# lowquark/uflow

Hardware: AMD Instinct MI355X
Metric: device-resident frame-CRC GiB/s (1500-B frames, validate: crc+valid per frame) (higher is better)
Workload: dtype u8

## Files before the change

### include/uflow_frame_crc.h

```cpp
#ifndef UFLOW_FRAME_CRC_H
#define UFLOW_FRAME_CRC_H

#include <stddef.h>
#include <stdint.h>

#ifdef __cplusplus
extern "C" {
#endif

#define UFC_OK 0
#define UFC_ERR_INVALID_ARG (-1)
#define UFC_ERR_NO_DEVICE (-2)
#define UFC_ERR_HIP (-3)
#define UFC_ERR_NOMEM (-4)
#define UFC_ERR_COMM (-5)
#define UFC_ERR_PEER (-6)

#define UFC_FRAME_CRC_SIZE 4
#define UFC_FRAME_OVERHEAD 5
#define UFC_MAX_FRAME_SIZE 1472

uint32_t ufc_crc32_compute(const uint8_t* data, size_t len);
uint32_t ufc_crc32_extend(uint32_t initial_crc, const uint8_t* data, size_t len);
int ufc_frame_validate(const uint8_t* frame, size_t len);
int ufc_frame_seal(uint8_t* frame, size_t len);

typedef struct ufc_ctx ufc_ctx;
int ufc_device_count(void);
int ufc_ctx_create(ufc_ctx** out, int device);
int ufc_ctx_destroy(ufc_ctx* ctx);
int ufc_ctx_release_stream(ufc_ctx* ctx, void* stream);
const char* ufc_error_string(int code);
int ufc_ctx_last_hip_error(const ufc_ctx* ctx);

#define UFC_OPT_FIXED_KERNEL 0
#define UFC_FIXED_AUTO 0
#define UFC_FIXED_GENERIC 1
#define UFC_FIXED_CLAIM16 2
#define UFC_OPT_VARLEN_KERNEL 1
#define UFC_VARLEN_AUTO 0
#define UFC_VARLEN_GENERIC 1
#define UFC_VARLEN_SORTED 2
#define UFC_VARLEN_BLOCKED8 3
#define UFC_VARLEN_CLAIM16 4
#define UFC_VARLEN_BLOCKSTREAM 5
#define UFC_VARLEN_SORTED8 6
#define UFC_VARLEN_STREAM 7
#define UFC_OPT_GENERIC_JC 2
#define UFC_OPT_SEAL_KERNEL 3
#define UFC_SEAL_INLINE 0
#define UFC_SEAL_TWO_PASS 1
#define UFC_OPT_COUNT_ 4
int ufc_ctx_set_option(ufc_ctx* ctx, int option, int value);
int ufc_ctx_get_option(const ufc_ctx* ctx, int option);

int ufc_crc_batch_fixed(ufc_ctx* ctx, const uint8_t* d_frames, size_t stride, size_t frame_len, size_t n,
                        uint32_t* d_crc_out, uint8_t* d_valid_out, void* stream);
int ufc_crc_batch_varlen(ufc_ctx* ctx, const uint8_t* d_bytes, const uint64_t* d_offsets, size_t n,
                         uint32_t* d_crc_out, uint8_t* d_valid_out, void* stream);
int ufc_seal_batch_fixed(ufc_ctx* ctx, uint8_t* d_frames, size_t stride, size_t frame_len, size_t n,
                         uint32_t* d_crc_out, void* stream);
int ufc_seal_batch_varlen(ufc_ctx* ctx, uint8_t* d_bytes, const uint64_t* d_offsets, size_t n,
                          uint32_t* d_crc_out, void* stream);

int ufc_crc_batch_pairs(ufc_ctx* ctx, const uint8_t* d_bytes, size_t bytes_len, const uint64_t* d_pairs, size_t n,
                        uint32_t* d_crc_out, uint8_t* d_valid_out, void* stream);

int ufc_hbm_read_probe(ufc_ctx* ctx, const uint8_t* d_buf, size_t bytes, uint32_t* d_sink, size_t* bytes_read,
                       void* stream);

int ufc_validate_host_varlen(ufc_ctx* ctx, const uint8_t* h_bytes, const uint64_t* h_offsets, size_t n,
                             uint32_t* h_crc_out, uint8_t* h_valid_out);
int ufc_validate_host_slots(ufc_ctx* ctx, const uint8_t* h_slots, size_t slot_stride, const uint32_t* h_lens,
                            size_t n, uint32_t* h_crc_out, uint8_t* h_valid_out);
int ufc_validate_host_slots_async(ufc_ctx* ctx, const uint8_t* h_slots, size_t slot_stride, const uint32_t* h_lens,
                                  size_t n, uint32_t* h_crc_out, uint8_t* h_valid_out, void* stream);
int ufc_seal_host_slots(ufc_ctx* ctx, uint8_t* h_slots, size_t slot_stride, const uint32_t* h_lens, size_t n,
                        uint32_t* h_crc_scratch);
int ufc_seal_host_varlen(ufc_ctx* ctx, uint8_t* h_bytes, const uint64_t* h_offsets, size_t n, uint32_t* h_crc_scratch);

#define UFC_COMM_ID_BYTES 128
#define UFC_MAX_RANKS 64
typedef struct ufc_comm ufc_comm;
int ufc_shard_range(uint64_t n_total, int nranks, int rank, uint64_t* first, uint64_t* count);
int ufc_shard_chunk(uint64_t n_total, int nranks, int rank, int chunk, uint64_t* first, uint64_t* count);
int ufc_shard_bounds_fixed(uint64_t n_total, int nranks, uint64_t* bounds);
int ufc_shard_bounds_varlen(const uint64_t* h_offsets, uint64_t n_total, int nranks, uint64_t* bounds);
#define UFC_OP_GATE 0
#define UFC_OP_SEND 1
#define UFC_OP_RECV 2
typedef struct ufc_xfer {
  int32_t op;
  int32_t peer;
  uint64_t src;
  uint64_t dst;
  uint64_t count;
} ufc_xfer;
int ufc_shard_nchunks(const uint64_t* bounds, int nranks);
int ufc_shard_gather_plan(const uint64_t* bounds, int nranks, int rank, int root, int chunk, ufc_xfer* ops,
                          int max_ops);
int ufc_comm_id_create(uint8_t id[UFC_COMM_ID_BYTES]);
int ufc_comm_create(ufc_comm** out, ufc_ctx* ctx, int nranks, int rank, const uint8_t id[UFC_COMM_ID_BYTES]);
int ufc_comm_destroy(ufc_comm* comm);
int ufc_comm_set_timeout(ufc_comm* comm, int timeout_ms);
int ufc_comm_last_error(const ufc_comm* comm);
int ufc_crc_sharded(ufc_comm* comm, const uint8_t* d_frames, size_t stride, size_t frame_len, uint64_t n_total,
                    uint32_t* d_crc_out, uint8_t* d_valid_out, int root, void* stream, void* gather_stream);
int ufc_crc_sharded_varlen(ufc_comm* comm, const uint8_t* d_bytes, const uint64_t* d_offsets, const uint64_t* bounds,
                           uint32_t* d_crc_out, uint8_t* d_valid_out, int root, void* stream, void* gather_stream);

#ifdef __cplusplus
}
#endif

#endif
```

### uflow_amd/_build.py

```python
import os
import subprocess
import sys

PKG_DIR = os.path.dirname(os.path.abspath(__file__))
REPO_DIR = os.path.dirname(PKG_DIR)
CSRC = os.path.join(PKG_DIR, "csrc")
LIB_PATH = os.path.join(PKG_DIR, "libuflowcrc.so")
SOURCES = ["frame_crc.hip", "frame_crc_varlen8.hip", "frame_parse.hip", "frame_build.hip", "frame_pack.hip",
           "packet_emit.hip", "packet_receive.hip", "frame_window.hip", "frame_queue.hip", "send_rate.hip", "resend.hip",
           "flush_ctl.hip", "route.hip", "hbm_probe.hip", "ufc_api.cpp", "ufc_shard.cpp", "crc_math.cpp",
           "frame_codec.cpp"]
HEADERS = ["frame_crc_dev.hpp", "frame_crc_kernels.hpp", "crc_math.hpp", "frame_codec_core.hpp", "frame_parse.hpp",
           "frame_parse_plan.hpp", "frame_build.hpp", "frame_build_piece.hpp", "frame_pack.hpp", "packet_emit.hpp",
           "packet_receive.hpp", "frame_window.hpp", "frame_queue.hpp", "send_rate.hpp", "resend.hpp", "flush_ctl.hpp",
           "route.hpp", "ufc_internal.hpp", "wave.hpp", "wave_dev.hpp", "scratch.hpp", "scan.hpp"]
HIPCC = os.environ.get("HIPCC", "/opt/rocm/bin/hipcc")


def _stale(target, deps):
    if not os.path.exists(target):
        return True
    t = os.path.getmtime(target)
    return any(os.path.getmtime(d) > t for d in deps)


def _digest(paths, extra=()):
    import hashlib
    h = hashlib.sha256()
    for p in paths:
        h.update(os.path.relpath(p, REPO_DIR).encode() + b"\0")
        with open(p, "rb") as f:
            h.update(f.read())
    for x in extra:
        h.update(str(x).encode() + b"\0")
    return h.hexdigest()


def _stamp_ok(target, digest):
    try:
        with open(target + ".sha256") as f:
            return os.path.exists(target) and f.readline().strip() == digest
    except OSError:
        return False


def _stamp_defines(target):
    try:
        with open(target + ".sha256") as f:
            f.readline()
            line = f.readline().strip()
    except OSError:
        return ()
    return tuple(line[len("defines:"):].split()) if line.startswith("defines:") else ()


def _native_identity(defines=()):
    sources = list(SOURCES)
    deps = [os.path.join(CSRC, s) for s in sources + HEADERS]
    deps += [os.path.join(REPO_DIR, "include", h)
             for h in ("uflow_frame_crc.h", "uflow_frame_codec.h", "uflow_flush_ctl.h", "uflow_route.h")]
    flags = [HIPCC, "-O3", "--offload-arch=gfx950", "-fPIC", "-std=c++17", "-Wall",
             "-mllvm", "-amdgpu-atomic-optimizer-strategy=None"]
    flags += ["-D" + d for d in defines]
    per_source = {s: list(UNSTRUCTURED_FLAGS) for s in UNSTRUCTURED_SOURCES}
    extra = [f"{s}:{' '.join(per_source[s])}" for s in sorted(per_source)]
    return sources, flags, per_source, _digest(deps + [os.path.abspath(__file__)], flags[1:] + extra)


UNSTRUCTURED_FLAGS = ("-mllvm", "-structurizecfg-skip-uniform-regions=true")
UNSTRUCTURED_SOURCES = ("frame_crc_varlen8.hip", "frame_crc.hip")


def build_native(force=False, verbose=False, out=None, defines=()):
    sources, flags, per_source, digest = _native_identity(defines)
    target = out or LIB_PATH
    if not force and _stamp_ok(target, digest):
        return target
    objdir = os.path.join(REPO_DIR, "build", "obj_" + os.path.basename(target).replace(".", "_"))
    os.makedirs(objdir, exist_ok=True)
    jobs, objs = [], []
    for src in sources:
        obj = os.path.join(objdir, src + ".o")
        objs.append(obj)
        jobs.append(flags + per_source.get(src, []) + ["-c", os.path.join(CSRC, src), "-o", obj])
    from concurrent.futures import ThreadPoolExecutor

    def run(cmd):
        if verbose:
            print(" ".join(cmd), file=sys.stderr)
        return subprocess.run(cmd).returncode

    with ThreadPoolExecutor(max_workers=max(1, min(8, len(jobs)))) as ex:
        rcs = list(ex.map(run, jobs))
    if any(rcs):
        raise subprocess.CalledProcessError(max(rcs), "hipcc")
    link = [HIPCC, "--offload-arch=gfx950", "-shared", "-fPIC", "-o", target + ".tmp"] + objs + ["-ldl"]
    if verbose:
        print(" ".join(link), file=sys.stderr)
    subprocess.run(link, check=True)
    os.replace(target + ".tmp", target)
    with open(target + ".sha256", "w") as f:
        f.write(digest + "\n")
        if defines:
            f.write("defines: " + " ".join(defines) + "\n")
    return target


LOOPBACK_SRC = os.path.join(REPO_DIR, "tools", "loopback", "ufc_loopback.cpp")
LOOPBACK_BIN = os.path.join(REPO_DIR, "tools", "loopback", "ufc_loopback")


def build_tools(force=False, verbose=False):
    deps = [LOOPBACK_SRC] + [os.path.join(REPO_DIR, "include", h) for h in ("uflow_frame_crc.h", "uflow_frame_codec.h")]
    cmd = [HIPCC, "-O2", "-std=c++17", "-Wall", "-o", LOOPBACK_BIN + ".tmp", LOOPBACK_SRC,
           "-L" + PKG_DIR, "-luflowcrc", "-Wl,-rpath,$ORIGIN/../../uflow_amd", "-lpthread"]
    digest = _digest(deps + [os.path.abspath(__file__)], cmd[1:])
    if not force and _stamp_ok(LOOPBACK_BIN, digest):
        return LOOPBACK_BIN
    if verbose:
        print(" ".join(cmd), file=sys.stderr)
    subprocess.run(cmd, check=True)
    os.replace(LOOPBACK_BIN + ".tmp", LOOPBACK_BIN)
    with open(LOOPBACK_BIN + ".sha256", "w") as f:
        f.write(digest + "\n")
    return LOOPBACK_BIN


def build_oracle(force=False):
    odir = os.path.join(REPO_DIR, "oracle")
    target = os.path.join(odir, "liboracle.so")
    digest = _digest([os.path.join(odir, "crc_oracle.c"), os.path.join(odir, "Makefile")])
    if force or not _stamp_ok(target, digest):
        subprocess.run(["make", "-C", odir, "-s", "-B"], check=True)
        with open(target + ".sha256", "w") as f:
            f.write(digest + "\n")
    return target


if __name__ == "__main__":
    build_native(force="--force" in sys.argv, verbose=True)
    build_oracle(force="--force" in sys.argv)
    build_tools(force="--force" in sys.argv, verbose=True)
    print(LIB_PATH)
```

### uflow_amd/_native.py

```python
import ctypes
import os

from ._build import LIB_PATH as _DEFAULT_LIB

LIB_PATH = os.environ["UFC_LIB"] if os.environ.get("UFC_AB") == "1" and os.environ.get("UFC_LIB") else _DEFAULT_LIB

UFC_OK = 0
UFC_ERR_INVALID_ARG = -1
UFC_ERR_NO_DEVICE = -2
UFC_ERR_HIP = -3
UFC_ERR_NOMEM = -4
UFC_ERR_COMM = -5
UFC_ERR_PEER = -6
UFC_COMM_ID_BYTES = 128
UFC_MAX_RANKS = 64
UFC_OP_GATE, UFC_OP_SEND, UFC_OP_RECV = 0, 1, 2

UFC_OPT_FIXED_KERNEL, UFC_OPT_VARLEN_KERNEL, UFC_OPT_GENERIC_JC = 0, 1, 2
UFC_FIXED_AUTO, UFC_FIXED_GENERIC, UFC_FIXED_CLAIM16 = 0, 1, 2
UFC_VARLEN_AUTO, UFC_VARLEN_GENERIC, UFC_VARLEN_SORTED, UFC_VARLEN_BLOCKED8, UFC_VARLEN_CLAIM16 = 0, 1, 2, 3, 4
UFC_VARLEN_BLOCKSTREAM, UFC_VARLEN_SORTED8, UFC_VARLEN_STREAM = 5, 6, 7
UFC_OPT_SEAL_KERNEL, UFC_SEAL_INLINE, UFC_SEAL_TWO_PASS = 3, 0, 1
UFC_BUILD_OK, UFC_BUILD_SKIPPED, UFC_BUILD_BAD_FIELD, UFC_BUILD_BAD_SRC = 0, 1, 2, 3
UFC_PACK_DONE, UFC_PACK_SIZE_LIMITED, UFC_PACK_WINDOW_LIMITED, UFC_PACK_BAD_RANGE = 0, 1, 2, 3
UFC_SEND_TIME_SENSITIVE, UFC_SEND_UNRELIABLE, UFC_SEND_PERSISTENT, UFC_SEND_RELIABLE = 0, 1, 2, 3
UFC_NO_PARENT = 0xFFFFFFFF
UFC_EMIT_DONE, UFC_EMIT_WINDOW_LIMITED, UFC_EMIT_ALLOC_LIMITED, UFC_EMIT_BAD_PACKET, UFC_EMIT_BAD_RANGE = 0, 1, 2, 3, 4
UFC_PACKET_NOT_REACHED, UFC_PACKET_EMITTED, UFC_PACKET_DROPPED = 0, 1, 2
UFC_RX_ASM_OPEN, UFC_RX_ASM_CLOSED, UFC_RX_ASM_ACTIVE = 0, 1, 2
UFC_RX_SLOT_ENTRY, UFC_RX_SLOT_DATA, UFC_RX_SLOT_DUD = 1, 2, 4
UFC_RX_PACKET_DUD = 1
(UFC_RX_NOT_HANDLED, UFC_RX_STORED, UFC_RX_COMPLETED, UFC_RX_DUD, UFC_RX_DROPPED_INVALID, UFC_RX_DROPPED_WINDOW,
 UFC_RX_DROPPED_CHANNEL, UFC_RX_DROPPED_CLOSED, UFC_RX_DROPPED_MISMATCH, UFC_RX_DROPPED_DUPLICATE,
 UFC_RX_DROPPED_BAD_SRC) = range(11)
UFC_RX_STATUS_COUNT = 11
UFC_RX_DONE, UFC_RX_BAD_STATE = 0, 1
UFC_FW_DONE, UFC_FW_BAD_STATE = 0, 1
UFC_SENT_NONCE, UFC_SENT_RATE_LIMITED, UFC_SENT_ACKED, UFC_SENT_MARK = 1, 2, 4, 8
UFC_FQ_HAS_RTT, UFC_FQ_RESET_LOSS, UFC_FQ_MARK_RATE_LIMITED, UFC_FQ_FORGET, UFC_FQ_FEEDBACK = 1, 2, 4, 8, 16
UFC_FQ_DONE, UFC_FQ_BAD_STATE = 0, 1
UFC_RATE_AWAIT_SEND, UFC_RATE_SLOW_START, UFC_RATE_THROUGHPUT_EQN = 0, 1, 2
UFC_RATE_FRAME_SENT = 1
UFC_RATE_DONE, UFC_RATE_BAD_STATE, UFC_RATE_REF_PANIC, UFC_RATE_RECV_FULL = 0, 1, 2, 3
UFC_RATE_FEEDBACK, UFC_RATE_NOFEEDBACK, UFC_RATE_RESET_ISSUED, UFC_RATE_ENTERED_EQN, UFC_RATE_INV_STALLED = 1, 2, 4, 8, 16
UFC_TX_RESEND = 1
UFC_RS_NO_DATA_FLUSH = 1
(UFC_RS_DONE, UFC_RS_SIZE_LIMITED, UFC_RS_WINDOW_LIMITED, UFC_RS_REF_HANG, UFC_RS_BAD_STATE, UFC_RS_STAGE_FULL,
 UFC_RS_HEAP_FULL) = range(7)
UFC_FA_DONE, UFC_FA_BAD_STATE, UFC_FA_CARRY_FULL = 0, 1, 2
(UFC_FS_SENT, UFC_FS_ACK_LIMITED, UFC_FS_DATA_LIMITED, UFC_FS_UPSTREAM, UFC_FS_NOT_DUE, UFC_FS_IDLE,
 UFC_FS_NO_ALLOC) = range(7)
UFC_ROUTE_DROP, UFC_ROUTE_CONN, UFC_ROUTE_CONTROL, UFC_ROUTE_DEFERRED = range(4)

_c_u8p = ctypes.POINTER(ctypes.c_uint8)
_V, _Z, _I = ctypes.c_void_p, ctypes.c_size_t, ctypes.c_int
_PARSE_ARGS = [_V, _V, _Z, _V, _V, _V, _Z]
_BUILD_SIZES_ARGS = [_V, _V, _Z, _V, _Z, _Z, _V, _V]
_BUILD_ARGS = [_V, _V, _Z, _V, _V, _Z, _Z, _V, _V, _Z, _I, _V]
_PACK_ARGS = [_V, _Z, _V, _V, _Z, _V, _V, _Z, _V]
_EMIT_ARGS = [_V, _Z, _V, _V, _Z, _V, _Z, _V, _V, _V, _V]
_RX_ARGS = [_V, _Z, _V, _V, _Z, _V, _V, _Z, _V, _V, _Z, _V, _V, _Z, _V, _Z, _V, _Z, _V, _V, _V, _Z, _V, _V, _V, _Z, _V,
            _V, _V, _V]
_FW_ARGS = [_V, _Z, _V, _V, _Z, _V, _V, _Z, _V, _V, _V, _V]
_FQ_ARGS = [_V, _Z, _V, _Z, _V, _V, _Z, _V, _V, _V, _Z, _V, _Z, _V, _Z, _V, _V]
_RATE_BEGIN_ARGS = [_V, _V, _V, _Z, _V, _V]
_RS_BEGIN_ARGS = [_V, _Z, _V, _V, _V, _Z, _V, _V, _V, _V, _V, _Z, _V, _Z, _V, _Z, _V, _Z, _V, _Z, _V, _Z, _V, _Z, _V, _V,
                  _V]
_RS_PLACE_ARGS = [_V, _V, _Z, _V, _Z, _V, _V, _Z]
_RS_COMMIT_ARGS = [_V, _V, _Z, _V, _V, _V, _Z, _V, _V, _Z, _V, _V, _V, _V, _V, _V, _V, _Z, _V, _Z, _V, _Z, _V, _Z, _V, _Z,
                   _V, _Z, _V, _V, _V, _V, _V]
_RATE_STEP_ARGS = [_V, _V, _V, _Z, _V, _Z, _V, _Z, _V, _V, _Z, _V, _V, _V]
_FLUSH_ACKS_ARGS = [_V, _V, _V, _Z, _V, _V, _V, _Z, _V, _Z, _V, _Z, _V, _V, _V, _Z, _V, _V, _V, _V, _V, _V, _V]
_FLUSH_SYNC_ARGS = [_V, _V, _V, _V, _V, _V, _V, _V, _Z, _V, _Z, _V, _V, _V, _V, _V]
_U32, _U64 = ctypes.c_uint32, ctypes.c_uint64
_ROUTE_ARGS = [_V, _V, _V, _Z, _V, _Z, _U32, _U32, _Z, _V, _U64, _U64, _V, _V, _V, _V, _V, _V, _V, _V, _V, _V]
_SIGNATURES = {
    "ufc_crc32_compute": (ctypes.c_uint32, [ctypes.c_void_p, ctypes.c_size_t]),
    "ufc_crc32_extend": (ctypes.c_uint32, [ctypes.c_uint32, ctypes.c_void_p, ctypes.c_size_t]),
    "ufc_frame_validate": (ctypes.c_int, [ctypes.c_void_p, ctypes.c_size_t]),
    "ufc_frame_seal": (ctypes.c_int, [ctypes.c_void_p, ctypes.c_size_t]),
    "ufc_device_count": (ctypes.c_int, []),
    "ufc_ctx_create": (ctypes.c_int, [ctypes.POINTER(ctypes.c_void_p), ctypes.c_int]),
    "ufc_ctx_destroy": (ctypes.c_int, [ctypes.c_void_p]),
    "ufc_ctx_release_stream": (ctypes.c_int, [ctypes.c_void_p, ctypes.c_void_p]),
    "ufc_error_string": (ctypes.c_char_p, [ctypes.c_int]),
    "ufc_ctx_last_hip_error": (ctypes.c_int, [ctypes.c_void_p]),
    "ufc_ctx_set_option": (ctypes.c_int, [ctypes.c_void_p, ctypes.c_int, ctypes.c_int]),
    "ufc_ctx_get_option": (ctypes.c_int, [ctypes.c_void_p, ctypes.c_int]),
    "ufc_crc_batch_fixed": (ctypes.c_int, [ctypes.c_void_p, ctypes.c_void_p, ctypes.c_size_t, ctypes.c_size_t,
                                           ctypes.c_size_t, ctypes.c_void_p, ctypes.c_void_p, ctypes.c_void_p]),
    "ufc_crc_batch_varlen": (ctypes.c_int, [ctypes.c_void_p, ctypes.c_void_p, ctypes.c_void_p, ctypes.c_size_t,
                                            ctypes.c_void_p, ctypes.c_void_p, ctypes.c_void_p]),
    "ufc_seal_batch_fixed": (ctypes.c_int, [ctypes.c_void_p, ctypes.c_void_p, ctypes.c_size_t, ctypes.c_size_t,
                                            ctypes.c_size_t, ctypes.c_void_p, ctypes.c_void_p]),
    "ufc_seal_batch_varlen": (ctypes.c_int, [ctypes.c_void_p, ctypes.c_void_p, ctypes.c_void_p, ctypes.c_size_t,
                                             ctypes.c_void_p, ctypes.c_void_p]),
    "ufc_hbm_read_probe": (ctypes.c_int, [ctypes.c_void_p, ctypes.c_void_p, ctypes.c_size_t, ctypes.c_void_p,
                                          ctypes.POINTER(ctypes.c_size_t), ctypes.c_void_p]),
    "ufc_validate_host_varlen": (ctypes.c_int, [ctypes.c_void_p, ctypes.c_void_p, ctypes.c_void_p, ctypes.c_size_t,
                                                ctypes.c_void_p, ctypes.c_void_p]),
    "ufc_crc_batch_pairs": (ctypes.c_int, [ctypes.c_void_p, ctypes.c_void_p, ctypes.c_size_t, ctypes.c_void_p,
                                           ctypes.c_size_t, ctypes.c_void_p, ctypes.c_void_p, ctypes.c_void_p]),
    "ufc_validate_host_slots": (ctypes.c_int, [ctypes.c_void_p, ctypes.c_void_p, ctypes.c_size_t, ctypes.c_void_p,
                                               ctypes.c_size_t, ctypes.c_void_p, ctypes.c_void_p]),
    "ufc_validate_host_slots_async": (ctypes.c_int, [ctypes.c_void_p, ctypes.c_void_p, ctypes.c_size_t, ctypes.c_void_p,
                                                     ctypes.c_size_t, ctypes.c_void_p, ctypes.c_void_p, ctypes.c_void_p]),
    "ufc_seal_host_slots": (ctypes.c_int, [ctypes.c_void_p, ctypes.c_void_p, ctypes.c_size_t, ctypes.c_void_p,
                                           ctypes.c_size_t, ctypes.c_void_p]),
    "ufc_seal_host_varlen": (ctypes.c_int, [ctypes.c_void_p, ctypes.c_void_p, ctypes.c_void_p, ctypes.c_size_t,
                                            ctypes.c_void_p]),
    "ufc_shard_range": (ctypes.c_int, [ctypes.c_uint64, ctypes.c_int, ctypes.c_int, ctypes.POINTER(ctypes.c_uint64),
                                       ctypes.POINTER(ctypes.c_uint64)]),
    "ufc_shard_chunk": (ctypes.c_int, [ctypes.c_uint64, ctypes.c_int, ctypes.c_int, ctypes.c_int,
                                       ctypes.POINTER(ctypes.c_uint64), ctypes.POINTER(ctypes.c_uint64)]),
    "ufc_shard_bounds_fixed": (ctypes.c_int, [ctypes.c_uint64, ctypes.c_int, ctypes.c_void_p]),
    "ufc_shard_bounds_varlen": (ctypes.c_int, [ctypes.c_void_p, ctypes.c_uint64, ctypes.c_int, ctypes.c_void_p]),
    "ufc_shard_nchunks": (ctypes.c_int, [ctypes.c_void_p, ctypes.c_int]),
    "ufc_shard_gather_plan": (ctypes.c_int, [ctypes.c_void_p, ctypes.c_int, ctypes.c_int, ctypes.c_int, ctypes.c_int,
                                             ctypes.c_void_p, ctypes.c_int]),
    "ufc_comm_id_create": (ctypes.c_int, [ctypes.c_void_p]),
    "ufc_comm_create": (ctypes.c_int, [ctypes.POINTER(ctypes.c_void_p), ctypes.c_void_p, ctypes.c_int, ctypes.c_int,
                                       ctypes.c_void_p]),
    "ufc_comm_destroy": (ctypes.c_int, [ctypes.c_void_p]),
    "ufc_comm_last_error": (ctypes.c_int, [ctypes.c_void_p]),
    "ufc_comm_set_timeout": (ctypes.c_int, [ctypes.c_void_p, ctypes.c_int]),
    "ufc_crc_sharded": (ctypes.c_int, [ctypes.c_void_p, ctypes.c_void_p, ctypes.c_size_t, ctypes.c_size_t, ctypes.c_uint64,
                                       ctypes.c_void_p, ctypes.c_void_p, ctypes.c_int, ctypes.c_void_p, ctypes.c_void_p]),
    "ufc_crc_sharded_varlen": (ctypes.c_int, [ctypes.c_void_p, ctypes.c_void_p, ctypes.c_void_p, ctypes.c_void_p,
                                              ctypes.c_void_p, ctypes.c_void_p, ctypes.c_int, ctypes.c_void_p,
                                              ctypes.c_void_p]),
    "ufc_frame_read": (ctypes.c_int, [ctypes.c_void_p, ctypes.c_size_t, ctypes.c_void_p, ctypes.c_void_p,
                                      ctypes.c_size_t]),
    "ufc_frame_parse": (ctypes.c_int, [ctypes.c_void_p, ctypes.c_size_t, ctypes.c_int, ctypes.c_void_p,
                                       ctypes.c_void_p, ctypes.c_size_t]),
    "ufc_datagram_is_valid": (ctypes.c_int, [ctypes.c_void_p]),
    "ufc_frame_write_fixed": (ctypes.c_size_t, [ctypes.c_void_p, ctypes.c_void_p, ctypes.c_size_t, ctypes.c_int]),
    "ufc_data_frame_builder_init": (ctypes.c_int, [ctypes.c_void_p, ctypes.c_void_p, ctypes.c_size_t, ctypes.c_uint32,
                                                   ctypes.c_int]),
    "ufc_data_frame_builder_add": (ctypes.c_int, [ctypes.c_void_p, ctypes.c_void_p]),
    "ufc_data_frame_encoded_size": (ctypes.c_size_t, [ctypes.c_void_p]),
    "ufc_ack_frame_builder_init": (ctypes.c_int, [ctypes.c_void_p, ctypes.c_void_p, ctypes.c_size_t, ctypes.c_uint32,
                                                  ctypes.c_uint32]),
    "ufc_ack_frame_builder_add": (ctypes.c_int, [ctypes.c_void_p, ctypes.c_uint32, ctypes.c_uint32, ctypes.c_int]),
    "ufc_builder_size": (ctypes.c_size_t, [ctypes.c_void_p]),
    "ufc_builder_build": (ctypes.c_size_t, [ctypes.c_void_p, ctypes.c_int]),
    "ufc_parse_batch_host": (_I, _PARSE_ARGS + [ctypes.POINTER(_Z), _I]),
    "ufc_parse_batch_varlen": (_I, [_V] + _PARSE_ARGS + [_V, _V]),
    "ufc_build_sizes_host": (_I, _BUILD_SIZES_ARGS + [_I]),
    "ufc_build_batch_host": (_I, _BUILD_ARGS + [_I]),
    "ufc_build_sizes_varlen": (_I, [_V] + _BUILD_SIZES_ARGS + [_V]),
    "ufc_build_batch_varlen": (_I, [_V] + _BUILD_ARGS + [_V]),
    "ufc_pack_host": (_I, _PACK_ARGS + [ctypes.POINTER(ctypes.c_uint64), _I]),
    "ufc_pack_varlen": (_I, [_V] + _PACK_ARGS + [_V, _V]),
    "ufc_emit_packets_host": (_I, _EMIT_ARGS + [ctypes.POINTER(ctypes.c_uint64), _I]),
    "ufc_emit_packets_varlen": (_I, [_V] + _EMIT_ARGS + [_V, _V]),
    "ufc_receive_packets_host": (ctypes.c_int, _RX_ARGS + [ctypes.c_int]),
    "ufc_receive_packets_varlen": (ctypes.c_int, [ctypes.c_void_p] + _RX_ARGS + [ctypes.c_void_p]),
    "ufc_frame_window_host": (ctypes.c_int, _FW_ARGS + [ctypes.c_int]),
    "ufc_frame_window_varlen": (ctypes.c_int, [ctypes.c_void_p] + _FW_ARGS + [ctypes.c_void_p]),
    "ufc_frame_queue_host": (ctypes.c_int, _FQ_ARGS + [ctypes.c_int]),
    "ufc_frame_queue_varlen": (ctypes.c_int, [ctypes.c_void_p] + _FQ_ARGS + [ctypes.c_void_p]),
    "ufc_rate_begin_host": (ctypes.c_int, _RATE_BEGIN_ARGS + [ctypes.c_int]),
    "ufc_rate_begin_varlen": (ctypes.c_int, [ctypes.c_void_p] + _RATE_BEGIN_ARGS + [ctypes.c_void_p]),
    "ufc_rate_step_host": (ctypes.c_int, _RATE_STEP_ARGS + [ctypes.c_int]),
    "ufc_rate_step_varlen": (ctypes.c_int, [ctypes.c_void_p] + _RATE_STEP_ARGS + [ctypes.c_void_p]),
    "ufc_resend_begin_host": (ctypes.c_int, _RS_BEGIN_ARGS + [ctypes.c_int]),
    "ufc_resend_begin_varlen": (ctypes.c_int, [ctypes.c_void_p] + _RS_BEGIN_ARGS + [ctypes.c_void_p]),
    "ufc_resend_place_host": (ctypes.c_int, _RS_PLACE_ARGS + [ctypes.c_int]),
    "ufc_resend_place_varlen": (ctypes.c_int, [ctypes.c_void_p] + _RS_PLACE_ARGS + [ctypes.c_void_p]),
    "ufc_resend_commit_host": (ctypes.c_int, _RS_COMMIT_ARGS + [ctypes.c_int]),
    "ufc_resend_commit_varlen": (ctypes.c_int, [ctypes.c_void_p] + _RS_COMMIT_ARGS + [ctypes.c_void_p]),
}
SYMBOLS = tuple(_SIGNATURES)
_FLUSH_SIGNATURES = {
    "ufc_flush_acks_host": (_I, _FLUSH_ACKS_ARGS + [_I]),
    "ufc_flush_acks_varlen": (_I, [_V] + _FLUSH_ACKS_ARGS + [_V]),
    "ufc_flush_sync_host": (_I, _FLUSH_SYNC_ARGS + [_I]),
    "ufc_flush_sync_varlen": (_I, [_V] + _FLUSH_SYNC_ARGS + [_V]),
}
FLUSH_SYMBOLS = tuple(_FLUSH_SIGNATURES)
_ROUTE_SIGNATURES = {
    "ufc_route_table_build_host": (_I, [_V, _Z, _U32, _V, _Z, _V, _V]),
    "ufc_route_frames_host": (_I, _ROUTE_ARGS + [_I]),
    "ufc_route_frames_varlen": (_I, [_V] + _ROUTE_ARGS + [_V]),
}
ROUTE_SYMBOLS = tuple(_ROUTE_SIGNATURES)


class FrameInfo(ctypes.Structure):
    _fields_ = [("kind", ctypes.c_uint8), ("ok", ctypes.c_uint8), ("aux", ctypes.c_uint8), ("crc_ok", ctypes.c_uint8),
                ("f", ctypes.c_uint32 * 5), ("item_count", ctypes.c_uint32), ("item_first", ctypes.c_uint32)]


class Item(ctypes.Structure):
    _fields_ = [("id", ctypes.c_uint32), ("channel_id", ctypes.c_uint8), ("form", ctypes.c_uint8),
                ("window_parent_lead", ctypes.c_uint16), ("channel_parent_lead", ctypes.c_uint16),
                ("fragment_id", ctypes.c_uint16), ("fragment_id_last", ctypes.c_uint16), ("flags", ctypes.c_uint16),
                ("data_offset", ctypes.c_uint32), ("data_len", ctypes.c_uint32)]


class Builder(ctypes.Structure):
    _fields_ = [("buf", ctypes.c_void_p), ("cap", ctypes.c_size_t), ("len", ctypes.c_size_t),
                ("count", ctypes.c_uint32), ("kind", ctypes.c_uint32)]


class Xfer(ctypes.Structure):
    _fields_ = [("op", ctypes.c_int32), ("peer", ctypes.c_int32), ("src", ctypes.c_uint64), ("dst", ctypes.c_uint64),
                ("count", ctypes.c_uint64)]


class DatagramRef(ctypes.Structure):
    _fields_ = [("sequence_id", ctypes.c_uint32), ("channel_id", ctypes.c_uint8), ("reserved", ctypes.c_uint8),
                ("window_parent_lead", ctypes.c_uint16), ("channel_parent_lead", ctypes.c_uint16),
                ("fragment_id", ctypes.c_uint16), ("fragment_id_last", ctypes.c_uint16),
                ("data", ctypes.c_void_p), ("data_len", ctypes.c_size_t)]

_lib = None


class NativeError(RuntimeError):
    def __init__(self, code, what=""):
        msg = _lib.ufc_error_string(code).decode() if _lib is not None else str(code)
        super().__init__(f"{what}: {msg} (code {code})" if what else f"{msg} (code {code})")
        self.code = code


def lib():
    global _lib
    if _lib is None:
        if not os.path.exists(LIB_PATH):
            raise ImportError(f"libuflowcrc.so not found at {LIB_PATH}: run `python -m uflow_amd._build` "
                              "(the native library is required; there is no CPU fallback)")
        l = ctypes.CDLL(LIB_PATH)
        for name, (res, args) in (list(_SIGNATURES.items()) + list(_FLUSH_SIGNATURES.items()) +
                                   list(_ROUTE_SIGNATURES.items())):
            fn = getattr(l, name)
            fn.restype = res
            fn.argtypes = args
        _lib = l
    return _lib


def check(rc, what=""):
    if rc != UFC_OK:
        raise NativeError(rc, what)
    return rc
```

### uflow_amd/csrc/frame_crc.hip

```cpp
#include "frame_crc_dev.hpp"

namespace ufc_dev {

struct RunAcc {
  uint32_t crc;
  uint32_t valid;
};

template <bool SEAL>
__device__ __forceinline__ void finish_set(const Lane& L, const KernelParams& p, const FrameDesc& d, const Chains& c,
                                           uint64_t set, int t, RunAcc& acc) {
  const uint32_t X0 = L.odd ? c.v2 : c.v0, X1 = L.odd ? c.v3 : c.v1;
  const uint32_t X2 = L.odd ? c.v0 : c.v2, X3 = L.odd ? c.v1 : c.v3;
  uint32_t lin = xor3(nib_mul<0>(L.lds, X0, L.K2), nib_mul<1>(L.lds, X1, L.K2), nib_mul<2>(L.lds, X2, L.K2)) ^
                 nib_mul<3>(L.lds, X3, L.K2);
  lin = row_xor16(lin);
  const uint32_t crc = ~lin;
  if (SEAL) {
    const uint64_t f = set * 4 + (uint64_t)L.grp;
    if (L.col == 15 && f < p.nframes && d.len >= 4u) {
      uint8_t* a = p.wbytes + d.start + d.n;
      if (((uintptr_t)a & 3u) == 0) {
        *as_global<g_u32w>((uint32_t*)a) = __builtin_bswap32(crc);
      } else {
        g_u8w* w = as_global<g_u8w>(a);
        w[0] = (uint8_t)(crc >> 24);
        w[1] = (uint8_t)(crc >> 16);
        w[2] = (uint8_t)(crc >> 8);
        w[3] = (uint8_t)crc;
      }
    }
  }
  const uint32_t ok = (d.len >= 5u && __builtin_bswap32(c.tr) == crc) ? 1u : 0u;
  const int dst = L.lane - 4 * t;
#pragma unroll
  for (int g = 0; g < 4; g++) {
    const uint32_t cg = __builtin_amdgcn_readlane(crc, 16 * g);
    acc.crc = (dst == g) ? cg : acc.crc;
    if (!SEAL) {
      const uint32_t vg = __builtin_amdgcn_readlane(ok, 16 * g + 15);
      acc.valid = (dst == g) ? vg : acc.valid;
    }
  }
}

template <bool SEAL>
__device__ __forceinline__ void store_run(const Lane& L, const KernelParams& p, uint64_t run_first, const RunAcc& acc) {
  const uint64_t f = run_first + (uint64_t)L.lane;
  if (f < p.nframes) {
    if (p.crc_out) *as_global<g_u32w>(p.crc_out + f) = acc.crc;
    if (!SEAL && p.valid_out) *as_global<g_u8w>(p.valid_out + f) = (uint8_t)acc.valid;
  }
}

template <bool SEAL>
__device__ __forceinline__ void slow_set(const Lane& L, const KernelParams& p, const FrameDesc& d, int nblocks,
                                         uint64_t set, int t, RunAcc& acc) {
  Chains c{0u, 0u, 0u, 0u, 0u};
#pragma unroll 1
  for (int blk = 0; blk < nblocks; blk++) {
    const int bl = min(blk, d.J - 1);
    uint32_t w[4];
#pragma unroll
    for (int b = 0; b < 4; b++) {
      const int o = 256 * bl + 16 * L.col + 4 * b - d.pad;
      uint32_t a = 0;
#pragma unroll 1
      for (int k = 0; k < 4; k++) {
        const int ob = o + k;
        if (ob >= 0 && ob < (int)d.len) a |= (uint32_t)*as_global<g_u8>(p.bytes + d.start + (uint64_t)ob) << (8 * k);
      }
      w[b] = a;
    }
    process_block<true>(L, d, blk, make_uint4(w[0], w[1], w[2], w[3]), c);
  }
  finish_set<SEAL>(L, p, d, c, set, t, acc);
}


template <int JC>
__device__ __forceinline__ void load_item(const uint8_t* lane_base, int part, ItemBuf<JC>& b) {
  const uint8_t* q = lane_base + (int64_t)part * (JC * 256);
#pragma unroll
  for (int j = 0; j < JC; j++) {
    const u32x4 v = __builtin_nontemporal_load(as_global<g_u32x4>(q + 256 * j));
    b.x[j] = make_uint4(v.x, v.y, v.z, v.w);
  }
}

template <int JC, bool FREEZE, bool PART0>
__device__ __forceinline__ void compute_item(const Lane& L, const FrameDesc& d, int part, const ItemBuf<JC>& b,
                                             Chains& c) {
#pragma unroll
  for (int j = 0; j < JC; j++) process_block<FREEZE>(L, d, PART0 ? j : part * JC + j, b.x[j], c);
}

template <int JC, int MODE>
__global__ __launch_bounds__(1024) void frame_crc_kernel(const KernelParams p) {
  constexpr bool VARLEN = (MODE & kModeVarlen) != 0;
  constexpr bool SEAL = (MODE & kModeSeal) != 0;
  constexpr bool FREEZE = VARLEN || (MODE & kModeFreeze) != 0;
  constexpr bool SINGLE = !VARLEN && (MODE & kModeFreeze) == 0;
  __shared__ __attribute__((aligned(16))) char lds[kLdsBytes];
  stage_tables(p, lds);

  Lane L;
  init_lane(L, lds, p.G);
  const uint64_t nsets = (p.nframes + 3) >> 2;
  const uint64_t W = (uint64_t)gridDim.x * (blockDim.x >> 6);
  const uint32_t wid = __builtin_amdgcn_readfirstlane(threadIdx.x >> 6);
  const uint64_t w0 = (uint64_t)blockIdx.x * (blockDim.x >> 6) + wid;
  constexpr int R = kSetsPerRun;
  uint64_t run = w0;
  int t = 0;
  if (run * R >= nsets) return;
  auto set_of = [&](uint64_t r, int tt) -> uint64_t { return r * R + (uint64_t)tt; };
  auto next_pos = [&](uint64_t r, int tt, uint64_t& r2, int& t2) {
    if (tt + 1 < R && set_of(r, tt + 1) < nsets) {
      r2 = r;
      t2 = tt + 1;
    } else {
      r2 = r + W;
      t2 = 0;
    }
  };
  const uint64_t buf_end =
      VARLEN ? *as_global<g_u64>(p.offsets + p.nframes) : (p.nframes - 1) * p.stride + p.frame_len;

  auto frame_index = [&](uint64_t set) -> uint64_t {
    const uint64_t f = set * 4 + (uint64_t)L.grp;
    return f < p.nframes ? f : p.nframes - 1;
  };
  auto desc_now = [&](uint64_t set) -> FrameDesc {
    const uint64_t f = frame_index(set);
    if (VARLEN) {
      const uint64_t a = *as_global<g_u64>(p.offsets + f), b = *as_global<g_u64>(p.offsets + f + 1);
      return make_desc(a, b - a);
    }
    return make_desc(f * p.stride, p.frame_len);
  };
  auto wave_max = [&](int v) -> int {
    int m = __builtin_amdgcn_readlane(v, 0);
    m = max(m, __builtin_amdgcn_readlane(v, 16));
    m = max(m, __builtin_amdgcn_readlane(v, 32));
    m = max(m, __builtin_amdgcn_readlane(v, 48));
    return m;
  };
  auto set_parts = [&](const FrameDesc& dd) -> int { return (wave_max(dd.J) + JC - 1) / JC; };
  auto set_slow = [&](const FrameDesc& dd, int parts) -> bool {
    const int bad =
        (dd.start < (uint64_t)dd.pad || dd.start - dd.pad + (uint64_t)(256 * JC) * parts > buf_end) ? 1 : 0;
    return wave_max(bad) != 0;
  };

  RunAcc acc{0u, 0u};
  auto after_set = [&](uint64_t r, int tt) {
    uint64_t r2;
    int t2;
    next_pos(r, tt, r2, t2);
    if (r2 != r) store_run<SEAL>(L, p, set_of(r, 0) * 4, acc);
  };

  FrameDesc d = desc_now(set_of(run, t));
  int parts = set_parts(d);
  while (set_slow(d, parts)) {
    slow_set<SEAL>(L, p, d, parts * JC, set_of(run, t), t, acc);
    after_set(run, t);
    next_pos(run, t, run, t);
    if (set_of(run, t) >= nsets) return;
    d = desc_now(set_of(run, t));
    parts = set_parts(d);
  }

  struct Cursor {
    uint64_t run;
    int t, part, parts;
    bool valid, slow;
    FrameDesc d;
  };
  uint64_t pre_a = 0, pre_b = 0;
  auto prefetch_offsets = [&](uint64_t r2, int t2) {
    if (VARLEN) {
      const uint64_t s2 = set_of(r2, t2);
      const uint64_t f = frame_index(s2 < nsets ? s2 : 0);
      pre_a = *as_global<g_u64>(p.offsets + f);
      pre_b = *as_global<g_u64>(p.offsets + f + 1);
    }
  };
  auto advance = [&](Cursor& c) {
    if (!c.valid || c.slow) {
      c.valid = false;
      return;
    }
    if (!SINGLE && c.part + 1 < c.parts) {
      c.part++;
      return;
    }
    uint64_t r2;
    int t2;
    next_pos(c.run, c.t, r2, t2);
    c.run = r2;
    c.t = t2;
    c.part = 0;
    if (set_of(r2, t2) >= nsets) {
      c.valid = false;
      return;
    }
    c.d = VARLEN ? make_desc(pre_a, pre_b - pre_a) : make_desc(frame_index(set_of(r2, t2)) * p.stride, p.frame_len);
    {
      uint64_t r3;
      int t3;
      next_pos(r2, t2, r3, t3);
      prefetch_offsets(r3, t3);
    }
    c.parts = set_parts(c.d);
    c.slow = set_slow(c.d, c.parts);
  };
  auto lane_base = [&](const Cursor& c) -> const uint8_t* { return p.bytes + c.d.start - c.d.pad + 16 * L.col; };

  Cursor C0{run, t, 0, parts, true, false, d};
  {
    uint64_t r2;
    int t2;
    next_pos(run, t, r2, t2);
    prefetch_offsets(r2, t2);
  }
  Cursor C1 = C0;
  advance(C1);
  Cursor C2 = C1;
  advance(C2);
  auto load_cursor = [&](const Cursor& c, ItemBuf<JC>& b) {
    const bool ok = c.valid && !c.slow;
    load_item<JC>(ok ? lane_base(c) : lane_base(C0), ok ? c.part : 0, b);
  };

  Chains c{0u, 0u, 0u, 0u, 0u};
  bool go_slow = false;
  uint64_t slow_run = 0;
  int slow_t = 0;
  auto step = [&](ItemBuf<JC>& cur, ItemBuf<JC>& nxt2) -> bool {
    {
      const bool ok = C2.valid && !C2.slow;
      const uint8_t* q = (ok ? lane_base(C2) : lane_base(C0)) + (int64_t)(ok ? C2.part : 0) * (JC * 256);
      const bool p0 = SINGLE || C0.part == 0;
      if (!p0) __builtin_assume(C0.part >= 1);
#pragma unroll
      for (int j = 0; j < JC; j++) {
        const u32x4 v = __builtin_nontemporal_load(as_global<g_u32x4>(q + 256 * j));
        nxt2.x[j] = make_uint4(v.x, v.y, v.z, v.w);
        __builtin_amdgcn_sched_barrier(0);
        if (p0)
          process_block<FREEZE>(L, C0.d, j, cur.x[j], c);
        else
          process_block<FREEZE>(L, C0.d, C0.part * JC + j, cur.x[j], c);
        __builtin_amdgcn_sched_barrier(0);
      }
    }
    if (SINGLE || C0.part + 1 == C0.parts) {
      finish_set<SEAL>(L, p, C0.d, c, set_of(C0.run, C0.t), C0.t, acc);
      after_set(C0.run, C0.t);
    }
    if (!C1.valid) return false;
    if (C1.slow) {
      go_slow = true;
      slow_run = C1.run;
      slow_t = C1.t;
      return false;
    }
    C0 = C1;
    C1 = C2;
    advance(C2);
    return true;
  };
  {
    ItemBuf<JC> X, Y, Z;
    load_cursor(C0, X);
    load_cursor(C1, Y);
    while (step(X, Z) && step(Y, X) && step(Z, Y)) {
    }
  }
  if (go_slow) {
    run = slow_run;
    t = slow_t;
    while (set_of(run, t) < nsets) {
      d = desc_now(set_of(run, t));
      parts = set_parts(d);
      slow_set<SEAL>(L, p, d, parts * JC, set_of(run, t), t, acc);
      after_set(run, t);
      next_pos(run, t, run, t);
    }
  }
}




constexpr int lean_loadv(int skip, int first, int mid, int last) { return skip | first << 1 | mid << 6 | last << 11; }
[[maybe_unused]] constexpr int kLoadvAllNT = lean_loadv(0, kFixAuxNT, kFixAuxNT, kFixAuxNT);
constexpr int kLoadvProduct = lean_loadv(0, 0, kFixAuxNT, kFixAuxNT);
template <int J, bool SEAL, int DEPTH, int SCHED, int WAVES, int LOADV = kLoadvProduct>
__global__ __launch_bounds__(WAVES * 64) void frame_crc_fixed_kernel(const KernelParams p) {
  static_assert(DEPTH >= 1 && DEPTH <= 3, "pipeline depth (4 spills at J = 6)");
  static_assert(DEPTH != 1 || SCHED != kSchedClaim, "depth 1: static schedules only");
  constexpr bool DYN = SCHED == kSchedClaim;
  constexpr bool ILV = SCHED == kSchedInterleave;
  constexpr uint32_t kInc = ILV ? (uint32_t)WAVES : 1u;
  __shared__ __attribute__((aligned(16))) char lds[kLdsBytes];
  const StageSet<WAVES * 64> sr = stage_load<WAVES * 64>(p);
  Lane L;
  init_lane(L, lds, p.G);

  const uint64_t stride = p.stride;
  const uint32_t len = (uint32_t)p.frame_len;
  const uint32_t n = len - 4u;
  const int pad = J * 256 - (int)len;
  const uint32_t nsets = (uint32_t)((p.nframes + 3) >> 2);
  const uint32_t nfull = (uint32_t)(p.nframes >> 2);
  const bool tail = (p.nframes & 3) != 0;
  const uint32_t wpb = WAVES;
  const uint32_t wid = __builtin_amdgcn_readfirstlane(threadIdx.x >> 6);
  const uint32_t w = blockIdx.x * wpb + wid;
  const uint32_t s_edge =
      p.front_ok ? 0u : (uint32_t)min(((uint64_t)pad + 4 * stride - 1) / (4 * stride), (uint64_t)nsets);
  const bool edge0 = s_edge == 1 && (p.nframes - 1) * stride + len >= 16;
  const uint32_t s_fast = edge0 ? 0u : s_edge;
  const uint32_t nfast = nfull - s_fast;
  uint32_t q_lo, q_end, q_cur, q_nx1, q_nx2;
  if (DYN || ILV) {
    q_lo = s_fast + (uint32_t)((uint64_t)nfast * blockIdx.x / gridDim.x);
    q_end = s_fast + (uint32_t)((uint64_t)nfast * (blockIdx.x + 1) / gridDim.x);
    q_cur = q_lo + wid;
    q_nx1 = q_lo + wpb + wid;
  } else {
    const uint32_t NW = gridDim.x * wpb;
    q_lo = s_fast + (uint32_t)((uint64_t)nfast * w / NW);
    q_end = s_fast + (uint32_t)((uint64_t)nfast * (w + 1) / NW);
    q_cur = q_lo;
    q_nx1 = q_lo + 1;
  }
  uint32_t* ctr = DYN ? p.ctr + blockIdx.x * kCtrWordsPerBlock : nullptr;
  auto claim_issue = [&]() -> uint32_t {
    uint32_t v = 0;
    if (L.lane == 0) v = __hip_atomic_fetch_add(ctr, 1u, __ATOMIC_RELAXED, __HIP_MEMORY_SCOPE_AGENT);
    return v;
  };
  auto claim_set = [&](uint32_t v) -> uint32_t {
    return q_lo + (DEPTH - 1) * wpb + __builtin_amdgcn_readfirstlane(v);
  };

  const int64_t lane_off = (int64_t)L.grp * (int64_t)stride + 16 * L.col - pad;
  uint32_t dm[4], pre[4];
#pragma unroll
  for (int b = 0; b < 4; b++) {
    const int o = 16 * L.col + 4 * b - pad;
    const uint32_t fz = fix_word(0u, o, L.G);
    const uint32_t f1 = fix_word(0xFFFFFFFFu, o, L.G);
    dm[b] = f1 & ~fz;
    pre[b] = fz;
  }
  uint32_t dm1, pre1;
  {
    const int o = 256 + 16 * L.col - pad;
    const uint32_t fz = fix_word(0u, o, L.G), f1 = fix_word(0xFFFFFFFFu, o, L.G);
    dm1 = f1 & ~fz;
    pre1 = fz;
  }
  const uint32_t tmask = (L.col == 15) ? 0u : 0xFFFFFFFFu;

  constexpr int RUNS = lean_runs(WAVES);
  uint32_t acc_crc = 0, acc_qv = 0;
  uint32_t hist_crc[RUNS], hist_qv[RUNS];
#pragma unroll
  for (int r = 0; r < RUNS; r++) hist_crc[r] = hist_qv[r] = 0;
  uint32_t t = 0, nhist = 0;
  auto write_trailer = [&](uint64_t f, uint32_t crc) {
    uint8_t* a = p.wbytes + f * stride + n;
    if (((uintptr_t)a & 3u) == 0) {
      *as_global<g_u32w>((uint32_t*)a) = __builtin_bswap32(crc);
    } else {
      g_u8w* wp = as_global<g_u8w>(a);
      wp[0] = (uint8_t)(crc >> 24);
      wp[1] = (uint8_t)(crc >> 16);
      wp[2] = (uint8_t)(crc >> 8);
      wp[3] = (uint8_t)crc;
    }
  };
  auto store_run = [&](int cnt, uint32_t crcs, uint32_t qv) {
    const uint64_t f = (uint64_t)(qv & 0x7FFFFFFFu) * 4 + (uint64_t)L.grp;
    if (L.col < cnt && f < p.nframes) {
      if (p.crc_out) *as_global<g_u32w>(p.crc_out + f) = crcs;
      if (!SEAL && p.valid_out) *as_global<g_u8w>(p.valid_out + f) = (uint8_t)(qv >> 31);
      if (SEAL) write_trailer(f, crcs);
    }
  };
  auto store_all = [&]() {
    if (t > 0) store_run((int)t, acc_crc, acc_qv);
#pragma unroll
    for (int r = 0; r < RUNS; r++)
      if ((uint32_t)r < nhist) store_run(kSetsPerRun, hist_crc[r], hist_qv[r]);
  };
  auto finish = [&](uint32_t q, const Chains& c, bool may_overflow) {
    const uint32_t crc = ~group_lin(L, c);
    const uint32_t tr = (uint32_t)__builtin_amdgcn_update_dpp(0, (int)c.tr, 0x15F, 0xF, 0xF, false);
    const uint32_t ok = (len >= 5u && __builtin_bswap32(tr) == crc) ? 1u : 0u;
    acc_crc = (L.col == (int)t) ? crc : acc_crc;
    acc_qv = (L.col == (int)t) ? (q | (ok << 31)) : acc_qv;
    if (++t == kSetsPerRun) {
      if (may_overflow && nhist == RUNS) {
        t = 0;
        store_all();
        __builtin_amdgcn_s_waitcnt(0x0F70);
        nhist = 0;
      }
#pragma unroll
      for (int r = RUNS - 1; r > 0; r--) {
        hist_crc[r] = hist_crc[r - 1];
        hist_qv[r] = hist_qv[r - 1];
      }
      hist_crc[0] = acc_crc;
      hist_qv[0] = acc_qv;
      nhist++;
      t = 0;
    }
  };
  auto compute_block = [&](uint32_t q, int j, uint4 x, Chains& c) {
    {
      if (j == J - 1) {
        c.tr = x.w;
        x.w &= tmask;
      }
      if (j == 0) {
        c.v0 = (x.x & dm[0]) | pre[0];
        c.v1 = (x.y & dm[1]) | pre[1];
        c.v2 = (x.z & dm[2]) | pre[2];
        c.v3 = (x.w & dm[3]) | pre[3];
      } else {
        if (j == 1) x.x = (x.x & dm1) | pre1;
        c.v0 = chain_step(L.lds, c.v0, L.K, x.x);
        c.v1 = chain_step(L.lds, c.v1, L.K, x.y);
        c.v2 = chain_step(L.lds, c.v2, L.K, x.z);
        c.v3 = chain_step(L.lds, c.v3, L.K, x.w);
      }
    }
  };
  auto compute = [&](uint32_t q, const ItemBuf<J>& b, Chains& c) {
#pragma unroll
    for (int j = 0; j < J; j++) compute_block(q, j, b.x[j], c);
  };
  const uint32_t voff = (uint32_t)(lane_off + 512);
  auto set_base = [&](uint32_t q) -> const uint8_t* {
    return p.bytes + (uint64_t)(q < q_end ? q : nfull - 1) * 4 * stride - 512;
  };
  auto load_edge0 = [&](ItemBuf<J>& b) {
    const int64_t room = (int64_t)min(p.nframes - 1, (uint64_t)3);
    const int64_t over = (int64_t)L.grp > room ? (int64_t)L.grp - room : 0;
    const int64_t off0 = lane_off - over * (int64_t)stride;
#pragma unroll
    for (int j = 0; j < J; j++) {
      const int64_t off = off0 + 256 * j;
      uint4 v = load_frame16<true>(p.bytes + (off < 0 ? 0 : off));
      if (off < 0) {
        const int64_t d = -off;
        uint64_t lo = (uint64_t)v.x | ((uint64_t)v.y << 32), hi = (uint64_t)v.z | ((uint64_t)v.w << 32);
        if (d >= 16) {
          lo = hi = 0;
        } else if (d >= 8) {
          hi = lo << (8 * (d - 8));
          lo = 0;
        } else {
          hi = (hi << (8 * d)) | (lo >> (64 - 8 * d));
          lo = lo << (8 * d);
        }
        v = make_uint4((uint32_t)lo, (uint32_t)(lo >> 32), (uint32_t)hi, (uint32_t)(hi >> 32));
      }
      b.x[j] = v;
    }
  };
  const uint32_t voff_b0 = ((LOADV & 1) && 16 * L.col + 16 <= pad - 4) ? kFixRecords : voff;
  auto load = [&](uint32_t q, ItemBuf<J>& b) {
    constexpr int kAuxFirst = (LOADV >> 1) & 31, kAuxMid = (LOADV >> 6) & 31, kAuxLast = (LOADV >> 11) & 31;
    const __amdgpu_buffer_rsrc_t rs =
        __builtin_amdgcn_make_buffer_rsrc((void*)set_base(q), 0, (int)kFixRecords, kFixRsrcWord3);
#pragma unroll
    for (int j = 0; j < J; j++) {
      const uint32_t o = (j == 0 ? voff_b0 : voff) + 256u * j;
      u32x4 v;
      if (j == 0)
        v = __builtin_amdgcn_raw_buffer_load_b128(rs, (int)o, 0, kAuxFirst);
      else if (j == J - 1)
        v = __builtin_amdgcn_raw_buffer_load_b128(rs, (int)o, 0, kAuxLast);
      else
        v = __builtin_amdgcn_raw_buffer_load_b128(rs, (int)o, 0, kAuxMid);
      b.x[j] = make_uint4(v.x, v.y, v.z, v.w);
    }
  };
  auto load_tail = [&](ItemBuf<J>& b) {
    const int64_t room = (int64_t)(p.nframes - 1 - 4 * (uint64_t)nfull);
    const int64_t over = (int64_t)L.grp > room ? (int64_t)L.grp - room : 0;
    load_set<J>(p.bytes + (uint64_t)nfull * 4 * stride - 512, voff - (uint32_t)(over * (int64_t)stride), b);
  };

  ItemBuf<J> A, B, C;
  uint32_t cX = 0, cY = 0, cZ = 0;
  if (DYN) {
    cY = claim_issue();
    cZ = claim_issue();
  }
  if (edge0 && q_cur == 0)
    load_edge0(A);
  else
    load(q_cur, A);
  if (DEPTH == 3) load(q_nx1, B);
  stage_store<WAVES * 64>(sr, lds);
  q_nx2 = (DEPTH == 3 && !DYN) ? q_cur + 2 * kInc : 0;

  if (w == 0 && s_fast > 0) {
#pragma unroll 1
    for (uint32_t e = 0; e < s_fast; e++) {
      FrameDesc d = make_desc(min((uint64_t)e * 4 + (uint64_t)L.grp, p.nframes - 1) * stride, len);
      Chains ce{0u, 0u, 0u, 0u, 0u};
#pragma unroll 1
      for (int blk = 0; blk < J; blk++) {
        uint32_t wv[4];
#pragma unroll
        for (int b = 0; b < 4; b++) {
          const int o = 256 * blk + 16 * L.col + 4 * b - d.pad;
          uint32_t a = 0;
#pragma unroll 1
          for (int k = 0; k < 4; k++) {
            const int ob = o + k;
            if (ob >= 0 && ob < (int)d.len) a |= (uint32_t)*as_global<g_u8>(p.bytes + d.start + (uint64_t)ob) << (8 * k);
          }
          wv[b] = a;
        }
        process_block<false>(L, d, blk, make_uint4(wv[0], wv[1], wv[2], wv[3]), ce);
      }
      const uint32_t crc = ~group_lin(L, ce);
      const uint32_t ok = (len >= 5u && __builtin_bswap32(ce.tr) == crc) ? 1u : 0u;
      const uint64_t f = (uint64_t)e * 4 + (uint64_t)L.grp;
      if (L.col == 15 && f < p.nframes) {
        if (p.crc_out) *as_global<g_u32w>(p.crc_out + f) = crc;
        if (!SEAL && p.valid_out) *as_global<g_u8w>(p.valid_out + f) = (uint8_t)ok;
        if (SEAL) write_trailer(f, crc);
      }
    }
    __builtin_amdgcn_s_waitcnt(0x0F70);
  }


  Chains c{0u, 0u, 0u, 0u, 0u};
  auto step = [&](ItemBuf<J>& cur, ItemBuf<J>& fill, uint32_t& c_issue, uint32_t& c_read) {
    uint32_t q_load;
    if (DYN) {
      q_load = claim_set(c_read);
      c_issue = claim_issue();
    } else {
      q_load = (DEPTH == 3) ? q_nx2 : q_nx1;
    }
    load(q_load, fill);
    __builtin_amdgcn_sched_barrier(0);
    if (q_cur < q_end) {
      compute(q_cur, cur, c);
      finish(q_cur, c, DYN);
    }
    __builtin_amdgcn_sched_barrier(0);
    if (DEPTH == 3) {
      q_cur = q_nx1;
      q_nx1 = q_load;
      q_nx2 = q_load + kInc;
    } else {
      q_cur = q_load;
      q_nx1 = q_load + kInc;
    }
  };
  if (DEPTH == 1) {
    while (q_cur < q_end) {
      compute(q_cur, A, c);
      finish(q_cur, c, false);
      q_cur += kInc;
      load(q_cur, A);
    }
  } else if (DEPTH == 2 && !DYN) {
    while (q_cur < q_end) {
      step(A, B, cX, cY);
      step(B, A, cY, cZ);
    }
  } else if (DEPTH == 2) {
    while (q_cur < q_end) {
      step(A, B, cX, cY);
      step(B, A, cY, cZ);
      step(A, B, cZ, cX);
      step(B, A, cX, cY);
      step(A, B, cY, cZ);
      step(B, A, cZ, cX);
    }
  } else {
    while (q_cur < q_end) {
      step(A, C, cX, cY);
      step(B, A, cY, cZ);
      step(C, B, cZ, cX);
    }
  }
  if (tail && blockIdx.x == gridDim.x - 1 && wid == wpb - 1) {
    ItemBuf<J> T;
    load_tail(T);
    compute(nfull, T, c);
    const uint32_t crc = ~group_lin(L, c);
    const uint32_t tr = (uint32_t)__builtin_amdgcn_update_dpp(0, (int)c.tr, 0x15F, 0xF, 0xF, false);
    const uint32_t ok = (len >= 5u && __builtin_bswap32(tr) == crc) ? 1u : 0u;
    const uint64_t f = (uint64_t)nfull * 4 + (uint64_t)L.grp;
    if (L.col == 0 && f < p.nframes) {
      if (p.crc_out) *as_global<g_u32w>(p.crc_out + f) = crc;
      if (!SEAL && p.valid_out) *as_global<g_u8w>(p.valid_out + f) = (uint8_t)ok;
      if (SEAL) write_trailer(f, crc);
    }
  }
  if (DYN) {
    store_all();
  } else {
    uint32_t blo = q_lo, bhi = q_end;
    if (!ILV) {
      const uint64_t NW = (uint64_t)gridDim.x * wpb;
      blo = s_fast + (uint32_t)((uint64_t)nfast * (blockIdx.x * wpb) / NW);
      bhi = s_fast + (uint32_t)((uint64_t)nfast * ((blockIdx.x + 1) * wpb) / NW);
    }
    const uint32_t nfr = 4 * (bhi - blo);
    uint32_t* lcrc = (uint32_t*)lds;
    uint8_t* lval = (uint8_t*)lds + 4 * nfr;
    __builtin_amdgcn_fence(__ATOMIC_RELEASE, "workgroup", "local");
    __builtin_amdgcn_s_barrier();
    __builtin_amdgcn_fence(__ATOMIC_ACQUIRE, "workgroup", "local");
    auto stage = [&](int cnt, uint32_t crcs, uint32_t qv) {
      if (L.col < cnt) {
        const uint32_t q = qv & 0x7FFFFFFFu;
        const uint32_t pos = (q - blo) * 4 + (uint32_t)L.grp;
        lcrc[pos] = crcs;
        lval[pos] = (uint8_t)(qv >> 31);
      }
    };
    if (t > 0) stage((int)t, acc_crc, acc_qv);
#pragma unroll
    for (int r = 0; r < RUNS; r++)
      if ((uint32_t)r < nhist) stage(kSetsPerRun, hist_crc[r], hist_qv[r]);
    __builtin_amdgcn_fence(__ATOMIC_RELEASE, "workgroup", "local");
    __builtin_amdgcn_s_barrier();
    __builtin_amdgcn_fence(__ATOMIC_ACQUIRE, "workgroup", "local");
    const uint64_t f0 = (uint64_t)blo * 4;
    if (p.crc_out)
      for (uint32_t i = threadIdx.x; i < nfr; i += WAVES * 64) *as_global<g_u32w>(p.crc_out + f0 + i) = lcrc[i];
    if (SEAL) {
      for (uint32_t i = threadIdx.x; i < nfr; i += WAVES * 64) {
        const uint32_t v = __builtin_bswap32(lcrc[i]);
        uint8_t* a = p.wbytes + (f0 + i) * stride + n;
        if (((uintptr_t)a & 3u) == 0) {
          __builtin_nontemporal_store(v, as_global<g_u32w>((uint32_t*)a));
        } else {
          g_u8w* wp = as_global<g_u8w>(a);
          __builtin_nontemporal_store((uint8_t)v, wp);
          __builtin_nontemporal_store((uint8_t)(v >> 8), wp + 1);
          __builtin_nontemporal_store((uint8_t)(v >> 16), wp + 2);
          __builtin_nontemporal_store((uint8_t)(v >> 24), wp + 3);
        }
      }
    }
    if (!SEAL && p.valid_out) {
      if ((((uintptr_t)(p.valid_out + f0)) & 3u) == 0) {
        for (uint32_t i = threadIdx.x; i < nfr / 4; i += WAVES * 64)
          *as_global<g_u32w>((uint32_t*)(p.valid_out + f0) + i) = ((const uint32_t*)lval)[i];
      } else {
        for (uint32_t i = threadIdx.x; i < nfr; i += WAVES * 64) *as_global<g_u8w>(p.valid_out + f0 + i) = lval[i];
      }
    }
  }

  if (DYN) {
    __builtin_amdgcn_s_waitcnt(0x0F70);
    uint32_t done = 0;
    if (L.lane == 0) done = __hip_atomic_fetch_add(ctr + 1, 1u, __ATOMIC_RELAXED, __HIP_MEMORY_SCOPE_AGENT);
    if (__builtin_amdgcn_readfirstlane(done) == wpb - 1 && L.lane == 0) {
      __hip_atomic_store(ctr, 0u, __ATOMIC_RELAXED, __HIP_MEMORY_SCOPE_AGENT);
      __hip_atomic_store(ctr + 1, 0u, __ATOMIC_RELAXED, __HIP_MEMORY_SCOPE_AGENT);
    }
  }
}

#define UFC_INST_FIXED(J)                                                                                  \
  template __global__ void frame_crc_fixed_kernel<J, false, 2, kSchedInterleave, 8>(const KernelParams); \
  template __global__ void frame_crc_fixed_kernel<J, true, 2, kSchedInterleave, 8>(const KernelParams);
UFC_INST_FIXED(1) UFC_INST_FIXED(2) UFC_INST_FIXED(3) UFC_INST_FIXED(4) UFC_INST_FIXED(5) UFC_INST_FIXED(6)


const void* fixed_kernel_symbol(int J, bool seal, int depth, int sched, int waves) {
  if (depth == 2 && sched == kSchedInterleave && waves == 8) {
    switch (J) {
#define UFC_PICK_FIXED(JJ)                                                                          \
  case JJ:                                                                                          \
    return seal ? (const void*)frame_crc_fixed_kernel<JJ, true, 2, kSchedInterleave, 8>          \
                : (const void*)frame_crc_fixed_kernel<JJ, false, 2, kSchedInterleave, 8>;
      UFC_PICK_FIXED(1) UFC_PICK_FIXED(2) UFC_PICK_FIXED(3) UFC_PICK_FIXED(4) UFC_PICK_FIXED(5) UFC_PICK_FIXED(6)
#undef UFC_PICK_FIXED
      default: return nullptr;
    }
  }
  return nullptr;
}

#define UFC_INST_MODES(JC)                                                                          \
  template __global__ void frame_crc_kernel<JC, 0>(const KernelParams);                             \
  template __global__ void frame_crc_kernel<JC, kModeSeal>(const KernelParams);                     \
  template __global__ void frame_crc_kernel<JC, kModeFreeze>(const KernelParams);                   \
  template __global__ void frame_crc_kernel<JC, kModeFreeze | kModeSeal>(const KernelParams);       \
  template __global__ void frame_crc_kernel<JC, kModeVarlen>(const KernelParams);                   \
  template __global__ void frame_crc_kernel<JC, kModeVarlen | kModeSeal>(const KernelParams);

#define UFC_CONFIGS(X) X(1) X(2) X(3) X(4) X(5) X(6)

UFC_CONFIGS(UFC_INST_MODES)


const void* kernel_symbol(int jc, int mode) {
#define UFC_PICK(JC)                                                                                   \
  if (jc == JC) {                                                                                      \
    switch (mode) {                                                                                    \
      case 0: return (const void*)frame_crc_kernel<JC, 0>;                                            \
      case kModeSeal: return (const void*)frame_crc_kernel<JC, kModeSeal>;                            \
      case kModeFreeze: return (const void*)frame_crc_kernel<JC, kModeFreeze>;                        \
      case kModeFreeze | kModeSeal: return (const void*)frame_crc_kernel<JC, kModeFreeze | kModeSeal>; \
      case kModeVarlen: return (const void*)frame_crc_kernel<JC, kModeVarlen>;                        \
      case kModeVarlen | kModeSeal: return (const void*)frame_crc_kernel<JC, kModeVarlen | kModeSeal>; \
      default: break;                                                                                  \
    }                                                                                                  \
  }
  UFC_CONFIGS(UFC_PICK)
#undef UFC_PICK
  return nullptr;
}

bool config_available(int jc) { return jc >= 1 && jc <= 6; }

namespace {
__global__ __launch_bounds__(256) void seal_scatter_kernel(uint8_t* bytes, uint64_t stride, uint64_t n_off,
                                                           uint64_t nframes, const uint32_t* crc) {
  for (uint64_t i = (uint64_t)blockIdx.x * 256 + threadIdx.x; i < nframes; i += (uint64_t)gridDim.x * 256) {
    const uint32_t v = __builtin_bswap32(crc[i]);
    uint8_t* a = bytes + i * stride + n_off;
    if (((uintptr_t)a & 3u) == 0) {
      __builtin_nontemporal_store(v, (uint32_t*)a);
    } else {
      __builtin_nontemporal_store((uint8_t)v, a);
      __builtin_nontemporal_store((uint8_t)(v >> 8), a + 1);
      __builtin_nontemporal_store((uint8_t)(v >> 16), a + 2);
      __builtin_nontemporal_store((uint8_t)(v >> 24), a + 3);
    }
  }
}
}

int seal_scatter(uint8_t* bytes, uint64_t stride, uint64_t frame_len, uint64_t nframes, const uint32_t* crc,
                 void* stream) {
  if (nframes == 0) return 0;
  const uint64_t blocks = std::min<uint64_t>((nframes + 255) / 256, 1u << 20);
  hipLaunchKernelGGL(seal_scatter_kernel, dim3((unsigned)blocks), dim3(256), 0, (hipStream_t)stream, bytes, stride,
                     frame_len - 4, nframes, crc);
  return (int)hipGetLastError();
}

}
```

### uflow_amd/csrc/frame_crc_dev.hpp

```cpp
#pragma once
#include <hip/hip_runtime.h>
#include <cstdint>

#include "frame_crc_kernels.hpp"

namespace ufc_dev {

typedef unsigned int u32x4 __attribute__((ext_vector_type(4)));
typedef const __attribute__((address_space(1))) u32x4 g_u32x4;
typedef const __attribute__((address_space(1))) uint8_t g_u8;
typedef const __attribute__((address_space(1))) uint32_t g_u32;
typedef const __attribute__((address_space(1))) uint64_t g_u64;
typedef __attribute__((address_space(1))) uint8_t g_u8w;
typedef __attribute__((address_space(1))) uint32_t g_u32w;

template <typename G, typename T>
__device__ __forceinline__ G* as_global(T* p) {
  return (G*)(p);
}

constexpr int kSetsPerRun = 16;

__device__ __forceinline__ uint32_t xor3(uint32_t a, uint32_t b, uint32_t c) {
  return __builtin_amdgcn_bitop3_b32(a, b, c, 0x96);
}

__device__ __forceinline__ uint32_t perm(uint32_t a, uint32_t b, uint32_t sel) {
  return __builtin_amdgcn_perm(a, b, sel);
}

constexpr uint32_t kChainBase = 32768u;
constexpr uint32_t kSelChain0 = 0x0C020400u, kSelChain1 = 0x0C020501u, kSelChain2 = 0x0C030600u,
                   kSelChain3 = 0x0C030701u;

__device__ __forceinline__ uint32_t chain_step(const char* lds, uint32_t v, uint32_t K, uint32_t x) {
  const char* t = lds + kChainBase;
  const uint32_t r0 = *(const uint32_t*)(t + perm(v, K, kSelChain0));
  const uint32_t r1 = *(const uint32_t*)(t + perm(v, K, kSelChain1));
  const uint32_t r2 = *(const uint32_t*)(t + perm(v, K, kSelChain2));
  const uint32_t r3 = *(const uint32_t*)(t + perm(v, K, kSelChain3));
  return xor3(xor3(r0, r1, r2), r3, x);
}

template <int I>
__device__ __forceinline__ uint32_t nib_mul(const char* lds, uint32_t v, uint32_t K2) {
  const uint32_t lo = v & 0x0F0F0F0Fu;
  const uint32_t hi = (v >> 4) & 0x0F0F0F0Fu;
  uint32_t r[8];
#pragma unroll
  for (int k = 0; k < 8; k++) {
    const uint32_t sel = 0x0C0C0000u | ((uint32_t)(4 + (k >> 1)) << 8) | (uint32_t)I;
    r[k] = *(const uint32_t*)(lds + perm((k & 1) ? hi : lo, K2, sel) + k * 4096);
  }
  return xor3(xor3(r[0], r[1], r[2]), xor3(r[3], r[4], r[5]), xor3(r[6], r[7], 0u));
}

template <int I>
__device__ __forceinline__ void nib_terms(const char* lds, uint32_t v, uint32_t K2, uint32_t* r) {
  const uint32_t lo = v & 0x0F0F0F0Fu, hi = (v >> 4) & 0x0F0F0F0Fu;
#pragma unroll
  for (int k = 0; k < 8; k++) {
    const uint32_t sel = 0x0C0C0000u | ((uint32_t)(4 + (k >> 1)) << 8) | (uint32_t)I;
    r[k] = *(const uint32_t*)(lds + perm((k & 1) ? hi : lo, K2, sel) + k * 4096);
  }
}

__device__ __forceinline__ uint32_t nib_mul4(const char* lds, uint32_t X0, uint32_t X1, uint32_t X2, uint32_t X3,
                                             uint32_t K2) {
  uint32_t r[32];
  nib_terms<0>(lds, X0, K2, r);
  nib_terms<1>(lds, X1, K2, r + 8);
  nib_terms<2>(lds, X2, K2, r + 16);
  nib_terms<3>(lds, X3, K2, r + 24);
  uint32_t t[12];
#pragma unroll
  for (int k = 0; k < 10; k++) t[k] = xor3(r[3 * k], r[3 * k + 1], r[3 * k + 2]);
  t[10] = r[30];
  t[11] = r[31];
  const uint32_t u0 = xor3(t[0], t[1], t[2]), u1 = xor3(t[3], t[4], t[5]), u2 = xor3(t[6], t[7], t[8]),
                 u3 = xor3(t[9], t[10], t[11]);
  return xor3(u0, u1, u2) ^ u3;
}

__device__ __forceinline__ uint32_t row_xor16(uint32_t v) {
  v ^= (uint32_t)__builtin_amdgcn_update_dpp(0, (int)v, 0xB1, 0xF, 0xF, false);
  v ^= (uint32_t)__builtin_amdgcn_update_dpp(0, (int)v, 0x4E, 0xF, 0xF, false);
  v ^= (uint32_t)__builtin_amdgcn_update_dpp(0, (int)v, 0x124, 0xF, 0xF, false);
  v ^= (uint32_t)__builtin_amdgcn_update_dpp(0, (int)v, 0x128, 0xF, 0xF, false);
  return v;
}


__host__ __device__ __forceinline__ uint32_t fix_word(uint32_t v, int o, uint32_t G) {
  const uint64_t pv = (uint64_t)G << 32;
  const uint32_t sh = (uint32_t)(8 * (o + 8)) & 63u;
  const uint32_t pre = (uint32_t)(pv >> sh);
  const uint32_t dm = (o > -4 && o < 0) ? (0xFFFFFFFFu << ((uint32_t)(-8 * o) & 31u)) : 0u;
  const uint32_t mixed = (v & dm) | (pre & ~dm);
  return (o >= 0) ? v : ((o <= -8) ? 0u : mixed);
}

__host__ __device__ __forceinline__ uint4 front_fix(uint4 x, int p, uint32_t G) {
  const uint32_t pc = (uint32_t)(p < 0 ? 0 : (p > 20 ? 20 : p));
  const uint32_t s = 8u * pc;
  const uint64_t lo = (uint64_t)x.x | ((uint64_t)x.y << 32), hi = (uint64_t)x.z | ((uint64_t)x.w << 32);
  const uint64_t mlo = s >= 64u ? 0ull : ~0ull << (s & 63u);
  const uint64_t mhi = s >= 128u ? 0ull : (s <= 64u ? ~0ull : ~0ull << ((s - 64u) & 63u));
  const int q = (int)pc - 4;
  const uint64_t g = G;
  const uint64_t glo = q < 0 ? (g >> ((uint32_t)(-8 * q) & 63u)) & (q == -4 ? 0ull : ~0ull)
                             : (q < 8 ? g << ((uint32_t)(8 * q) & 63u) : 0ull);
  const uint64_t ghi = q <= 4 ? 0ull
                              : (q < 8 ? g >> ((uint32_t)(64 - 8 * q) & 63u)
                                       : (q < 16 ? g << ((uint32_t)(8 * (q - 8)) & 63u) : 0ull));
  const uint64_t rlo = (lo & mlo) | glo, rhi = (hi & mhi) | ghi;
  return make_uint4((uint32_t)rlo, (uint32_t)(rlo >> 32), (uint32_t)rhi, (uint32_t)(rhi >> 32));
}

__host__ __device__ __forceinline__ uint32_t data_mask(int lb) {
  return lb >= 4 ? 0xFFFFFFFFu : (lb > 0 ? 0xFFFFFFFFu >> ((uint32_t)(32 - 8 * lb) & 31u) : 0u);
}

__host__ __device__ __forceinline__ uint32_t data_mask_bits(int b) {
  const uint32_t s = (uint32_t)(b < 0 ? 0 : (b > 32 ? 32 : b));
  return ~(uint32_t)(0xFFFFFFFFFFFFFFFFull << s);
}

__host__ __device__ __forceinline__ uint32_t frame_word_mask(int ob, uint32_t len) {
  const int lo = -ob < 0 ? 0 : (-ob > 4 ? 4 : -ob);
  const int64_t h = (int64_t)len - ob;
  const int hi = h < 0 ? 0 : (h > 4 ? 4 : (int)h);
  const uint32_t mhi = hi >= 4 ? ~0u : ((1u << ((uint32_t)(8 * hi) & 31u)) - 1u),
                 mlo = lo >= 4 ? 0u : (~0u << ((uint32_t)(8 * lo) & 31u));
  return mhi & mlo;
}

__host__ __device__ __forceinline__ uint32_t rot_nibble_key(uint32_t col, uint32_t u, uint32_t e) {
  const uint32_t R = 31u - (e & 31u), sh = (8u * u) & 31u;
  const uint32_t steps = (0x03020100u >> sh) | (0x03020100u << ((32u - sh) & 31u));
#if defined(__HIP_DEVICE_COMPILE__)
  const uint32_t rb = __builtin_amdgcn_perm(0u, R, 0u);
#else
  const uint32_t rb = R * 0x01010101u;
#endif
  return ((steps + (4u * (col & 7u)) * 0x01010101u + rb) & 0x1F1F1F1Fu) << 2;
}

struct FrameDesc {
  uint64_t start;
  uint32_t len;
  uint32_t n;
  int J;
  int pad;
};

__device__ __forceinline__ FrameDesc make_desc(uint64_t start, uint64_t len64) {
  FrameDesc d;
  d.start = start;
  d.len = (uint32_t)len64;
  d.n = d.len >= 4u ? d.len - 4u : d.len;
  const uint32_t E = d.n + 4u;
  d.J = (int)((E + 4u + 255u) >> 8);
  d.pad = d.J * 256 - (int)E;
  return d;
}

struct Lane {
  const char* lds;
  int lane;
  int col;
  int grp;
  bool odd;
  uint32_t K;
  uint32_t K2;
  uint32_t G;
};

struct Chains {
  uint32_t v0, v1, v2, v3;
  uint32_t tr;
};

template <bool FREEZE>
__device__ __forceinline__ void process_block(const Lane& L, const FrameDesc& d, int blk, uint4 x, Chains& c) {
  {
    const bool t = (L.col == 15) && (blk == d.J - 1);
    c.tr = t ? x.w : c.tr;
    x.w = t ? 0u : x.w;
  }
  if (blk == 0) {
    const int o = 16 * L.col - d.pad;
    c.v0 = fix_word(x.x, o, L.G);
    c.v1 = fix_word(x.y, o + 4, L.G);
    c.v2 = fix_word(x.z, o + 8, L.G);
    c.v3 = fix_word(x.w, o + 12, L.G);
    return;
  }
  if (blk == 1) x.x = fix_word(x.x, 256 + 16 * L.col - d.pad, L.G);
  const uint32_t n0 = chain_step(L.lds, c.v0, L.K, x.x);
  const uint32_t n1 = chain_step(L.lds, c.v1, L.K, x.y);
  const uint32_t n2 = chain_step(L.lds, c.v2, L.K, x.z);
  const uint32_t n3 = chain_step(L.lds, c.v3, L.K, x.w);
  if (FREEZE) {
    const bool act = blk < d.J;
    c.v0 = act ? n0 : c.v0;
    c.v1 = act ? n1 : c.v1;
    c.v2 = act ? n2 : c.v2;
    c.v3 = act ? n3 : c.v3;
  } else {
    c.v0 = n0; c.v1 = n1; c.v2 = n2; c.v3 = n3;
  }
}

__device__ __forceinline__ void stage_tables(const KernelParams& p, char* lds) {
  const int t = threadIdx.x;
  const uint32_t cv = *as_global<g_u32>(p.chain_tab + t);
  const u32x4 n0 = *as_global<g_u32x4>(p.nib_img + 8 * t);
  const u32x4 n1 = *as_global<g_u32x4>(p.nib_img + 8 * t + 4);
  const uint32_t k = (uint32_t)t >> 8, e = (uint32_t)t & 255u;
  const uint32_t cbase = kChainBase + (k >> 1) * 65536u + e * 256u + (k & 1u) * 128u;
  const u32x4 cr = {cv, cv, cv, cv};
#pragma unroll
  for (int i = 0; i < 8; i++) *(u32x4*)(lds + cbase + 16 * i) = cr;
  *(u32x4*)(lds + 32 * t) = n0;
  *(u32x4*)(lds + 32 * t + 16) = n1;
  __syncthreads();
}

__device__ __forceinline__ void init_lane(Lane& L, char* lds, uint32_t G) {
  L.lds = lds;
  L.lane = threadIdx.x & 63;
  L.col = L.lane & 15;
  L.grp = L.lane >> 4;
  L.odd = (L.grp & 1) != 0;
  L.G = G;
  const uint32_t c4 = (uint32_t)(L.lane & 31) * 4u;
  L.K = c4 | ((c4 + 128u) << 8) | (1u << 24);
  uint32_t k2 = 0;
#pragma unroll
  for (int i = 0; i < 4; i++) {
    const int sl = 4 * L.col + ((i + (L.odd ? 2 : 0)) & 3);
    k2 |= (uint32_t)(((sl >> 1) + 32 * (sl & 1)) * 4) << (8 * i);
  }
  L.K2 = k2;
}

__device__ __forceinline__ uint32_t group_lin(const Lane& L, const Chains& c) {
  const uint32_t X0 = L.odd ? c.v2 : c.v0, X1 = L.odd ? c.v3 : c.v1;
  const uint32_t X2 = L.odd ? c.v0 : c.v2, X3 = L.odd ? c.v1 : c.v3;
  const uint32_t lin = xor3(nib_mul<0>(L.lds, X0, L.K2), nib_mul<1>(L.lds, X1, L.K2), nib_mul<2>(L.lds, X2, L.K2)) ^
                       nib_mul<3>(L.lds, X3, L.K2);
  return row_xor16(lin);
}

template <int JC>
struct ItemBuf {
  uint4 x[JC];
};

template <bool NT>
__device__ __forceinline__ uint4 load_frame16(const uint8_t* q) {
  u32x4 v;
  if constexpr (NT)
    v = __builtin_nontemporal_load(as_global<g_u32x4>(q));
  else
    v = *as_global<g_u32x4>(q);
  return make_uint4(v.x, v.y, v.z, v.w);
}
constexpr uint32_t kFixRecords = 0x7FFFFFF0u;
constexpr int kFixRsrcWord3 = 0x00020000;
constexpr int kFixAuxNT = 2;
template <int J>
__device__ __forceinline__ void load_set(const uint8_t* sbase, uint32_t voff, ItemBuf<J>& b) {
  const __amdgpu_buffer_rsrc_t rs =
      __builtin_amdgcn_make_buffer_rsrc((void*)sbase, 0, (int)kFixRecords, kFixRsrcWord3);
#pragma unroll
  for (int j = 0; j < J; j++) {
    const u32x4 v = __builtin_amdgcn_raw_buffer_load_b128(rs, (int)(voff + 256u * j), 0, kFixAuxNT);
    b.x[j] = make_uint4(v.x, v.y, v.z, v.w);
  }
}

__device__ __forceinline__ void st_u32_hidden(uint32_t* a, uint32_t v) {
  asm volatile("global_store_dword %0, %1, off" : : "v"(a), "v"(v));
}
__device__ __forceinline__ void st_u8_hidden(uint8_t* a, uint32_t v) {
  asm volatile("global_store_byte %0, %1, off" : : "v"(a), "v"(v));
}

struct StageRegs {
  uint32_t cv;
  u32x4 n0, n1;
};
template <int THREADS = 1024>
struct StageSet {
  static constexpr int kRounds = (1024 + THREADS - 1) / THREADS;
  StageRegs r[kRounds];
};

template <int THREADS = 1024>
__device__ __forceinline__ StageSet<THREADS> stage_load(const KernelParams& p) {
  StageSet<THREADS> s;
#pragma unroll
  for (int i = 0; i < StageSet<THREADS>::kRounds; i++) {
    const int t = min((int)threadIdx.x + i * THREADS, 1023);
    s.r[i].cv = *as_global<g_u32>(p.chain_tab + t);
    s.r[i].n0 = *as_global<g_u32x4>(p.nib_img + 8 * t);
    s.r[i].n1 = *as_global<g_u32x4>(p.nib_img + 8 * t + 4);
  }
  return s;
}

template <int THREADS = 1024>
__device__ __forceinline__ void stage_store(const StageSet<THREADS>& s, char* lds) {
#pragma unroll
  for (int i = 0; i < StageSet<THREADS>::kRounds; i++) {
    const int t = (int)threadIdx.x + i * THREADS;
    if (1024 % THREADS != 0 && t >= 1024) break;
    const StageRegs& r = s.r[i];
    const uint32_t k = (uint32_t)t >> 8, e = (uint32_t)t & 255u;
    const uint32_t cbase = kChainBase + (k >> 1) * 65536u + e * 256u + (k & 1u) * 128u;
    const u32x4 cr = {r.cv, r.cv, r.cv, r.cv};
#pragma unroll
    for (int j = 0; j < 8; j++) *(u32x4*)(lds + cbase + 16 * j) = cr;
    *(u32x4*)(lds + 32 * t) = r.n0;
    *(u32x4*)(lds + 32 * t + 16) = r.n1;
  }
  __builtin_amdgcn_fence(__ATOMIC_RELEASE, "workgroup", "local");
  __builtin_amdgcn_s_barrier();
  __builtin_amdgcn_fence(__ATOMIC_ACQUIRE, "workgroup", "local");
}
}
```

### uflow_amd/csrc/frame_crc_kernels.hpp

```cpp
#pragma once
#include <cstdint>

namespace ufc_dev {

constexpr int kModeVarlen = 1;
constexpr int kModeSeal = 2;
constexpr int kModeFreeze = 4;

constexpr int kBlockThreads = 1024;
constexpr int kLdsBytes = 131072 + 32768;

struct KernelParams {
  const uint8_t* bytes;
  uint8_t* wbytes;
  const uint64_t* offsets;
  uint64_t stride;
  uint64_t frame_len;
  uint64_t nframes;
  uint32_t* crc_out;
  uint8_t* valid_out;
  const uint32_t* chain_tab;
  const uint32_t* nib_img;
  uint32_t G;
  uint32_t* ctr;
  uint32_t front_ok;
  uint32_t* defer_list;
  uint32_t* defer_counts;
};

const void* kernel_symbol(int jc, int mode);
bool config_available(int jc);
constexpr int kLeanDepthDefault = 2;
constexpr int kLeanRuns = 8;
constexpr int lean_runs(int waves) { return waves == 8 ? 32 : kLeanRuns; }
constexpr int kLeanWavesDefault = 8;
constexpr int kSchedRange = 0;
constexpr int kSchedClaim = 1;
constexpr int kSchedInterleave = 2;
constexpr int kLeanSchedDefault = kSchedInterleave;
const void* fixed_kernel_symbol(int J, bool seal, int depth, int sched, int waves);
constexpr int kRunFrames = 64;
const void* varlen8_kernel_symbol(bool seal, bool pairs);
int varlen8_waves();
const void* long8_kernel_symbol(bool seal, bool pairs);
int slots_to_pairs(const uint32_t* d_lens, uint64_t stride, uint64_t n, uint64_t* d_pairs, void* stream);
int seal_scatter(uint8_t* bytes, uint64_t stride, uint64_t frame_len, uint64_t nframes, const uint32_t* crc,
                 void* stream);
int read_stream(const uint8_t* bytes, uint64_t nbytes, uint32_t* sink, int ncu, void* stream);
constexpr int kCtrWordsPerBlock = 32;

}
```

### uflow_amd/csrc/ufc_api.cpp

```cpp
#include <hip/hip_runtime.h>

#include <algorithm>
#include <atomic>
#include <cstdio>
#include <cstdlib>
#include <cstring>
#include <mutex>
#include <new>
#include <vector>

#include "../../include/uflow_frame_codec.h"
#include "../../include/uflow_frame_crc.h"
#include "crc_math.hpp"
#include "frame_build.hpp"
#include "frame_crc_kernels.hpp"
#include "frame_pack.hpp"
#include "frame_parse.hpp"
#include "frame_queue.hpp"
#include "frame_window.hpp"
#include "flush_ctl.hpp"
#include "packet_emit.hpp"
#include "packet_receive.hpp"
#include "resend.hpp"
#include "route.hpp"
#include "send_rate.hpp"
#include "ufc_internal.hpp"

struct ufc_ctx {
  int device = -1;
  int ncu = 0;
  uint32_t* d_chain = nullptr;
  uint32_t* d_nib = nullptr;
  uint32_t* d_chain128 = nullptr;
  uint32_t* d_nib32 = nullptr;
  uint32_t G = 0;
  int last_hip_error = 0;
  std::atomic<int> stalled_comms{0};
  uint8_t* d_stage = nullptr;
  size_t d_stage_cap = 0;
  uint64_t* d_off = nullptr;
  size_t d_off_cap = 0;
  uint32_t* d_crc = nullptr;
  uint8_t* d_valid = nullptr;
  size_t d_out_cap = 0;
  uint64_t* h_off_pinned = nullptr;
  hipStream_t streams[2] = {nullptr, nullptr};
  uint32_t* d_ctr = nullptr;
  std::atomic<uint32_t> ctr_seq{0};
  int opt[UFC_OPT_COUNT_] = {};
  struct Scratch {
    int kind;
    hipStream_t stream;
    void* p;
    size_t cap;
  };
  std::mutex scratch_mu;
  std::vector<Scratch> scratch;
};

constexpr uint32_t kCtrSlots = 64;

namespace {

enum ScratchKind {
  kScratchParse = 0,
  kScratchAsyncSlots = 2,
  kScratchSealCrc = 3,
  kScratchDeferList = 4,
  kScratchDeferCounts = 5,
  kScratchBuild = 6,
  kScratchPack = 7,
  kScratchEmit = 8,
  kScratchReceive = 9,
  kScratchWindow = 10,
  kScratchFlushAcks = 11,
  kScratchFlushSync = 12,
  kScratchRoute = 13
};

hipError_t stream_scratch(ufc_ctx* ctx, int kind, hipStream_t stream, size_t need, void** out, bool* fresh = nullptr) {
  if (fresh) *fresh = false;
  std::lock_guard<std::mutex> lk(ctx->scratch_mu);
  ufc_ctx::Scratch* sc = nullptr;
  for (auto& x : ctx->scratch)
    if (x.kind == kind && x.stream == stream) sc = &x;
  if (!sc) {
    ctx->scratch.push_back({kind, stream, nullptr, 0});
    sc = &ctx->scratch.back();
  }
  if (sc->cap < need) {
    hipError_t e;
    if (sc->p) {
      if ((e = hipStreamSynchronize(stream)) != hipSuccess) return e;
      (void)hipFree(sc->p);
      sc->p = nullptr;
      sc->cap = 0;
    }
    if ((e = hipMalloc(&sc->p, need)) != hipSuccess) return e;
    sc->cap = need;
    if (fresh) *fresh = true;
  }
  *out = sc->p;
  return hipSuccess;
}

struct DeviceGuard {
  int prev = -1;
  explicit DeviceGuard(int dev) {
    if (hipGetDevice(&prev) != hipSuccess) prev = -1;
    if (prev != dev) (void)hipSetDevice(dev);
  }
  ~DeviceGuard() {
    int cur = -1;
    if (prev >= 0 && hipGetDevice(&cur) == hipSuccess && cur != prev) (void)hipSetDevice(prev);
  }
};

int hip_fail(ufc_ctx* ctx, hipError_t e) {
  if (ctx) ctx->last_hip_error = (int)e;
  return UFC_ERR_HIP;
}

struct Config {
  int jc;
};

int launch(ufc_ctx* ctx, Config cfg, int mode, ufc_dev::KernelParams& kp, hipStream_t stream) {
  const void* fn = ufc_dev::kernel_symbol(cfg.jc, mode);
  if (!fn) return UFC_ERR_INVALID_ARG;
  const uint64_t nsets = (kp.nframes + 3) / 4;
  const uint64_t nruns = (nsets + 15) / 16;
  const uint64_t waves_per_block = ufc_dev::kBlockThreads / 64;
  uint64_t blocks = (nruns + waves_per_block - 1) / waves_per_block;
  if (blocks > (uint64_t)ctx->ncu) blocks = (uint64_t)ctx->ncu;
  if (blocks < 1) blocks = 1;
  kp.chain_tab = ctx->d_chain;
  kp.nib_img = ctx->d_nib;
  kp.G = ctx->G;
  void* args[] = {&kp};
  hipError_t e = hipLaunchKernel(fn, dim3((unsigned)blocks), dim3(ufc_dev::kBlockThreads), args, 0, stream);
  if (e != hipSuccess) return hip_fail(ctx, e);
  return UFC_OK;
}

int lean_fixed_blocks(const ufc_ctx* ctx, uint64_t frame_len, uint64_t stride, uint64_t n) {
  if (frame_len < 4) return 0;
  const uint64_t J = (frame_len + 4 + 255) / 256;
  if (J > 6 || stride >= (1ull << 28)) return 0;
  const uint64_t pad = 256 * J - frame_len;
  const uint64_t s_edge = (pad + 4 * stride - 1) / (4 * stride);
  if (n / 4 <= s_edge) return 0;
  if (ctx->opt[UFC_OPT_FIXED_KERNEL] == UFC_FIXED_GENERIC || ctx->opt[UFC_OPT_GENERIC_JC] != 0) return 0;
  return (int)J;
}

int launch_lean_fixed(ufc_ctx* ctx, int J, bool seal, ufc_dev::KernelParams& kp, hipStream_t stream,
                      bool front_ok = false) {
  const int depth = ufc_dev::kLeanDepthDefault, waves = ufc_dev::kLeanWavesDefault;
  const int sched = ufc_dev::kLeanSchedDefault;
  const void* fn = ufc_dev::fixed_kernel_symbol(J, seal, depth, sched, waves);
  if (!fn) return UFC_ERR_INVALID_ARG;
  kp.chain_tab = ctx->d_chain;
  kp.nib_img = ctx->d_nib;
  kp.G = ctx->G;
  const uint64_t waves_per_block = (uint64_t)waves;
  const uint64_t chunk = (uint64_t)ctx->ncu * waves_per_block * (16 * ufc_dev::lean_runs(waves) - 1) * 4;
  const uint64_t total = kp.nframes;
  for (uint64_t f0 = 0, step = 0; f0 < total; f0 += step) {
    ufc_dev::KernelParams c = kp;
    c.nframes = std::min(chunk, total - f0);
    if (total - f0 - c.nframes > 0 && total - f0 - c.nframes < 4) c.nframes -= 4;
    step = c.nframes;
    c.bytes = kp.bytes + f0 * kp.stride;
    if (kp.wbytes) c.wbytes = kp.wbytes + f0 * kp.stride;
    if (kp.crc_out) c.crc_out = kp.crc_out + f0;
    if (kp.valid_out) c.valid_out = kp.valid_out + f0;
    c.front_ok = (f0 > 0 || front_ok) ? 1u : 0u;
    const uint32_t slot = ctx->ctr_seq.fetch_add(1) % kCtrSlots;
    c.ctr = ctx->d_ctr + (size_t)slot * ctx->ncu * ufc_dev::kCtrWordsPerBlock;
    const uint64_t nsets = (c.nframes + 3) / 4;
    uint64_t blocks = (nsets + waves_per_block - 1) / waves_per_block;
    if (blocks > (uint64_t)ctx->ncu) blocks = (uint64_t)ctx->ncu;
    if (blocks < 1) blocks = 1;
    void* args[] = {&c};
    hipError_t e = hipLaunchKernel(fn, dim3((unsigned)blocks), dim3((unsigned)(waves * 64)), args, 0, stream);
    if (e != hipSuccess) return hip_fail(ctx, e);
  }
  return UFC_OK;
}


int launch_varlen8(ufc_ctx* ctx, bool seal, bool pairs, ufc_dev::KernelParams& kp, hipStream_t stream) {
  const void* fn = ufc_dev::varlen8_kernel_symbol(seal, pairs);
  const void* fn_long = ufc_dev::long8_kernel_symbol(seal, pairs);
  if (!fn || !fn_long) return UFC_ERR_INVALID_ARG;
  const int waves = ufc_dev::varlen8_waves();
  kp.chain_tab = ctx->d_chain128;
  kp.nib_img = ctx->d_nib32;
  kp.G = ctx->G;
  const uint64_t chunk = (uint64_t)1 << 29;
  const uint64_t total = kp.nframes;
  void* list = nullptr;
  void* counts = nullptr;
  bool fresh = false;
  hipError_t e;
  const uint64_t nmax = std::min(chunk, total);
  if ((e = stream_scratch(ctx, kScratchDeferList, stream, (size_t)(nmax + 64) * 4, &list)) != hipSuccess ||
      (e = stream_scratch(ctx, kScratchDeferCounts, stream, (size_t)ctx->ncu * 4, &counts, &fresh)) != hipSuccess)
    return hip_fail(ctx, e);
  if (fresh && (e = hipMemsetAsync(counts, 0, (size_t)ctx->ncu * 4, stream)) != hipSuccess) return hip_fail(ctx, e);
  for (uint64_t f0 = 0; f0 < total; f0 += chunk) {
    ufc_dev::KernelParams c = kp;
    c.nframes = std::min(chunk, total - f0);
    c.offsets = kp.offsets + (pairs ? 2 * f0 : f0);
    if (kp.crc_out) c.crc_out = kp.crc_out + f0;
    if (kp.valid_out) c.valid_out = kp.valid_out + f0;
    c.defer_list = (uint32_t*)list;
    c.defer_counts = (uint32_t*)counts;
    const uint64_t nruns = (c.nframes + 63) / 64;
    uint64_t blocks = (nruns + waves - 1) / waves;
    if (blocks > (uint64_t)ctx->ncu) blocks = (uint64_t)ctx->ncu;
    if (blocks < 1) blocks = 1;
    void* args[] = {&c};
    if ((e = hipLaunchKernel(fn, dim3((unsigned)blocks), dim3((unsigned)(waves * 64)), args, 0, stream)) != hipSuccess)
      return hip_fail(ctx, e);
    uint32_t nb = (uint32_t)blocks;
    void* args_long[] = {&c, &nb};
    if ((e = hipLaunchKernel(fn_long, dim3((unsigned)blocks), dim3((unsigned)(waves * 64)), args_long, 0, stream)) !=
        hipSuccess)
      return hip_fail(ctx, e);
  }
  return UFC_OK;
}

Config fixed_config(const ufc_ctx* ctx, uint64_t frame_len, int* freeze) {
  const uint64_t n = frame_len >= 4 ? frame_len - 4 : frame_len;
  const uint64_t J = (n + 8 + 255) / 256;
  Config c;
  const int jc = ctx->opt[UFC_OPT_GENERIC_JC];
  c.jc = ufc_dev::config_available(jc) ? jc : (J <= 6 ? (int)J : 6);
  *freeze = ((uint64_t)c.jc == J) ? 0 : ufc_dev::kModeFreeze;
  return c;
}

Config varlen_config(const ufc_ctx* ctx) {
  const int jc = ctx->opt[UFC_OPT_GENERIC_JC];
  return Config{ufc_dev::config_available(jc) ? jc : 3};
}

int launch_varlen_any(ufc_ctx* ctx, bool seal, bool pairs, ufc_dev::KernelParams& kp, hipStream_t stream) {
  if (ctx->opt[UFC_OPT_VARLEN_KERNEL] == UFC_VARLEN_GENERIC && !pairs)
    return launch(ctx, varlen_config(ctx), ufc_dev::kModeVarlen | (seal ? ufc_dev::kModeSeal : 0), kp, stream);
  return launch_varlen8(ctx, seal, pairs, kp, stream);
}

using ufc_internal::kMaxFrameLen;

hipError_t grow_staging(ufc_ctx* ctx, size_t stage_bytes, size_t off_entries, size_t out_frames) {
  hipError_t e;
  if (ctx->d_stage_cap < stage_bytes) {
    if (ctx->d_stage) (void)hipFree(ctx->d_stage);
    ctx->d_stage = nullptr;
    ctx->d_stage_cap = 0;
    if ((e = hipMalloc(&ctx->d_stage, stage_bytes)) != hipSuccess) return e;
    ctx->d_stage_cap = stage_bytes;
  }
  if (ctx->d_off_cap < off_entries) {
    if (ctx->d_off) (void)hipFree(ctx->d_off);
    if (ctx->h_off_pinned) (void)hipHostFree(ctx->h_off_pinned);
    ctx->d_off = nullptr;
    ctx->h_off_pinned = nullptr;
    ctx->d_off_cap = 0;
    if ((e = hipMalloc(&ctx->d_off, off_entries * 8)) != hipSuccess) return e;
    if ((e = hipHostMalloc(&ctx->h_off_pinned, off_entries * 8, hipHostMallocDefault)) != hipSuccess) return e;
    ctx->d_off_cap = off_entries;
  }
  if (ctx->d_out_cap < out_frames) {
    if (ctx->d_crc) (void)hipFree(ctx->d_crc);
    if (ctx->d_valid) (void)hipFree(ctx->d_valid);
    ctx->d_crc = nullptr;
    ctx->d_valid = nullptr;
    ctx->d_out_cap = 0;
    if ((e = hipMalloc(&ctx->d_crc, out_frames * 4)) != hipSuccess) return e;
    if ((e = hipMalloc(&ctx->d_valid, out_frames)) != hipSuccess) return e;
    ctx->d_out_cap = out_frames;
  }
  return hipSuccess;
}

}

hipError_t ufc_dev::ScratchSource::get(size_t bytes, char** out) const {
  return stream_scratch(ctx, kind, stream, bytes, (void**)out);
}

extern "C" {

uint32_t ufc_crc32_compute(const uint8_t* data, size_t len) {
  if (!data) return 0;
  return ufc::host_extend(0u, data, len);
}

uint32_t ufc_crc32_extend(uint32_t initial_crc, const uint8_t* data, size_t len) {
  if (!data) return initial_crc;
  return ufc::host_extend(initial_crc, data, len);
}

int ufc_frame_validate(const uint8_t* frame, size_t len) {
  if (!frame || len < 5) return 0;
  const uint32_t c = ufc::host_extend(0u, frame, len - 4);
  const uint8_t* t = frame + len - 4;
  const uint32_t rx = ((uint32_t)t[0] << 24) | ((uint32_t)t[1] << 16) | ((uint32_t)t[2] << 8) | (uint32_t)t[3];
  return c == rx ? 1 : 0;
}

int ufc_frame_seal(uint8_t* frame, size_t len) {
  if (!frame || len < 4) return UFC_ERR_INVALID_ARG;
  const uint32_t c = ufc::host_extend(0u, frame, len - 4);
  uint8_t* t = frame + len - 4;
  t[0] = (uint8_t)(c >> 24);
  t[1] = (uint8_t)(c >> 16);
  t[2] = (uint8_t)(c >> 8);
  t[3] = (uint8_t)c;
  return UFC_OK;
}

int ufc_device_count(void) {
  int n = 0;
  if (hipGetDeviceCount(&n) != hipSuccess) return 0;
  return n;
}

const char* ufc_error_string(int code) {
  switch (code) {
    case UFC_OK: return "ok";
    case UFC_ERR_INVALID_ARG: return "invalid argument";
    case UFC_ERR_NO_DEVICE: return "no usable gfx950 (MI355X) device";
    case UFC_ERR_HIP: return "HIP runtime error (see ufc_ctx_last_hip_error)";
    case UFC_ERR_NOMEM: return "out of memory";
    case UFC_ERR_COMM: return "RCCL unavailable or failed (see ufc_comm_last_error)";
    case UFC_ERR_PEER: return "another rank rejected its part of this sharded call (nothing was transferred)";
    default: return "unknown error";
  }
}

int ufc_ctx_last_hip_error(const ufc_ctx* ctx) { return ctx ? ctx->last_hip_error : 0; }

int ufc_ctx_set_option(ufc_ctx* ctx, int option, int value) {
  if (!ctx || option < 0 || option >= UFC_OPT_COUNT_) return UFC_ERR_INVALID_ARG;
  switch (option) {
    case UFC_OPT_FIXED_KERNEL:
      if (value != UFC_FIXED_AUTO && value != UFC_FIXED_GENERIC) return UFC_ERR_INVALID_ARG;
      break;
    case UFC_OPT_VARLEN_KERNEL:
      if (value != UFC_VARLEN_AUTO && value != UFC_VARLEN_GENERIC && value != UFC_VARLEN_SORTED8)
        return UFC_ERR_INVALID_ARG;
      break;
    case UFC_OPT_GENERIC_JC:
      if (value != 0 && !ufc_dev::config_available(value)) return UFC_ERR_INVALID_ARG;
      break;
    case UFC_OPT_SEAL_KERNEL:
      if (value != UFC_SEAL_INLINE && value != UFC_SEAL_TWO_PASS) return UFC_ERR_INVALID_ARG;
      break;
    default: return UFC_ERR_INVALID_ARG;
  }
  ctx->opt[option] = value;
  return UFC_OK;
}

int ufc_ctx_get_option(const ufc_ctx* ctx, int option) {
  if (!ctx || option < 0 || option >= UFC_OPT_COUNT_) return UFC_ERR_INVALID_ARG;
  return ctx->opt[option];
}

int ufc_ctx_create(ufc_ctx** out, int device) {
  if (!out) return UFC_ERR_INVALID_ARG;
  *out = nullptr;
  int ndev = 0;
  if (hipGetDeviceCount(&ndev) != hipSuccess || ndev <= 0) return UFC_ERR_NO_DEVICE;
  if (device < 0 || device >= ndev) return UFC_ERR_INVALID_ARG;
  hipDeviceProp_t prop;
  if (hipGetDeviceProperties(&prop, device) != hipSuccess) return UFC_ERR_NO_DEVICE;
  if (std::strncmp(prop.gcnArchName, "gfx950", 6) != 0) return UFC_ERR_NO_DEVICE;
  DeviceGuard g(device);
  ufc_ctx* ctx = new (std::nothrow) ufc_ctx();
  if (!ctx) return UFC_ERR_NOMEM;
  ctx->device = device;
  ctx->ncu = prop.multiProcessorCount;
  std::vector<uint32_t> chain(1024), nib(8192), chain128(1024), nib32(8192);
  ufc::build_chain_table(chain.data(), 256);
  ufc::build_nibble_image(nib.data());
  ufc::build_chain_table(chain128.data(), 128);
  ufc::build_nibble_image32(nib32.data());
  ctx->G = ufc::init_prefix_word();
  ctx->opt[UFC_OPT_SEAL_KERNEL] = UFC_SEAL_INLINE;
  hipError_t e;
  if ((e = hipMalloc(&ctx->d_chain, chain.size() * 4)) != hipSuccess ||
      (e = hipMalloc(&ctx->d_nib, nib.size() * 4)) != hipSuccess ||
      (e = hipMalloc(&ctx->d_chain128, chain128.size() * 4)) != hipSuccess ||
      (e = hipMalloc(&ctx->d_nib32, nib32.size() * 4)) != hipSuccess ||
      (e = hipMemcpy(ctx->d_chain, chain.data(), chain.size() * 4, hipMemcpyHostToDevice)) != hipSuccess ||
      (e = hipMemcpy(ctx->d_nib, nib.data(), nib.size() * 4, hipMemcpyHostToDevice)) != hipSuccess ||
      (e = hipMemcpy(ctx->d_chain128, chain128.data(), chain128.size() * 4, hipMemcpyHostToDevice)) != hipSuccess ||
      (e = hipMemcpy(ctx->d_nib32, nib32.data(), nib32.size() * 4, hipMemcpyHostToDevice)) != hipSuccess ||
      (e = hipMalloc(&ctx->d_ctr, (size_t)kCtrSlots * ctx->ncu * ufc_dev::kCtrWordsPerBlock * 4)) != hipSuccess ||
      (e = hipMemset(ctx->d_ctr, 0, (size_t)kCtrSlots * ctx->ncu * ufc_dev::kCtrWordsPerBlock * 4)) != hipSuccess ||
      (e = hipDeviceSynchronize()) != hipSuccess) {
    ufc_ctx_destroy(ctx);
    return UFC_ERR_HIP;
  }
  *out = ctx;
  return UFC_OK;
}

int ufc_ctx_release_stream(ufc_ctx* ctx, void* stream) {
  if (!ctx) return UFC_ERR_INVALID_ARG;
  DeviceGuard g(ctx->device);
  bool any = false;
  {
    std::lock_guard<std::mutex> lk(ctx->scratch_mu);
    for (const auto& sc : ctx->scratch) any = any || sc.stream == (hipStream_t)stream;
  }
  if (!any) return UFC_OK;
  const hipError_t e = hipStreamSynchronize((hipStream_t)stream);
  if (e != hipSuccess) return hip_fail(ctx, e);
  std::vector<void*> dead;
  {
    std::lock_guard<std::mutex> lk(ctx->scratch_mu);
    for (size_t i = 0; i < ctx->scratch.size();) {
      if (ctx->scratch[i].stream != (hipStream_t)stream) {
        i++;
        continue;
      }
      if (ctx->scratch[i].p) dead.push_back(ctx->scratch[i].p);
      ctx->scratch.erase(ctx->scratch.begin() + (long)i);
    }
  }
  for (void* p : dead) (void)hipFree(p);
  return UFC_OK;
}

int ufc_ctx_destroy(ufc_ctx* ctx) {
  if (!ctx) return UFC_OK;
  if (ctx->stalled_comms.load() > 0) {
    delete ctx;
    return UFC_ERR_COMM;
  }
  {
    DeviceGuard g(ctx->device >= 0 ? ctx->device : 0);
    if (ctx->d_chain) (void)hipFree(ctx->d_chain);
    if (ctx->d_nib) (void)hipFree(ctx->d_nib);
    if (ctx->d_chain128) (void)hipFree(ctx->d_chain128);
    if (ctx->d_nib32) (void)hipFree(ctx->d_nib32);
    if (ctx->d_ctr) (void)hipFree(ctx->d_ctr);
    for (auto& sc : ctx->scratch)
      if (sc.p) (void)hipFree(sc.p);
    if (ctx->d_stage) (void)hipFree(ctx->d_stage);
    if (ctx->d_off) (void)hipFree(ctx->d_off);
    if (ctx->d_crc) (void)hipFree(ctx->d_crc);
    if (ctx->d_valid) (void)hipFree(ctx->d_valid);
    if (ctx->h_off_pinned) (void)hipHostFree(ctx->h_off_pinned);
    for (hipStream_t& s : ctx->streams)
      if (s) (void)hipStreamDestroy(s);
  }
  delete ctx;
  return UFC_OK;
}

int ufc_hbm_read_probe(ufc_ctx* ctx, const uint8_t* d_buf, size_t bytes, uint32_t* d_sink, size_t* bytes_read,
                       void* stream) {
  if (!ctx || !d_sink || (bytes >= 1024 && !d_buf)) return UFC_ERR_INVALID_ARG;
  if (bytes_read) *bytes_read = bytes / 1024 * 1024;
  DeviceGuard g(ctx->device);
  const hipError_t e = (hipError_t)ufc_dev::read_stream(d_buf, bytes, d_sink, ctx->ncu, stream);
  return e == hipSuccess ? UFC_OK : hip_fail(ctx, e);
}

int ufc_crc_batch_fixed(ufc_ctx* ctx, const uint8_t* d_frames, size_t stride, size_t frame_len, size_t n,
                        uint32_t* d_crc_out, uint8_t* d_valid_out, void* stream) {
  return ufc_internal::crc_fixed(ctx, d_frames, stride, frame_len, n, d_crc_out, d_valid_out, (hipStream_t)stream,
                                 false);
}

}

int ufc_internal::ctx_device(const ufc_ctx* ctx) { return ctx ? ctx->device : -1; }

void ufc_internal::note_hip_error(ufc_ctx* ctx, int e) {
  if (ctx) ctx->last_hip_error = e;
}

void ufc_internal::note_stall(ufc_ctx* ctx) {
  if (ctx) ctx->stalled_comms.fetch_add(1);
}

int ufc_internal::crc_fixed(ufc_ctx* ctx, const uint8_t* d_frames, size_t stride, size_t frame_len, size_t n,
                            uint32_t* d_crc_out, uint8_t* d_valid_out, hipStream_t stream, bool front_ok) {
  if (!ctx) return UFC_ERR_INVALID_ARG;
  if (n == 0) return UFC_OK;
  if (!d_frames || stride < frame_len || frame_len > kMaxFrameLen || (!d_crc_out && !d_valid_out))
    return UFC_ERR_INVALID_ARG;
  int freeze;
  const Config cfg = fixed_config(ctx, frame_len, &freeze);
  int lean = lean_fixed_blocks(ctx, frame_len, stride, n);
  ufc_dev::KernelParams kp{};
  kp.bytes = d_frames;
  kp.stride = stride;
  kp.frame_len = frame_len;
  kp.nframes = n;
  kp.crc_out = d_crc_out;
  kp.valid_out = d_valid_out;
  DeviceGuard g(ctx->device);
  if (lean) return launch_lean_fixed(ctx, lean, false, kp, stream, front_ok);
  return launch(ctx, cfg, freeze, kp, stream);
}

extern "C" {

int ufc_crc_batch_varlen(ufc_ctx* ctx, const uint8_t* d_bytes, const uint64_t* d_offsets, size_t n,
                         uint32_t* d_crc_out, uint8_t* d_valid_out, void* stream) {
  if (!ctx) return UFC_ERR_INVALID_ARG;
  if (n == 0) return UFC_OK;
  if (!d_bytes || !d_offsets || (!d_crc_out && !d_valid_out)) return UFC_ERR_INVALID_ARG;
  ufc_dev::KernelParams kp{};
  kp.bytes = d_bytes;
  kp.offsets = d_offsets;
  kp.nframes = n;
  kp.crc_out = d_crc_out;
  kp.valid_out = d_valid_out;
  DeviceGuard g(ctx->device);
  return launch_varlen_any(ctx, false, false, kp, (hipStream_t)stream);
}

int ufc_seal_batch_fixed(ufc_ctx* ctx, uint8_t* d_frames, size_t stride, size_t frame_len, size_t n,
                         uint32_t* d_crc_out, void* stream) {
  if (!ctx) return UFC_ERR_INVALID_ARG;
  if (n == 0) return UFC_OK;
  if (!d_frames || stride < frame_len || frame_len < 4 || frame_len > kMaxFrameLen) return UFC_ERR_INVALID_ARG;
  int freeze;
  const Config cfg = fixed_config(ctx, frame_len, &freeze);
  ufc_dev::KernelParams kp{};
  kp.bytes = d_frames;
  kp.wbytes = d_frames;
  kp.stride = stride;
  kp.frame_len = frame_len;
  kp.nframes = n;
  kp.crc_out = d_crc_out;
  DeviceGuard g(ctx->device);
  if (const int lean = lean_fixed_blocks(ctx, frame_len, stride, n)) {
    if (ctx->opt[UFC_OPT_SEAL_KERNEL] == UFC_SEAL_INLINE) return launch_lean_fixed(ctx, lean, true, kp, (hipStream_t)stream);
    uint32_t* crc = d_crc_out;
    hipError_t e;
    if (!crc && (e = stream_scratch(ctx, kScratchSealCrc, (hipStream_t)stream, n * 4, (void**)&crc)) != hipSuccess)
      return hip_fail(ctx, e);
    kp.wbytes = nullptr;
    kp.crc_out = crc;
    if (const int r = launch_lean_fixed(ctx, lean, false, kp, (hipStream_t)stream)) return r;
    if ((e = (hipError_t)ufc_dev::seal_scatter(d_frames, stride, frame_len, n, crc, stream)) != hipSuccess)
      return hip_fail(ctx, e);
    return UFC_OK;
  }
  return launch(ctx, cfg, freeze | ufc_dev::kModeSeal, kp, (hipStream_t)stream);
}

int ufc_seal_batch_varlen(ufc_ctx* ctx, uint8_t* d_bytes, const uint64_t* d_offsets, size_t n,
                          uint32_t* d_crc_out, void* stream) {
  if (!ctx) return UFC_ERR_INVALID_ARG;
  if (n == 0) return UFC_OK;
  if (!d_bytes || !d_offsets) return UFC_ERR_INVALID_ARG;
  ufc_dev::KernelParams kp{};
  kp.bytes = d_bytes;
  kp.wbytes = d_bytes;
  kp.offsets = d_offsets;
  kp.nframes = n;
  kp.crc_out = d_crc_out;
  DeviceGuard g(ctx->device);
  return launch_varlen_any(ctx, true, false, kp, (hipStream_t)stream);
}

static int validate_host_varlen_impl(ufc_ctx* ctx, const uint8_t* h_bytes, const uint64_t* h_offsets, size_t n,
                                     uint32_t* h_crc_out, uint8_t* h_valid_out) {
  if (!ctx) return UFC_ERR_INVALID_ARG;
  if (n == 0) return UFC_OK;
  if (!h_bytes || !h_offsets || (!h_crc_out && !h_valid_out)) return UFC_ERR_INVALID_ARG;
  for (size_t i = 0; i < n; i++)
    if (h_offsets[i + 1] < h_offsets[i]) return UFC_ERR_INVALID_ARG;
  DeviceGuard g(ctx->device);
  hipError_t e;
  for (hipStream_t& s : ctx->streams)
    if (!s && (e = hipStreamCreateWithFlags(&s, hipStreamNonBlocking)) != hipSuccess) return hip_fail(ctx, e);
  const size_t kChunkBytes = (size_t)64 << 20;
  const size_t kChunkFrames = (size_t)1 << 20;
  const uint64_t base = h_offsets[0];
  const uint64_t total = h_offsets[n] - base;
  size_t max_chunk_bytes = 0, max_chunk_frames = 0;
  std::vector<size_t> cuts;
  cuts.push_back(0);
  while (cuts.back() < n) {
    size_t a = cuts.back(), b = a + 1;
    while (b < n && b - a < kChunkFrames && h_offsets[b + 1] - h_offsets[a] <= kChunkBytes) b++;
    const size_t cb = (size_t)(h_offsets[b] - h_offsets[a]);
    if (cb > max_chunk_bytes) max_chunk_bytes = cb;
    if (b - a > max_chunk_frames) max_chunk_frames = b - a;
    cuts.push_back(b);
  }
  (void)total;
  if ((e = grow_staging(ctx, 2 * max_chunk_bytes + 64, 2 * (max_chunk_frames + 1), 2 * max_chunk_frames)) != hipSuccess)
    return hip_fail(ctx, e);
  for (size_t k = 0; k + 1 < cuts.size(); k++) {
    const int slot = (int)(k & 1);
    hipStream_t s = ctx->streams[slot];
    const size_t a = cuts[k], b = cuts[k + 1], nf = b - a;
    const uint64_t off0 = h_offsets[a];
    const size_t bytes = (size_t)(h_offsets[b] - off0);
    uint8_t* dst = ctx->d_stage + (size_t)slot * (max_chunk_bytes + 32);
    uint64_t* hoff = ctx->h_off_pinned + (size_t)slot * (max_chunk_frames + 1);
    uint64_t* doff = ctx->d_off + (size_t)slot * (max_chunk_frames + 1);
    uint32_t* dcrc = ctx->d_crc + (size_t)slot * max_chunk_frames;
    uint8_t* dval = ctx->d_valid + (size_t)slot * max_chunk_frames;
    if (k >= 2 && (e = hipStreamSynchronize(s)) != hipSuccess) return hip_fail(ctx, e);
    for (size_t i = 0; i <= nf; i++) hoff[i] = h_offsets[a + i] - off0;
    if (bytes && (e = hipMemcpyAsync(dst, h_bytes + off0, bytes, hipMemcpyHostToDevice, s)) != hipSuccess)
      return hip_fail(ctx, e);
    if ((e = hipMemcpyAsync(doff, hoff, (nf + 1) * 8, hipMemcpyHostToDevice, s)) != hipSuccess) return hip_fail(ctx, e);
    ufc_dev::KernelParams kp{};
    kp.bytes = dst;
    kp.offsets = doff;
    kp.nframes = nf;
    kp.crc_out = dcrc;
    kp.valid_out = dval;
    int rc = launch_varlen_any(ctx, false, false, kp, s);
    if (rc != UFC_OK) return rc;
    if (h_crc_out && (e = hipMemcpyAsync(h_crc_out + a, dcrc, nf * 4, hipMemcpyDeviceToHost, s)) != hipSuccess)
      return hip_fail(ctx, e);
    if (h_valid_out && (e = hipMemcpyAsync(h_valid_out + a, dval, nf, hipMemcpyDeviceToHost, s)) != hipSuccess)
      return hip_fail(ctx, e);
  }
  for (hipStream_t s : ctx->streams)
    if ((e = hipStreamSynchronize(s)) != hipSuccess) return hip_fail(ctx, e);
  return UFC_OK;
}

int ufc_crc_batch_pairs(ufc_ctx* ctx, const uint8_t* d_bytes, size_t bytes_len, const uint64_t* d_pairs, size_t n,
                        uint32_t* d_crc_out, uint8_t* d_valid_out, void* stream) {
  if (!ctx) return UFC_ERR_INVALID_ARG;
  if (n == 0) return UFC_OK;
  if (!d_bytes || !d_pairs || (!d_crc_out && !d_valid_out)) return UFC_ERR_INVALID_ARG;
  ufc_dev::KernelParams kp{};
  kp.bytes = d_bytes;
  kp.offsets = d_pairs;
  kp.frame_len = bytes_len;
  kp.nframes = n;
  kp.crc_out = d_crc_out;
  kp.valid_out = d_valid_out;
  DeviceGuard g(ctx->device);
  return launch_varlen_any(ctx, false, true, kp, (hipStream_t)stream);
}

static int validate_host_slots_impl(ufc_ctx* ctx, const uint8_t* h_slots, size_t slot_stride, const uint32_t* h_lens,
                                    size_t n, uint32_t* h_crc_out, uint8_t* h_valid_out) {
  if (!ctx) return UFC_ERR_INVALID_ARG;
  if (n == 0) return UFC_OK;
  if (!h_slots || !h_lens || slot_stride == 0 || (!h_crc_out && !h_valid_out)) return UFC_ERR_INVALID_ARG;
  for (size_t i = 0; i < n; i++)
    if (h_lens[i] > slot_stride) return UFC_ERR_INVALID_ARG;
  DeviceGuard g(ctx->device);
  hipError_t e;
  for (hipStream_t& s : ctx->streams)
    if (!s && (e = hipStreamCreateWithFlags(&s, hipStreamNonBlocking)) != hipSuccess) return hip_fail(ctx, e);
  const size_t per = std::max<size_t>(1, std::min<size_t>((size_t)1 << 20, ((size_t)64 << 20) / slot_stride));
  const size_t cf = std::min(per, n);
  const size_t cb = cf * slot_stride;
  if ((e = grow_staging(ctx, 2 * cb + 64, 4 * cf, 2 * cf)) != hipSuccess) return hip_fail(ctx, e);
  size_t k = 0;
  for (size_t a = 0; a < n; a += cf, k++) {
    const int slot = (int)(k & 1);
    hipStream_t s = ctx->streams[slot];
    const size_t nf = std::min(cf, n - a);
    uint8_t* dst = ctx->d_stage + (size_t)slot * (cb + 32);
    uint64_t* hp = ctx->h_off_pinned + (size_t)slot * 2 * cf;
    uint64_t* dp = ctx->d_off + (size_t)slot * 2 * cf;
    if (k >= 2 && (e = hipStreamSynchronize(s)) != hipSuccess) return hip_fail(ctx, e);
    for (size_t i = 0; i < nf; i++) {
      hp[2 * i] = (uint64_t)i * slot_stride;
      hp[2 * i + 1] = (uint64_t)i * slot_stride + h_lens[a + i];
    }
    const size_t bytes = (nf - 1) * slot_stride + h_lens[a + nf - 1];
    if (bytes && (e = hipMemcpyAsync(dst, h_slots + a * slot_stride, bytes, hipMemcpyHostToDevice, s)) != hipSuccess)
      return hip_fail(ctx, e);
    if ((e = hipMemcpyAsync(dp, hp, nf * 16, hipMemcpyHostToDevice, s)) != hipSuccess) return hip_fail(ctx, e);
    uint32_t* dcrc = ctx->d_crc + (size_t)slot * cf;
    uint8_t* dval = ctx->d_valid + (size_t)slot * cf;
    int rc = ufc_crc_batch_pairs(ctx, dst, bytes, dp, nf, dcrc, dval, s);
    if (rc != UFC_OK) return rc;
    if (h_crc_out && (e = hipMemcpyAsync(h_crc_out + a, dcrc, nf * 4, hipMemcpyDeviceToHost, s)) != hipSuccess)
      return hip_fail(ctx, e);
    if (h_valid_out && (e = hipMemcpyAsync(h_valid_out + a, dval, nf, hipMemcpyDeviceToHost, s)) != hipSuccess)
      return hip_fail(ctx, e);
  }
  for (hipStream_t s : ctx->streams)
    if ((e = hipStreamSynchronize(s)) != hipSuccess) return hip_fail(ctx, e);
  return UFC_OK;
}

static int validate_host_slots_async_impl(ufc_ctx* ctx, const uint8_t* h_slots, size_t slot_stride,
                                          const uint32_t* h_lens, size_t n, uint32_t* h_crc_out, uint8_t* h_valid_out,
                                          hipStream_t stream) {
  if (!ctx || !stream) return UFC_ERR_INVALID_ARG;
  if (n == 0) return UFC_OK;
  if (!h_slots || !h_lens || slot_stride == 0 || (!h_crc_out && !h_valid_out)) return UFC_ERR_INVALID_ARG;
  if (n > (((size_t)1 << 31) - ((size_t)1 << 20)) / slot_stride) return UFC_ERR_INVALID_ARG;
  for (size_t i = 0; i < n; i++)
    if (h_lens[i] > slot_stride) return UFC_ERR_INVALID_ARG;
  const size_t bytes = (n - 1) * slot_stride + h_lens[n - 1];
  ufc_dev::ScratchPlan plan;
  plan.take(bytes + 64);
  const size_t o_lens = plan.take(4 * n), o_pairs = plan.take(16 * n), o_crc = plan.take(4 * n), o_valid = plan.take(n);
  void* sp = nullptr;
  hipError_t e;
  if ((e = stream_scratch(ctx, kScratchAsyncSlots, stream, plan.end, &sp)) != hipSuccess) return hip_fail(ctx, e);
  uint8_t* s = (uint8_t*)sp;
  uint32_t* d_lens = (uint32_t*)(s + o_lens);
  uint64_t* d_pairs = (uint64_t*)(s + o_pairs);
  uint32_t* d_crc = (uint32_t*)(s + o_crc);
  uint8_t* d_valid = s + o_valid;
  if ((e = hipMemcpyAsync(s, h_slots, bytes, hipMemcpyHostToDevice, stream)) != hipSuccess ||
      (e = hipMemcpyAsync(d_lens, h_lens, 4 * n, hipMemcpyHostToDevice, stream)) != hipSuccess)
    return hip_fail(ctx, e);
  if ((e = (hipError_t)ufc_dev::slots_to_pairs(d_lens, slot_stride, n, d_pairs, stream)) != hipSuccess)
    return hip_fail(ctx, e);
  const int rc = ufc_crc_batch_pairs(ctx, s, bytes, d_pairs, n, d_crc, d_valid, stream);
  if (rc != UFC_OK) return rc;
  if (h_crc_out && (e = hipMemcpyAsync(h_crc_out, d_crc, 4 * n, hipMemcpyDeviceToHost, stream)) != hipSuccess)
    return hip_fail(ctx, e);
  if (h_valid_out && (e = hipMemcpyAsync(h_valid_out, d_valid, n, hipMemcpyDeviceToHost, stream)) != hipSuccess)
    return hip_fail(ctx, e);
  return UFC_OK;
}

static int drain_on_error(ufc_ctx* ctx, int rc) {
  if (rc != UFC_OK && ctx)
    for (hipStream_t s : ctx->streams)
      if (s) (void)hipStreamSynchronize(s);
  return rc;
}

int ufc_validate_host_varlen(ufc_ctx* ctx, const uint8_t* h_bytes, const uint64_t* h_offsets, size_t n,
                             uint32_t* h_crc_out, uint8_t* h_valid_out) {
  DeviceGuard g(ctx ? ctx->device : 0);
  return drain_on_error(ctx, validate_host_varlen_impl(ctx, h_bytes, h_offsets, n, h_crc_out, h_valid_out));
}

int ufc_validate_host_slots(ufc_ctx* ctx, const uint8_t* h_slots, size_t slot_stride, const uint32_t* h_lens,
                            size_t n, uint32_t* h_crc_out, uint8_t* h_valid_out) {
  DeviceGuard g(ctx ? ctx->device : 0);
  return drain_on_error(ctx, validate_host_slots_impl(ctx, h_slots, slot_stride, h_lens, n, h_crc_out, h_valid_out));
}

int ufc_validate_host_slots_async(ufc_ctx* ctx, const uint8_t* h_slots, size_t slot_stride, const uint32_t* h_lens,
                                  size_t n, uint32_t* h_crc_out, uint8_t* h_valid_out, void* stream) {
  DeviceGuard g(ctx ? ctx->device : 0);
  const int rc = validate_host_slots_async_impl(ctx, h_slots, slot_stride, h_lens, n, h_crc_out, h_valid_out,
                                                (hipStream_t)stream);
  if (rc != UFC_OK && ctx && stream) (void)hipStreamSynchronize((hipStream_t)stream);
  return rc;
}

namespace {
void put_trailer(uint8_t* f, size_t len, uint32_t crc) {
  uint8_t* t = f + len - 4;
  t[0] = (uint8_t)(crc >> 24);
  t[1] = (uint8_t)(crc >> 16);
  t[2] = (uint8_t)(crc >> 8);
  t[3] = (uint8_t)crc;
}
}

int ufc_seal_host_slots(ufc_ctx* ctx, uint8_t* h_slots, size_t slot_stride, const uint32_t* h_lens, size_t n,
                        uint32_t* h_crc_scratch) {
  if (!ctx) return UFC_ERR_INVALID_ARG;
  if (n == 0) return UFC_OK;
  if (!h_slots || !h_lens || !h_crc_scratch) return UFC_ERR_INVALID_ARG;
  for (size_t i = 0; i < n; i++)
    if (h_lens[i] < 4) return UFC_ERR_INVALID_ARG;
  const int rc = ufc_validate_host_slots(ctx, h_slots, slot_stride, h_lens, n, h_crc_scratch, nullptr);
  if (rc != UFC_OK) return rc;
  for (size_t i = 0; i < n; i++) put_trailer(h_slots + i * slot_stride, h_lens[i], h_crc_scratch[i]);
  return UFC_OK;
}

int ufc_seal_host_varlen(ufc_ctx* ctx, uint8_t* h_bytes, const uint64_t* h_offsets, size_t n,
                         uint32_t* h_crc_scratch) {
  if (!ctx) return UFC_ERR_INVALID_ARG;
  if (n == 0) return UFC_OK;
  if (!h_bytes || !h_offsets || !h_crc_scratch) return UFC_ERR_INVALID_ARG;
  for (size_t i = 0; i < n; i++)
    if (h_offsets[i + 1] < h_offsets[i] + 4) return UFC_ERR_INVALID_ARG;
  const int rc = ufc_validate_host_varlen(ctx, h_bytes, h_offsets, n, h_crc_scratch, nullptr);
  if (rc != UFC_OK) return rc;
  for (size_t i = 0; i < n; i++) put_trailer(h_bytes + h_offsets[i], (size_t)(h_offsets[i + 1] - h_offsets[i]), h_crc_scratch[i]);
  return UFC_OK;
}

int ufc_parse_batch_varlen(ufc_ctx* ctx, const uint8_t* d_bytes, const uint64_t* d_offsets, size_t n,
                           const uint8_t* d_valid, ufc_frame_info* d_infos, ufc_item* d_items, size_t items_cap,
                           uint64_t* d_items_used, void* stream) {
  if (!ctx) return UFC_ERR_INVALID_ARG;
  if (n == 0) return UFC_OK;
  if (!d_bytes || !d_offsets || !d_valid || !d_infos || n >= ((size_t)1 << 31)) return UFC_ERR_INVALID_ARG;
  DeviceGuard g(ctx->device);
  hipError_t e;
  ufc_dev::ParseArgs a{d_bytes, d_offsets, (uint64_t)n, d_valid, d_infos, d_items, (uint64_t)(d_items ? items_cap : 0),
                       d_items_used};
  if ((e = ufc_dev::parse_batch(a, {ctx, kScratchParse, (hipStream_t)stream}, (hipStream_t)stream)) != hipSuccess)
    return hip_fail(ctx, e);
  return UFC_OK;
}

namespace {
bool build_args_ok(const ufc_frame_info* d_infos, const ufc_item* d_items, size_t n_items, size_t n,
                   const uint64_t* d_out_offsets) {
  return d_infos && d_out_offsets && (d_items || n_items == 0) && n < ((size_t)1 << 31) - 1 &&
         n_items < ((size_t)1 << 31) - 1;
}
}

int ufc_build_sizes_varlen(ufc_ctx* ctx, const ufc_frame_info* d_infos, const ufc_item* d_items, size_t n_items,
                           const uint64_t* d_src_base, size_t payload_len, size_t n, uint64_t* d_out_offsets,
                           uint8_t* d_status, void* stream) {
  if (!ctx) return UFC_ERR_INVALID_ARG;
  if (n == 0) return UFC_OK;
  if (!build_args_ok(d_infos, d_items, n_items, n, d_out_offsets)) return UFC_ERR_INVALID_ARG;
  DeviceGuard g(ctx->device);
  hipError_t e;
  ufc_dev::BuildArgs a{d_infos, d_items, (uint64_t)n_items, d_src_base, nullptr, (uint64_t)payload_len, (uint64_t)n,
                       d_out_offsets, d_status, nullptr, 0};
  if ((e = ufc_dev::build_sizes(a, {ctx, kScratchBuild, (hipStream_t)stream}, (hipStream_t)stream)) != hipSuccess)
    return hip_fail(ctx, e);
  return UFC_OK;
}

int ufc_build_batch_varlen(ufc_ctx* ctx, const ufc_frame_info* d_infos, const ufc_item* d_items, size_t n_items,
                           const uint64_t* d_src_base, const uint8_t* d_payload, size_t payload_len, size_t n,
                           const uint64_t* d_out_offsets, uint8_t* d_out_bytes, size_t out_len, int seal,
                           uint32_t* d_crc_out, void* stream) {
  if (!ctx) return UFC_ERR_INVALID_ARG;
  if (n == 0) return UFC_OK;
  if (!build_args_ok(d_infos, d_items, n_items, n, d_out_offsets) || (!d_payload && payload_len) ||
      (!d_out_bytes && out_len))
    return UFC_ERR_INVALID_ARG;
  DeviceGuard g(ctx->device);
  hipError_t e;
  ufc_dev::BuildArgs a{d_infos, d_items, (uint64_t)n_items, d_src_base, d_payload, (uint64_t)payload_len, (uint64_t)n,
                       const_cast<uint64_t*>(d_out_offsets), nullptr, d_out_bytes, (uint64_t)out_len};
  if ((e = ufc_dev::build_write(a, {ctx, kScratchBuild, (hipStream_t)stream}, (hipStream_t)stream)) != hipSuccess)
    return hip_fail(ctx, e);
  if (!seal || !d_out_bytes) return UFC_OK;
  ufc_dev::KernelParams kp{};
  kp.bytes = d_out_bytes;
  kp.wbytes = d_out_bytes;
  kp.offsets = d_out_offsets;
  kp.nframes = n;
  kp.crc_out = d_crc_out;
  return launch_varlen_any(ctx, true, false, kp, (hipStream_t)stream);
}

int ufc_pack_varlen(ufc_ctx* ctx, const ufc_item* d_items, size_t n_items, const uint64_t* d_flush_first,
                    const ufc_flush* d_flushes, size_t n_flushes, const uint32_t* d_nonce_bits,
                    ufc_frame_info* d_infos, size_t frames_cap, ufc_flush_result* d_results,
                    uint64_t* d_frames_used, void* stream) {
  if (!ctx) return UFC_ERR_INVALID_ARG;
  if (n_flushes == 0) return UFC_OK;
  if (!d_flush_first || !d_flushes || !d_results || !d_frames_used || (!d_items && n_items) ||
      (!d_infos && frames_cap) || n_flushes >= ((size_t)1 << 31) - 1 || n_items >= ((size_t)1 << 31) - 1)
    return UFC_ERR_INVALID_ARG;
  DeviceGuard g(ctx->device);
  hipError_t e;
  ufc_dev::PackArgs a{d_items, (uint64_t)n_items, d_flush_first, d_flushes, (uint64_t)n_flushes, d_nonce_bits,
                      d_infos, (uint64_t)frames_cap, d_results, d_frames_used};
  if ((e = ufc_dev::pack_batch(a, {ctx, kScratchPack, (hipStream_t)stream}, (hipStream_t)stream)) != hipSuccess)
    return hip_fail(ctx, e);
  return UFC_OK;
}


int ufc_emit_packets_varlen(ufc_ctx* ctx, const ufc_packet* d_packets, size_t n_packets,
                            const uint64_t* d_packet_first, const ufc_sender* d_senders, size_t n_senders,
                            ufc_item* d_items, size_t items_cap, uint64_t* d_flush_first,
                            ufc_packet_result* d_packet_results, ufc_sender_result* d_sender_results,
                            ufc_sender* d_senders_out, uint64_t* d_items_used, void* stream) {
  if (!ctx) return UFC_ERR_INVALID_ARG;
  if (n_senders == 0) return UFC_OK;
  if (!d_packet_first || !d_senders || !d_flush_first || !d_sender_results || !d_items_used ||
      (!d_packets && n_packets) || (!d_items && items_cap) || n_senders >= ((size_t)1 << 31) - 1 ||
      n_packets >= ((size_t)1 << 31) - 1)
    return UFC_ERR_INVALID_ARG;
  DeviceGuard g(ctx->device);
  hipError_t e;
  ufc_dev::EmitArgs a{d_packets, (uint64_t)n_packets, d_packet_first, d_senders, (uint64_t)n_senders, d_items,
                      (uint64_t)items_cap, d_flush_first, d_packet_results, d_sender_results, d_senders_out,
                      d_items_used};
  if ((e = ufc_dev::emit_batch(a, {ctx, kScratchEmit, (hipStream_t)stream}, (hipStream_t)stream)) != hipSuccess)
    return hip_fail(ctx, e);
  return UFC_OK;
}

int ufc_receive_packets_varlen(ufc_ctx* ctx, const ufc_frame_info* d_infos, size_t n_frames,
                               const uint8_t* d_frame_accept, const ufc_item* d_items, size_t n_items,
                               const uint64_t* d_src_base, const uint8_t* d_payload, size_t payload_len,
                               const uint64_t* d_frame_first, const ufc_receiver* d_receivers, size_t n_receivers,
                               ufc_rx_slot* d_slots, const uint64_t* d_slot_first, size_t n_slots,
                               const uint8_t* d_carry_in, size_t carry_in_len, uint8_t* d_carry_out, size_t carry_cap,
                               uint64_t* d_carry_first, uint64_t* d_carry_used, ufc_rx_packet* d_packets,
                               size_t packets_cap, uint64_t* d_packet_first, uint64_t* d_packets_used,
                               uint8_t* d_out_bytes, size_t out_cap, uint64_t* d_out_used, uint8_t* d_item_status,
                               ufc_receiver_result* d_results, ufc_receiver* d_receivers_out, void* stream) {
  if (!ctx) return UFC_ERR_INVALID_ARG;
  if (n_receivers == 0) return UFC_OK;
  const ufc_codec::RxArgs a{d_infos, n_frames, d_frame_accept, d_items, n_items, d_src_base, d_payload, payload_len,
                            d_frame_first, d_receivers, n_receivers, d_slots, d_slot_first, n_slots, d_carry_in,
                            carry_in_len, d_carry_out, carry_cap, d_carry_first, d_carry_used, d_packets, packets_cap,
                            d_packet_first, d_packets_used, d_out_bytes, out_cap, d_out_used, d_item_status, d_results,
                            d_receivers_out};
  if (!ufc_codec::rx_args_ok(a) || n_slots >= ufc_codec::kCountLim / 2) return UFC_ERR_INVALID_ARG;
  DeviceGuard g(ctx->device);
  hipError_t e;
  if ((e = ufc_dev::receive_batch(a, {ctx, kScratchReceive, (hipStream_t)stream}, (hipStream_t)stream)) != hipSuccess)
    return hip_fail(ctx, e);
  return UFC_OK;
}

int ufc_frame_window_varlen(ufc_ctx* ctx, const ufc_frame_info* d_infos, size_t n_frames, const uint64_t* d_frame_first,
                            const ufc_frame_window* d_windows, size_t n_windows, uint8_t* d_frame_accept,
                            ufc_item* d_groups, size_t groups_cap, uint64_t* d_group_first, uint64_t* d_groups_used,
                            ufc_frame_window_result* d_results, ufc_frame_window* d_windows_out, void* stream) {
  if (!ctx) return UFC_ERR_INVALID_ARG;
  if (n_windows == 0) return UFC_OK;
  const ufc_codec::FwArgs a{d_infos, n_frames, d_frame_first, d_windows, n_windows, d_frame_accept, d_groups,
                            groups_cap, d_group_first, d_groups_used, d_results, d_windows_out};
  if (!ufc_codec::fw_args_ok(a)) return UFC_ERR_INVALID_ARG;
  DeviceGuard g(ctx->device);
  hipError_t e;
  if ((e = ufc_dev::window_batch(a, {ctx, kScratchWindow, (hipStream_t)stream}, (hipStream_t)stream)) != hipSuccess)
    return hip_fail(ctx, e);
  return UFC_OK;
}

int ufc_frame_queue_varlen(ufc_ctx* ctx, const ufc_frame_info* d_infos, size_t n_frames, const ufc_item* d_items,
                           size_t n_items, const uint64_t* d_frame_first, const ufc_sent_frame* d_sent, size_t n_sent,
                           const uint64_t* d_sent_first, const ufc_frame_queue* d_queues,
                           const ufc_frame_queue_step* d_steps, size_t n_queues, ufc_sent_frame* d_log, size_t n_log,
                           uint8_t* d_ref_acked, size_t refs_cap, ufc_frame_queue_result* d_results,
                           ufc_frame_queue* d_queues_out, void* stream) {
  if (!ctx) return UFC_ERR_INVALID_ARG;
  if (n_queues == 0) return UFC_OK;
  const ufc_codec::FqArgs a{d_infos, n_frames, d_items, n_items, d_frame_first, d_sent, n_sent, d_sent_first, d_queues,
                            d_steps, n_queues, d_log, n_log, d_ref_acked, refs_cap, d_results, d_queues_out};
  if (!ufc_codec::fq_args_ok(a)) return UFC_ERR_INVALID_ARG;
  DeviceGuard g(ctx->device);
  hipError_t e;
  if ((e = ufc_dev::queue_batch(a, (hipStream_t)stream)) != hipSuccess) return hip_fail(ctx, e);
  return UFC_OK;
}

int ufc_rate_begin_varlen(ufc_ctx* ctx, const ufc_rate_state* d_states, const uint64_t* d_now_ms,
                          const uint32_t* d_extra_flags, size_t n, ufc_frame_queue_step* d_steps,
                          ufc_rate_state* d_states_out, void* stream) {
  if (!ctx) return UFC_ERR_INVALID_ARG;
  if (n == 0) return UFC_OK;
  const ufc_codec::RateBeginArgs a{d_states, d_now_ms, d_extra_flags, n, d_steps, d_states_out};
  if (!ufc_codec::rate_begin_args_ok(a)) return UFC_ERR_INVALID_ARG;
  DeviceGuard g(ctx->device);
  hipError_t e;
  if ((e = ufc_dev::rate_begin_batch(a, (hipStream_t)stream)) != hipSuccess) return hip_fail(ctx, e);
  return UFC_OK;
}

int ufc_rate_step_varlen(ufc_ctx* ctx, const ufc_rate_state* d_states, const ufc_rate_tick* d_ticks,
                         const ufc_frame_queue_result* d_fq, size_t n, ufc_recv_rate_entry* d_entries, size_t n_entries,
                         const ufc_flush_result* d_flush_results, size_t n_flush_results, const uint32_t* d_result_index,
                         ufc_flush* d_flushes, size_t n_flushes, const uint32_t* d_flush_index,
                         ufc_rate_result* d_results, ufc_rate_state* d_states_out, void* stream) {
  if (!ctx) return UFC_ERR_INVALID_ARG;
  if (n == 0) return UFC_OK;
  const ufc_codec::RateArgs a{d_states, d_ticks, d_fq, n, d_entries, n_entries, d_flush_results, n_flush_results,
                              d_result_index, d_flushes, n_flushes, d_flush_index, d_results, d_states_out};
  if (!ufc_codec::rate_args_ok(a)) return UFC_ERR_INVALID_ARG;
  DeviceGuard g(ctx->device);
  hipError_t e;
  if ((e = ufc_dev::rate_step_batch(a, (hipStream_t)stream)) != hipSuccess) return hip_fail(ctx, e);
  return UFC_OK;
}

int ufc_resend_begin_varlen(ufc_ctx* ctx, const ufc_frame_info* d_infos, size_t n_frames, const uint64_t* d_frame_first,
                            const ufc_frame_queue* d_queues, const ufc_sent_frame* d_log, size_t n_log,
                            const ufc_rate_result* d_rate, const uint32_t* d_flags, const ufc_flush* d_flushes,
                            const ufc_resend* d_states, const ufc_sender* d_senders, size_t n, ufc_resend_entry* d_heap,
                            size_t n_heap, const ufc_sent_packet* d_pkts, size_t n_pkts, uint8_t* d_frag_acked,
                            size_t n_frag, const ufc_tx_ref* d_tx, size_t n_tx, uint8_t* d_ref_acked, size_t refs_cap,
                            ufc_item* d_stage, size_t n_stage, ufc_resend_result* d_results, ufc_resend* d_states_out,
                            ufc_sender* d_senders_out, void* stream) {
  if (!ctx) return UFC_ERR_INVALID_ARG;
  if (n == 0) return UFC_OK;
  const ufc_codec::RsBeginArgs a{d_infos, n_frames, d_frame_first, d_queues, d_log, n_log, d_rate, d_flags, d_flushes,
                                 d_states, d_senders, n, d_heap, n_heap, d_pkts, n_pkts, d_frag_acked, n_frag, d_tx, n_tx,
                                 d_ref_acked, refs_cap, d_stage, n_stage, d_results, d_states_out, d_senders_out};
  if (!ufc_codec::rs_begin_args_ok(a)) return UFC_ERR_INVALID_ARG;
  DeviceGuard g(ctx->device);
  hipError_t e;
  if ((e = ufc_dev::resend_begin_batch(a, (hipStream_t)stream)) != hipSuccess) return hip_fail(ctx, e);
  return UFC_OK;
}

int ufc_resend_place_varlen(ufc_ctx* ctx, const ufc_resend* d_states, const ufc_resend_result* d_begin_results, size_t n,
                            const ufc_item* d_stage, size_t n_stage, const uint64_t* d_flush_first, ufc_item* d_items,
                            size_t items_cap, void* stream) {
  if (!ctx) return UFC_ERR_INVALID_ARG;
  if (n == 0) return UFC_OK;
  const ufc_codec::RsPlaceArgs a{d_states, d_begin_results, n, d_stage, n_stage, d_flush_first, d_items, items_cap};
  if (!ufc_codec::rs_place_args_ok(a)) return UFC_ERR_INVALID_ARG;
  DeviceGuard g(ctx->device);
  hipError_t e;
  if ((e = ufc_dev::resend_place_batch(a, (hipStream_t)stream)) != hipSuccess) return hip_fail(ctx, e);
  return UFC_OK;
}

int ufc_resend_commit_varlen(ufc_ctx* ctx, const ufc_flush_result* d_flush_results, const ufc_frame_info* d_infos,
                             size_t n_infos, const uint64_t* d_out_offsets, const uint64_t* d_frames_used,
                             const ufc_item* d_items, size_t n_items, const uint64_t* d_flush_first,
                             const ufc_packet* d_packets, size_t n_packets, const uint64_t* d_packet_first,
                             const ufc_packet_result* d_packet_results, const ufc_sender_result* d_sender_results,
                             const ufc_resend_result* d_begin_results, const ufc_rate_result* d_rate,
                             const ufc_resend* d_states, const ufc_sender* d_senders, size_t n, ufc_resend_entry* d_heap,
                             size_t n_heap, ufc_sent_packet* d_pkts, size_t n_pkts, uint8_t* d_frag_acked, size_t n_frag,
                             ufc_tx_ref* d_tx, size_t n_tx, ufc_sent_frame* d_sent, size_t sent_cap,
                             uint64_t* d_sent_first, uint32_t* d_next_extra_flags, ufc_resend_commit_result* d_results,
                             ufc_resend* d_states_out, ufc_sender* d_retake, void* stream) {
  if (!ctx) return UFC_ERR_INVALID_ARG;
  if (n == 0) return UFC_OK;
  const ufc_codec::RsCommitArgs a{d_flush_results, d_infos, n_infos, d_out_offsets, d_frames_used, d_items, n_items,
                                  d_flush_first, d_packets, n_packets, d_packet_first, d_packet_results,
                                  d_sender_results, d_begin_results, d_rate, d_states, d_senders, n, d_heap, n_heap,
                                  d_pkts, n_pkts, d_frag_acked, n_frag, d_tx, n_tx, d_sent, sent_cap, d_sent_first,
                                  d_next_extra_flags, d_results, d_states_out, d_retake};
  if (!ufc_codec::rs_commit_args_ok(a)) return UFC_ERR_INVALID_ARG;
  DeviceGuard g(ctx->device);
  hipError_t e;
  if ((e = ufc_dev::resend_commit_batch(a, (hipStream_t)stream)) != hipSuccess) return hip_fail(ctx, e);
  return UFC_OK;
}

int ufc_flush_acks_varlen(ufc_ctx* ctx, const ufc_flush_ctl* d_ctl, const ufc_frame_window* d_windows,
                          const ufc_item* d_groups, size_t n_groups, const uint64_t* d_group_first,
                          const ufc_receiver* d_receivers, const ufc_rate_result* d_rate, size_t n, ufc_item* d_carry,
                          size_t n_carry, ufc_item* d_merged, size_t merged_cap, uint64_t* d_merged_first,
                          uint64_t* d_merged_used, ufc_frame_info* d_infos, size_t frames_cap, uint64_t* d_frames_used,
                          ufc_flush_result* d_results, ufc_flush_acks_result* d_ack_results,
                          ufc_frame_window* d_windows_out, ufc_flush_ctl* d_ctl_out, ufc_flush* d_flushes,
                          uint32_t* d_flags, void* stream) {
  if (!ctx) return UFC_ERR_INVALID_ARG;
  if (n == 0) return UFC_OK;
  const ufc_codec::FaArgs a{d_ctl, d_windows, d_groups, n_groups, d_group_first, d_receivers, d_rate, n, d_carry, n_carry,
                            d_merged, merged_cap, d_merged_first, d_merged_used, d_infos, frames_cap, d_frames_used,
                            d_results, d_ack_results, d_windows_out, d_ctl_out, d_flushes, d_flags};
  if (!ufc_codec::fa_args_ok(a)) return UFC_ERR_INVALID_ARG;
  DeviceGuard g(ctx->device);
  hipError_t e;
  if ((e = ufc_dev::flush_acks_batch(a, {ctx, kScratchFlushAcks, (hipStream_t)stream}, (hipStream_t)stream)) != hipSuccess)
    return hip_fail(ctx, e);
  return UFC_OK;
}

int ufc_flush_sync_varlen(ufc_ctx* ctx, const ufc_flush_ctl* d_ctl, const ufc_rate_result* d_rate,
                          const ufc_flush_result* d_ack_results, const ufc_resend_result* d_begin_results,
                          const ufc_flush_result* d_pack_results, const ufc_resend_commit_result* d_commit_results,
                          const ufc_frame_queue* d_queues, const ufc_sender* d_senders, size_t n,
                          ufc_frame_info* d_infos, size_t syncs_cap, uint32_t* d_sync_index, uint64_t* d_syncs_used,
                          ufc_flush_sync_result* d_results, ufc_flush_ctl* d_ctl_out, ufc_rate_tick* d_ticks_next,
                          void* stream) {
  if (!ctx) return UFC_ERR_INVALID_ARG;
  if (n == 0) return UFC_OK;
  const ufc_codec::FsArgs a{d_ctl, d_rate, d_ack_results, d_begin_results, d_pack_results, d_commit_results, d_queues,
                            d_senders, n, d_infos, syncs_cap, d_sync_index, d_syncs_used, d_results, d_ctl_out,
                            d_ticks_next};
  if (!ufc_codec::fs_args_ok(a)) return UFC_ERR_INVALID_ARG;
  DeviceGuard g(ctx->device);
  hipError_t e;
  if ((e = ufc_dev::flush_sync_batch(a, {ctx, kScratchFlushSync, (hipStream_t)stream}, (hipStream_t)stream)) != hipSuccess)
    return hip_fail(ctx, e);
  return UFC_OK;
}

int ufc_route_frames_varlen(ufc_ctx* ctx, const ufc_frame_info* d_infos, const ufc_addr* d_addrs,
                            const uint64_t* d_offsets, size_t n, const ufc_route_slot* d_slots, size_t n_slots,
                            uint32_t seed, uint32_t max_probe, size_t n_conns, const uint8_t* d_conn_active,
                            uint64_t now_ms, uint64_t active_timeout_ms, const uint64_t* d_timeout_in,
                            uint32_t* d_route, uint8_t* d_cls, uint64_t* d_bucket_first, uint32_t* d_order,
                            ufc_frame_info* d_infos_out, uint64_t* d_src_base_out, ufc_route_result* d_results,
                            uint64_t* d_timeout_out, uint32_t* d_first_unknown_control, void* stream) {
  if (!ctx) return UFC_ERR_INVALID_ARG;
  const ufc_codec::RtArgs a{d_infos, d_addrs, d_offsets, n, d_slots, n_slots, seed, max_probe, n_conns, d_conn_active,
                            now_ms, active_timeout_ms, d_timeout_in, d_route, d_cls, d_bucket_first, d_order,
                            d_infos_out, d_src_base_out, d_results, d_timeout_out, d_first_unknown_control};
  if (!ufc_codec::rt_args_ok(a)) return UFC_ERR_INVALID_ARG;
  DeviceGuard g(ctx->device);
  hipError_t e;
  if ((e = ufc_dev::route_frames_batch(a, {ctx, kScratchRoute, (hipStream_t)stream}, (hipStream_t)stream)) != hipSuccess)
    return hip_fail(ctx, e);
  return UFC_OK;
}

}
```

Measured before the change: 6253.

## Process fixed-frame chunk rounds inside one persistent kernel launch

The host loop used to issue one kernel launch per chunk of frames. Now, for static schedules, a single launch loops over all rounds on the device. Each round reloads the kernel arguments, restages the LDS tables and recomputes per-round offsets, with a workgroup barrier between rounds. This is meant to remove launch overhead and the drain/refill gaps between launches, at the cost of extra per-round setup work and register pressure inside the kernel.

```diff
diff --git a/include/uflow_fixed_rounds.h b/include/uflow_fixed_rounds.h
--- /dev/null
+++ b/include/uflow_fixed_rounds.h
@@ -0,0 +1,16 @@
+#ifndef UFLOW_FIXED_ROUNDS_H
+#define UFLOW_FIXED_ROUNDS_H
+
+#include <stdint.h>
+
+#ifdef __cplusplus
+extern "C" {
+#endif
+
+int ufc_fixed_round(uint64_t n, int ncu, int round_sets, uint64_t round, uint64_t* first, uint64_t* count);
+
+#ifdef __cplusplus
+}
+#endif
+
+#endif
diff --git a/include/uflow_frame_crc.h b/include/uflow_frame_crc.h
--- a/include/uflow_frame_crc.h
+++ b/include/uflow_frame_crc.h
@@ -50,7 +50,11 @@
 #define UFC_OPT_SEAL_KERNEL 3
 #define UFC_SEAL_INLINE 0
 #define UFC_SEAL_TWO_PASS 1
-#define UFC_OPT_COUNT_ 4
+#define UFC_OPT_FIXED_ROUNDS 4
+#define UFC_FIXED_ROUNDS_KERNEL 0
+#define UFC_FIXED_ROUNDS_LAUNCHES 1
+#define UFC_OPT_FIXED_ROUND_SETS 5
+#define UFC_OPT_COUNT_ 6
 int ufc_ctx_set_option(ufc_ctx* ctx, int option, int value);
 int ufc_ctx_get_option(const ufc_ctx* ctx, int option);
 
diff --git a/uflow_amd/_build.py b/uflow_amd/_build.py
--- a/uflow_amd/_build.py
+++ b/uflow_amd/_build.py
@@ -58,7 +58,8 @@
     sources = list(SOURCES)
     deps = [os.path.join(CSRC, s) for s in sources + HEADERS]
     deps += [os.path.join(REPO_DIR, "include", h)
-             for h in ("uflow_frame_crc.h", "uflow_frame_codec.h", "uflow_flush_ctl.h", "uflow_route.h")]
+             for h in ("uflow_frame_crc.h", "uflow_frame_codec.h", "uflow_flush_ctl.h", "uflow_route.h",
+                       "uflow_fixed_rounds.h")]
     flags = [HIPCC, "-O3", "--offload-arch=gfx950", "-fPIC", "-std=c++17", "-Wall",
              "-mllvm", "-amdgpu-atomic-optimizer-strategy=None"]
     flags += ["-D" + d for d in defines]
diff --git a/uflow_amd/_native.py b/uflow_amd/_native.py
--- a/uflow_amd/_native.py
+++ b/uflow_amd/_native.py
@@ -21,6 +21,8 @@
 UFC_VARLEN_AUTO, UFC_VARLEN_GENERIC, UFC_VARLEN_SORTED, UFC_VARLEN_BLOCKED8, UFC_VARLEN_CLAIM16 = 0, 1, 2, 3, 4
 UFC_VARLEN_BLOCKSTREAM, UFC_VARLEN_SORTED8, UFC_VARLEN_STREAM = 5, 6, 7
 UFC_OPT_SEAL_KERNEL, UFC_SEAL_INLINE, UFC_SEAL_TWO_PASS = 3, 0, 1
+UFC_OPT_FIXED_ROUNDS, UFC_FIXED_ROUNDS_KERNEL, UFC_FIXED_ROUNDS_LAUNCHES = 4, 0, 1
+UFC_OPT_FIXED_ROUND_SETS = 5
 UFC_BUILD_OK, UFC_BUILD_SKIPPED, UFC_BUILD_BAD_FIELD, UFC_BUILD_BAD_SRC = 0, 1, 2, 3
 UFC_PACK_DONE, UFC_PACK_SIZE_LIMITED, UFC_PACK_WINDOW_LIMITED, UFC_PACK_BAD_RANGE = 0, 1, 2, 3
 UFC_SEND_TIME_SENSITIVE, UFC_SEND_UNRELIABLE, UFC_SEND_PERSISTENT, UFC_SEND_RELIABLE = 0, 1, 2, 3
@@ -185,6 +187,11 @@
     "ufc_route_frames_varlen": (_I, [_V] + _ROUTE_ARGS + [_V]),
 }
 ROUTE_SYMBOLS = tuple(_ROUTE_SIGNATURES)
+_ROUNDS_SIGNATURES = {
+    "ufc_fixed_round": (ctypes.c_int, [ctypes.c_uint64, ctypes.c_int, ctypes.c_int, ctypes.c_uint64,
+                                       ctypes.POINTER(ctypes.c_uint64), ctypes.POINTER(ctypes.c_uint64)]),
+}
+ROUNDS_SYMBOLS = tuple(_ROUNDS_SIGNATURES)
 
 
 class FrameInfo(ctypes.Structure):
@@ -233,7 +240,7 @@
                               "(the native library is required; there is no CPU fallback)")
         l = ctypes.CDLL(LIB_PATH)
         for name, (res, args) in (list(_SIGNATURES.items()) + list(_FLUSH_SIGNATURES.items()) +
-                                   list(_ROUTE_SIGNATURES.items())):
+                                   list(_ROUTE_SIGNATURES.items()) + list(_ROUNDS_SIGNATURES.items())):
             fn = getattr(l, name)
             fn.restype = res
             fn.argtypes = args
diff --git a/uflow_amd/csrc/frame_crc.hip b/uflow_amd/csrc/frame_crc.hip
--- a/uflow_amd/csrc/frame_crc.hip
+++ b/uflow_amd/csrc/frame_crc.hip
@@ -299,46 +299,96 @@
 [[maybe_unused]] constexpr int kLoadvAllNT = lean_loadv(0, kFixAuxNT, kFixAuxNT, kFixAuxNT);
 constexpr int kLoadvProduct = lean_loadv(0, 0, kFixAuxNT, kFixAuxNT);
 template <int J, bool SEAL, int DEPTH, int SCHED, int WAVES, int LOADV = kLoadvProduct>
-__global__ __launch_bounds__(WAVES * 64) void frame_crc_fixed_kernel(const KernelParams p) {
+__global__ __launch_bounds__(WAVES * 64) void frame_crc_fixed_kernel(const KernelParams args) {
   static_assert(DEPTH >= 1 && DEPTH <= 3, "pipeline depth (4 spills at J = 6)");
   static_assert(DEPTH != 1 || SCHED != kSchedClaim, "depth 1: static schedules only");
   constexpr bool DYN = SCHED == kSchedClaim;
   constexpr bool ILV = SCHED == kSchedInterleave;
   constexpr uint32_t kInc = ILV ? (uint32_t)WAVES : 1u;
   __shared__ __attribute__((aligned(16))) char lds[kLdsBytes];
-  const StageSet<WAVES * 64> sr = stage_load<WAVES * 64>(p);
+  uint32_t tid = threadIdx.x;
+  KernelParams p;
+  uint32_t grid;
+  StageSet<WAVES * 64> sr;
   Lane L;
-  init_lane(L, lds, p.G);
-
-  const uint64_t stride = p.stride;
-  const uint32_t len = (uint32_t)p.frame_len;
-  const uint32_t n = len - 4u;
-  const int pad = J * 256 - (int)len;
-  const uint32_t nsets = (uint32_t)((p.nframes + 3) >> 2);
-  const uint32_t nfull = (uint32_t)(p.nframes >> 2);
-  const bool tail = (p.nframes & 3) != 0;
+  uint64_t stride;
+  uint32_t len, n;
+  int pad;
+  uint32_t nrounds;
+  (void)args;
+  auto begin_args = [&]() {
+    typedef const __attribute__((address_space(4))) KernelParams* KernargPtr;
+    KernargPtr a = (KernargPtr)__builtin_amdgcn_kernarg_segment_ptr();
+    asm volatile("" : "+s"(a));
+    p.bytes = a->bytes;
+    p.wbytes = a->wbytes;
+    p.stride = a->stride;
+    p.frame_len = a->frame_len;
+    p.nframes = a->nframes;
+    p.crc_out = a->crc_out;
+    p.valid_out = a->valid_out;
+    p.chain_tab = a->chain_tab;
+    p.nib_img = a->nib_img;
+    p.G = a->G;
+    p.ctr = a->ctr;
+    p.front_ok = a->front_ok;
+    p.nrounds = a->nrounds;
+    p.round_frames = a->round_frames;
+    grid = gridDim.x;
+    asm volatile("" : "+s"(grid));
+    stride = p.stride;
+    len = (uint32_t)p.frame_len;
+    n = len - 4u;
+    pad = J * 256 - (int)len;
+    nrounds = DYN ? 1u : p.nrounds;
+  };
   const uint32_t wpb = WAVES;
-  const uint32_t wid = __builtin_amdgcn_readfirstlane(threadIdx.x >> 6);
-  const uint32_t w = blockIdx.x * wpb + wid;
-  const uint32_t s_edge =
-      p.front_ok ? 0u : (uint32_t)min(((uint64_t)pad + 4 * stride - 1) / (4 * stride), (uint64_t)nsets);
-  const bool edge0 = s_edge == 1 && (p.nframes - 1) * stride + len >= 16;
-  const uint32_t s_fast = edge0 ? 0u : s_edge;
-  const uint32_t nfast = nfull - s_fast;
+  uint32_t wid, w;
+  struct RoundView {
+    const uint8_t* bytes;
+    uint8_t* wbytes;
+    uint32_t* crc_out;
+    uint8_t* valid_out;
+    uint64_t nframes;
+  } rb;
+  uint32_t nfull;
+  bool tail;
+  bool edge0;
+  uint32_t s_fast, nfast;
   uint32_t q_lo, q_end, q_cur, q_nx1, q_nx2;
-  if (DYN || ILV) {
-    q_lo = s_fast + (uint32_t)((uint64_t)nfast * blockIdx.x / gridDim.x);
-    q_end = s_fast + (uint32_t)((uint64_t)nfast * (blockIdx.x + 1) / gridDim.x);
-    q_cur = q_lo + wid;
-    q_nx1 = q_lo + wpb + wid;
-  } else {
-    const uint32_t NW = gridDim.x * wpb;
-    q_lo = s_fast + (uint32_t)((uint64_t)nfast * w / NW);
-    q_end = s_fast + (uint32_t)((uint64_t)nfast * (w + 1) / NW);
-    q_cur = q_lo;
-    q_nx1 = q_lo + 1;
-  }
-  uint32_t* ctr = DYN ? p.ctr + blockIdx.x * kCtrWordsPerBlock : nullptr;
+  uint32_t t = 0, nhist = 0;
+  auto begin_round = [&](uint32_t r) {
+    uint64_t f0 = 0, cnt = p.nframes;
+    if (nrounds > 1) fixed_round(p.nframes, p.round_frames, nrounds, r, &f0, &cnt);
+    rb.bytes = p.bytes + f0 * stride;
+    rb.wbytes = SEAL ? p.wbytes + f0 * stride : nullptr;
+    rb.crc_out = p.crc_out ? p.crc_out + f0 : nullptr;
+    rb.valid_out = (!SEAL && p.valid_out) ? p.valid_out + f0 : nullptr;
+    rb.nframes = cnt;
+    const uint32_t nsets = (uint32_t)((cnt + 3) >> 2);
+    nfull = (uint32_t)(cnt >> 2);
+    tail = (cnt & 3) != 0;
+    const uint32_t s_edge = (r > 0 || p.front_ok)
+                                ? 0u
+                                : (uint32_t)min(((uint64_t)pad + 4 * stride - 1) / (4 * stride), (uint64_t)nsets);
+    edge0 = s_edge == 1 && (cnt - 1) * stride + len >= 16;
+    s_fast = edge0 ? 0u : s_edge;
+    nfast = nfull - s_fast;
+    if (DYN || ILV) {
+      q_lo = s_fast + (uint32_t)((uint64_t)nfast * blockIdx.x / grid);
+      q_end = s_fast + (uint32_t)((uint64_t)nfast * (blockIdx.x + 1) / grid);
+      q_cur = q_lo + wid;
+      q_nx1 = q_lo + wpb + wid;
+    } else {
+      const uint32_t NW = grid * wpb;
+      q_lo = s_fast + (uint32_t)((uint64_t)nfast * w / NW);
+      q_end = s_fast + (uint32_t)((uint64_t)nfast * (w + 1) / NW);
+      q_cur = q_lo;
+      q_nx1 = q_lo + 1;
+    }
+    t = nhist = 0;
+  };
+  uint32_t* ctr = DYN ? args.ctr + blockIdx.x * kCtrWordsPerBlock : nullptr;
   auto claim_issue = [&]() -> uint32_t {
     uint32_t v = 0;
     if (L.lane == 0) v = __hip_atomic_fetch_add(ctr, 1u, __ATOMIC_RELAXED, __HIP_MEMORY_SCOPE_AGENT);
@@ -348,33 +398,41 @@
     return q_lo + (DEPTH - 1) * wpb + __builtin_amdgcn_readfirstlane(v);
   };
 
-  const int64_t lane_off = (int64_t)L.grp * (int64_t)stride + 16 * L.col - pad;
-  uint32_t dm[4], pre[4];
-#pragma unroll
-  for (int b = 0; b < 4; b++) {
-    const int o = 16 * L.col + 4 * b - pad;
-    const uint32_t fz = fix_word(0u, o, L.G);
-    const uint32_t f1 = fix_word(0xFFFFFFFFu, o, L.G);
-    dm[b] = f1 & ~fz;
-    pre[b] = fz;
-  }
-  uint32_t dm1, pre1;
-  {
-    const int o = 256 + 16 * L.col - pad;
-    const uint32_t fz = fix_word(0u, o, L.G), f1 = fix_word(0xFFFFFFFFu, o, L.G);
-    dm1 = f1 & ~fz;
-    pre1 = fz;
-  }
-  const uint32_t tmask = (L.col == 15) ? 0u : 0xFFFFFFFFu;
+  int64_t lane_off;
+  uint32_t dm[4], pre[4], dm1, pre1;
+  uint32_t tmask;
+  uint32_t voff, voff_b0;
+  auto begin_lane = [&]() {
+    init_lane(L, lds, p.G, tid);
+    wid = __builtin_amdgcn_readfirstlane(tid >> 6);
+    w = blockIdx.x * wpb + wid;
+    lane_off = (int64_t)L.grp * (int64_t)stride + 16 * L.col - pad;
+#pragma unroll
+    for (int b = 0; b < 4; b++) {
+      const int o = 16 * L.col + 4 * b - pad;
+      const uint32_t fz = fix_word(0u, o, L.G);
+      const uint32_t f1 = fix_word(0xFFFFFFFFu, o, L.G);
+      dm[b] = f1 & ~fz;
+      pre[b] = fz;
+    }
+    {
+      const int o = 256 + 16 * L.col - pad;
+      const uint32_t fz = fix_word(0u, o, L.G), f1 = fix_word(0xFFFFFFFFu, o, L.G);
+      dm1 = f1 & ~fz;
+      pre1 = fz;
+    }
+    tmask = (L.col == 15) ? 0u : 0xFFFFFFFFu;
+    voff = (uint32_t)(lane_off + 512);
+    voff_b0 = ((LOADV & 1) && 16 * L.col + 16 <= pad - 4) ? kFixRecords : voff;
+  };
 
   constexpr int RUNS = lean_runs(WAVES);
   uint32_t acc_crc = 0, acc_qv = 0;
   uint32_t hist_crc[RUNS], hist_qv[RUNS];
 #pragma unroll
   for (int r = 0; r < RUNS; r++) hist_crc[r] = hist_qv[r] = 0;
-  uint32_t t = 0, nhist = 0;
   auto write_trailer = [&](uint64_t f, uint32_t crc) {
-    uint8_t* a = p.wbytes + f * stride + n;
+    uint8_t* a = rb.wbytes + f * stride + n;
     if (((uintptr_t)a & 3u) == 0) {
       *as_global<g_u32w>((uint32_t*)a) = __builtin_bswap32(crc);
     } else {
@@ -387,9 +445,9 @@
   };
   auto store_run = [&](int cnt, uint32_t crcs, uint32_t qv) {
     const uint64_t f = (uint64_t)(qv & 0x7FFFFFFFu) * 4 + (uint64_t)L.grp;
-    if (L.col < cnt && f < p.nframes) {
-      if (p.crc_out) *as_global<g_u32w>(p.crc_out + f) = crcs;
-      if (!SEAL && p.valid_out) *as_global<g_u8w>(p.valid_out + f) = (uint8_t)(qv >> 31);
+    if (L.col < cnt && f < rb.nframes) {
+      if (rb.crc_out) *as_global<g_u32w>(rb.crc_out + f) = crcs;
+      if (!SEAL && rb.valid_out) *as_global<g_u8w>(rb.valid_out + f) = (uint8_t)(qv >> 31);
       if (SEAL) write_trailer(f, crcs);
     }
   };
@@ -447,18 +505,17 @@
 #pragma unroll
     for (int j = 0; j < J; j++) compute_block(q, j, b.x[j], c);
   };
-  const uint32_t voff = (uint32_t)(lane_off + 512);
   auto set_base = [&](uint32_t q) -> const uint8_t* {
-    return p.bytes + (uint64_t)(q < q_end ? q : nfull - 1) * 4 * stride - 512;
+    return rb.bytes + (uint64_t)(q < q_end ? q : nfull - 1) * 4 * stride - 512;
   };
   auto load_edge0 = [&](ItemBuf<J>& b) {
-    const int64_t room = (int64_t)min(p.nframes - 1, (uint64_t)3);
+    const int64_t room = (int64_t)min(rb.nframes - 1, (uint64_t)3);
     const int64_t over = (int64_t)L.grp > room ? (int64_t)L.grp - room : 0;
     const int64_t off0 = lane_off - over * (int64_t)stride;
 #pragma unroll
     for (int j = 0; j < J; j++) {
       const int64_t off = off0 + 256 * j;
-      uint4 v = load_frame16<true>(p.bytes + (off < 0 ? 0 : off));
+      uint4 v = load_frame16<true>(rb.bytes + (off < 0 ? 0 : off));
       if (off < 0) {
         const int64_t d = -off;
         uint64_t lo = (uint64_t)v.x | ((uint64_t)v.y << 32), hi = (uint64_t)v.z | ((uint64_t)v.w << 32);
@@ -476,7 +533,6 @@
       b.x[j] = v;
     }
   };
-  const uint32_t voff_b0 = ((LOADV & 1) && 16 * L.col + 16 <= pad - 4) ? kFixRecords : voff;
   auto load = [&](uint32_t q, ItemBuf<J>& b) {
     constexpr int kAuxFirst = (LOADV >> 1) & 31, kAuxMid = (LOADV >> 6) & 31, kAuxLast = (LOADV >> 11) & 31;
     const __amdgpu_buffer_rsrc_t rs =
@@ -495,182 +551,198 @@
     }
   };
   auto load_tail = [&](ItemBuf<J>& b) {
-    const int64_t room = (int64_t)(p.nframes - 1 - 4 * (uint64_t)nfull);
+    const int64_t room = (int64_t)(rb.nframes - 1 - 4 * (uint64_t)nfull);
     const int64_t over = (int64_t)L.grp > room ? (int64_t)L.grp - room : 0;
-    load_set<J>(p.bytes + (uint64_t)nfull * 4 * stride - 512, voff - (uint32_t)(over * (int64_t)stride), b);
+    load_set<J>(rb.bytes + (uint64_t)nfull * 4 * stride - 512, voff - (uint32_t)(over * (int64_t)stride), b);
   };
 
   ItemBuf<J> A, B, C;
   uint32_t cX = 0, cY = 0, cZ = 0;
-  if (DYN) {
-    cY = claim_issue();
-    cZ = claim_issue();
-  }
-  if (edge0 && q_cur == 0)
-    load_edge0(A);
-  else
-    load(q_cur, A);
-  if (DEPTH == 3) load(q_nx1, B);
-  stage_store<WAVES * 64>(sr, lds);
-  q_nx2 = (DEPTH == 3 && !DYN) ? q_cur + 2 * kInc : 0;
-
-  if (w == 0 && s_fast > 0) {
 #pragma unroll 1
-    for (uint32_t e = 0; e < s_fast; e++) {
-      FrameDesc d = make_desc(min((uint64_t)e * 4 + (uint64_t)L.grp, p.nframes - 1) * stride, len);
-      Chains ce{0u, 0u, 0u, 0u, 0u};
+  for (uint32_t round = 0;;) {
+    asm volatile("" : "+v"(tid));
+    begin_args();
+    sr = stage_load<WAVES * 64>(p, tid);
+    begin_lane();
+    begin_round(round);
+    if (DYN) {
+      cY = claim_issue();
+      cZ = claim_issue();
+    }
+    if (edge0 && q_cur == 0)
+      load_edge0(A);
+    else
+      load(q_cur, A);
+    if (DEPTH == 3) load(q_nx1, B);
+    if (round > 0) {
+      __builtin_amdgcn_fence(__ATOMIC_RELEASE, "workgroup", "local");
+      __builtin_amdgcn_s_barrier();
+      __builtin_amdgcn_fence(__ATOMIC_ACQUIRE, "workgroup", "local");
+    }
+    stage_store<WAVES * 64>(sr, lds, tid);
+    q_nx2 = (DEPTH == 3 && !DYN) ? q_cur + 2 * kInc : 0;
+
+    if (w == 0 && s_fast > 0) {
 #pragma unroll 1
-      for (int blk = 0; blk < J; blk++) {
-        uint32_t wv[4];
-#pragma unroll
-        for (int b = 0; b < 4; b++) {
-          const int o = 256 * blk + 16 * L.col + 4 * b - d.pad;
-          uint32_t a = 0;
+      for (uint32_t e = 0; e < s_fast; e++) {
+        FrameDesc d = make_desc(min((uint64_t)e * 4 + (uint64_t)L.grp, rb.nframes - 1) * stride, len);
+        Chains ce{0u, 0u, 0u, 0u, 0u};
 #pragma unroll 1
-          for (int k = 0; k < 4; k++) {
-            const int ob = o + k;
-            if (ob >= 0 && ob < (int)d.len) a |= (uint32_t)*as_global<g_u8>(p.bytes + d.start + (uint64_t)ob) << (8 * k);
+        for (int blk = 0; blk < J; blk++) {
+          uint32_t wv[4];
+#pragma unroll
+          for (int b = 0; b < 4; b++) {
+            const int o = 256 * blk + 16 * L.col + 4 * b - d.pad;
+            uint32_t a = 0;
+#pragma unroll 1
+            for (int k = 0; k < 4; k++) {
+              const int ob = o + k;
+              if (ob >= 0 && ob < (int)d.len)
+                a |= (uint32_t)*as_global<g_u8>(rb.bytes + d.start + (uint64_t)ob) << (8 * k);
+            }
+            wv[b] = a;
           }
-          wv[b] = a;
+          process_block<false>(L, d, blk, make_uint4(wv[0], wv[1], wv[2], wv[3]), ce);
         }
-        process_block<false>(L, d, blk, make_uint4(wv[0], wv[1], wv[2], wv[3]), ce);
-      }
-      const uint32_t crc = ~group_lin(L, ce);
-      const uint32_t ok = (len >= 5u && __builtin_bswap32(ce.tr) == crc) ? 1u : 0u;
-      const uint64_t f = (uint64_t)e * 4 + (uint64_t)L.grp;
-      if (L.col == 15 && f < p.nframes) {
-        if (p.crc_out) *as_global<g_u32w>(p.crc_out + f) = crc;
-        if (!SEAL && p.valid_out) *as_global<g_u8w>(p.valid_out + f) = (uint8_t)ok;
+        const uint32_t crc = ~group_lin(L, ce);
+        const uint32_t ok = (len >= 5u && __builtin_bswap32(ce.tr) == crc) ? 1u : 0u;
+        const uint64_t f = (uint64_t)e * 4 + (uint64_t)L.grp;
+        if (L.col == 15 && f < rb.nframes) {
+          if (rb.crc_out) *as_global<g_u32w>(rb.crc_out + f) = crc;
+          if (!SEAL && rb.valid_out) *as_global<g_u8w>(rb.valid_out + f) = (uint8_t)ok;
+          if (SEAL) write_trailer(f, crc);
+        }
+      }
+      __builtin_amdgcn_s_waitcnt(0x0F70);
+    }
+
+
+    Chains c{0u, 0u, 0u, 0u, 0u};
+    auto step = [&](ItemBuf<J>& cur, ItemBuf<J>& fill, uint32_t& c_issue, uint32_t& c_read) {
+      uint32_t q_load;
+      if (DYN) {
+        q_load = claim_set(c_read);
+        c_issue = claim_issue();
+      } else {
+        q_load = (DEPTH == 3) ? q_nx2 : q_nx1;
+      }
+      load(q_load, fill);
+      __builtin_amdgcn_sched_barrier(0);
+      if (q_cur < q_end) {
+        compute(q_cur, cur, c);
+        finish(q_cur, c, DYN);
+      }
+      __builtin_amdgcn_sched_barrier(0);
+      if (DEPTH == 3) {
+        q_cur = q_nx1;
+        q_nx1 = q_load;
+        q_nx2 = q_load + kInc;
+      } else {
+        q_cur = q_load;
+        q_nx1 = q_load + kInc;
+      }
+    };
+    if (DEPTH == 1) {
+      while (q_cur < q_end) {
+        compute(q_cur, A, c);
+        finish(q_cur, c, false);
+        q_cur += kInc;
+        load(q_cur, A);
+      }
+    } else if (DEPTH == 2 && !DYN) {
+      while (q_cur < q_end) {
+        step(A, B, cX, cY);
+        step(B, A, cY, cZ);
+      }
+    } else if (DEPTH == 2) {
+      while (q_cur < q_end) {
+        step(A, B, cX, cY);
+        step(B, A, cY, cZ);
+        step(A, B, cZ, cX);
+        step(B, A, cX, cY);
+        step(A, B, cY, cZ);
+        step(B, A, cZ, cX);
+      }
+    } else {
+      while (q_cur < q_end) {
+        step(A, C, cX, cY);
+        step(B, A, cY, cZ);
+        step(C, B, cZ, cX);
+      }
+    }
+    if (tail && blockIdx.x == grid - 1 && wid == wpb - 1) {
+      ItemBuf<J> T;
+      load_tail(T);
+      compute(nfull, T, c);
+      const uint32_t crc = ~group_lin(L, c);
+      const uint32_t tr = (uint32_t)__builtin_amdgcn_update_dpp(0, (int)c.tr, 0x15F, 0xF, 0xF, false);
+      const uint32_t ok = (len >= 5u && __builtin_bswap32(tr) == crc) ? 1u : 0u;
+      const uint64_t f = (uint64_t)nfull * 4 + (uint64_t)L.grp;
+      if (L.col == 0 && f < rb.nframes) {
+        if (rb.crc_out) *as_global<g_u32w>(rb.crc_out + f) = crc;
+        if (!SEAL && rb.valid_out) *as_global<g_u8w>(rb.valid_out + f) = (uint8_t)ok;
         if (SEAL) write_trailer(f, crc);
       }
     }
+    if (DYN) {
+      store_all();
+    } else {
+      uint32_t blo = q_lo, bhi = q_end;
+      if (!ILV) {
+        const uint64_t NW = (uint64_t)grid * wpb;
+        blo = s_fast + (uint32_t)((uint64_t)nfast * (blockIdx.x * wpb) / NW);
+        bhi = s_fast + (uint32_t)((uint64_t)nfast * ((blockIdx.x + 1) * wpb) / NW);
+      }
+      const uint32_t nfr = 4 * (bhi - blo);
+      uint32_t* lcrc = (uint32_t*)lds;
+      uint8_t* lval = (uint8_t*)lds + 4 * nfr;
+      __builtin_amdgcn_fence(__ATOMIC_RELEASE, "workgroup", "local");
+      __builtin_amdgcn_s_barrier();
+      __builtin_amdgcn_fence(__ATOMIC_ACQUIRE, "workgroup", "local");
+      auto stage = [&](int cnt, uint32_t crcs, uint32_t qv) {
+        if (L.col < cnt) {
+          const uint32_t q = qv & 0x7FFFFFFFu;
+          const uint32_t pos = (q - blo) * 4 + (uint32_t)L.grp;
+          lcrc[pos] = crcs;
+          lval[pos] = (uint8_t)(qv >> 31);
+        }
+      };
+      if (t > 0) stage((int)t, acc_crc, acc_qv);
+#pragma unroll
+      for (int r = 0; r < RUNS; r++)
+        if ((uint32_t)r < nhist) stage(kSetsPerRun, hist_crc[r], hist_qv[r]);
+      __builtin_amdgcn_fence(__ATOMIC_RELEASE, "workgroup", "local");
+      __builtin_amdgcn_s_barrier();
+      __builtin_amdgcn_fence(__ATOMIC_ACQUIRE, "workgroup", "local");
+      const uint64_t f0 = (uint64_t)blo * 4;
+      if (rb.crc_out)
+        for (uint32_t i = tid; i < nfr; i += WAVES * 64) *as_global<g_u32w>(rb.crc_out + f0 + i) = lcrc[i];
+      if (SEAL) {
+        for (uint32_t i = tid; i < nfr; i += WAVES * 64) {
+          const uint32_t v = __builtin_bswap32(lcrc[i]);
+          uint8_t* a = rb.wbytes + (f0 + i) * stride + n;
+          if (((uintptr_t)a & 3u) == 0) {
+            __builtin_nontemporal_store(v, as_global<g_u32w>((uint32_t*)a));
+          } else {
+            g_u8w* wp = as_global<g_u8w>(a);
+            __builtin_nontemporal_store((uint8_t)v, wp);
+            __builtin_nontemporal_store((uint8_t)(v >> 8), wp + 1);
+            __builtin_nontemporal_store((uint8_t)(v >> 16), wp + 2);
+            __builtin_nontemporal_store((uint8_t)(v >> 24), wp + 3);
+          }
+        }
+      }
+      if (!SEAL && rb.valid_out) {
+        if ((((uintptr_t)(rb.valid_out + f0)) & 3u) == 0) {
+          for (uint32_t i = tid; i < nfr / 4; i += WAVES * 64)
+            *as_global<g_u32w>((uint32_t*)(rb.valid_out + f0) + i) = ((const uint32_t*)lval)[i];
+        } else {
+          for (uint32_t i = tid; i < nfr; i += WAVES * 64) *as_global<g_u8w>(rb.valid_out + f0 + i) = lval[i];
+        }
+      }
+    }
+    if (++round == nrounds) break;
     __builtin_amdgcn_s_waitcnt(0x0F70);
-  }
-
-
-  Chains c{0u, 0u, 0u, 0u, 0u};
-  auto step = [&](ItemBuf<J>& cur, ItemBuf<J>& fill, uint32_t& c_issue, uint32_t& c_read) {
-    uint32_t q_load;
-    if (DYN) {
-      q_load = claim_set(c_read);
-      c_issue = claim_issue();
-    } else {
-      q_load = (DEPTH == 3) ? q_nx2 : q_nx1;
-    }
-    load(q_load, fill);
-    __builtin_amdgcn_sched_barrier(0);
-    if (q_cur < q_end) {
-      compute(q_cur, cur, c);
-      finish(q_cur, c, DYN);
-    }
-    __builtin_amdgcn_sched_barrier(0);
-    if (DEPTH == 3) {
-      q_cur = q_nx1;
-      q_nx1 = q_load;
-      q_nx2 = q_load + kInc;
-    } else {
-      q_cur = q_load;
-      q_nx1 = q_load + kInc;
-    }
-  };
-  if (DEPTH == 1) {
-    while (q_cur < q_end) {
-      compute(q_cur, A, c);
-      finish(q_cur, c, false);
-      q_cur += kInc;
-      load(q_cur, A);
-    }
-  } else if (DEPTH == 2 && !DYN) {
-    while (q_cur < q_end) {
-      step(A, B, cX, cY);
-      step(B, A, cY, cZ);
-    }
-  } else if (DEPTH == 2) {
-    while (q_cur < q_end) {
-      step(A, B, cX, cY);
-      step(B, A, cY, cZ);
-      step(A, B, cZ, cX);
-      step(B, A, cX, cY);
-      step(A, B, cY, cZ);
-      step(B, A, cZ, cX);
-    }
-  } else {
-    while (q_cur < q_end) {
-      step(A, C, cX, cY);
-      step(B, A, cY, cZ);
-      step(C, B, cZ, cX);
-    }
-  }
-  if (tail && blockIdx.x == gridDim.x - 1 && wid == wpb - 1) {
-    ItemBuf<J> T;
-    load_tail(T);
-    compute(nfull, T, c);
-    const uint32_t crc = ~group_lin(L, c);
-    const uint32_t tr = (uint32_t)__builtin_amdgcn_update_dpp(0, (int)c.tr, 0x15F, 0xF, 0xF, false);
-    const uint32_t ok = (len >= 5u && __builtin_bswap32(tr) == crc) ? 1u : 0u;
-    const uint64_t f = (uint64_t)nfull * 4 + (uint64_t)L.grp;
-    if (L.col == 0 && f < p.nframes) {
-      if (p.crc_out) *as_global<g_u32w>(p.crc_out + f) = crc;
-      if (!SEAL && p.valid_out) *as_global<g_u8w>(p.valid_out + f) = (uint8_t)ok;
-      if (SEAL) write_trailer(f, crc);
-    }
-  }
-  if (DYN) {
-    store_all();
-  } else {
-    uint32_t blo = q_lo, bhi = q_end;
-    if (!ILV) {
-      const uint64_t NW = (uint64_t)gridDim.x * wpb;
-      blo = s_fast + (uint32_t)((uint64_t)nfast * (blockIdx.x * wpb) / NW);
-      bhi = s_fast + (uint32_t)((uint64_t)nfast * ((blockIdx.x + 1) * wpb) / NW);
-    }
-    const uint32_t nfr = 4 * (bhi - blo);
-    uint32_t* lcrc = (uint32_t*)lds;
-    uint8_t* lval = (uint8_t*)lds + 4 * nfr;
-    __builtin_amdgcn_fence(__ATOMIC_RELEASE, "workgroup", "local");
-    __builtin_amdgcn_s_barrier();
-    __builtin_amdgcn_fence(__ATOMIC_ACQUIRE, "workgroup", "local");
-    auto stage = [&](int cnt, uint32_t crcs, uint32_t qv) {
-      if (L.col < cnt) {
-        const uint32_t q = qv & 0x7FFFFFFFu;
-        const uint32_t pos = (q - blo) * 4 + (uint32_t)L.grp;
-        lcrc[pos] = crcs;
-        lval[pos] = (uint8_t)(qv >> 31);
-      }
-    };
-    if (t > 0) stage((int)t, acc_crc, acc_qv);
-#pragma unroll
-    for (int r = 0; r < RUNS; r++)
-      if ((uint32_t)r < nhist) stage(kSetsPerRun, hist_crc[r], hist_qv[r]);
-    __builtin_amdgcn_fence(__ATOMIC_RELEASE, "workgroup", "local");
-    __builtin_amdgcn_s_barrier();
-    __builtin_amdgcn_fence(__ATOMIC_ACQUIRE, "workgroup", "local");
-    const uint64_t f0 = (uint64_t)blo * 4;
-    if (p.crc_out)
-      for (uint32_t i = threadIdx.x; i < nfr; i += WAVES * 64) *as_global<g_u32w>(p.crc_out + f0 + i) = lcrc[i];
-    if (SEAL) {
-      for (uint32_t i = threadIdx.x; i < nfr; i += WAVES * 64) {
-        const uint32_t v = __builtin_bswap32(lcrc[i]);
-        uint8_t* a = p.wbytes + (f0 + i) * stride + n;
-        if (((uintptr_t)a & 3u) == 0) {
-          __builtin_nontemporal_store(v, as_global<g_u32w>((uint32_t*)a));
-        } else {
-          g_u8w* wp = as_global<g_u8w>(a);
-          __builtin_nontemporal_store((uint8_t)v, wp);
-          __builtin_nontemporal_store((uint8_t)(v >> 8), wp + 1);
-          __builtin_nontemporal_store((uint8_t)(v >> 16), wp + 2);
-          __builtin_nontemporal_store((uint8_t)(v >> 24), wp + 3);
-        }
-      }
-    }
-    if (!SEAL && p.valid_out) {
-      if ((((uintptr_t)(p.valid_out + f0)) & 3u) == 0) {
-        for (uint32_t i = threadIdx.x; i < nfr / 4; i += WAVES * 64)
-          *as_global<g_u32w>((uint32_t*)(p.valid_out + f0) + i) = ((const uint32_t*)lval)[i];
-      } else {
-        for (uint32_t i = threadIdx.x; i < nfr; i += WAVES * 64) *as_global<g_u8w>(p.valid_out + f0 + i) = lval[i];
-      }
-    }
   }
 
   if (DYN) {
diff --git a/uflow_amd/csrc/frame_crc_dev.hpp b/uflow_amd/csrc/frame_crc_dev.hpp
--- a/uflow_amd/csrc/frame_crc_dev.hpp
+++ b/uflow_amd/csrc/frame_crc_dev.hpp
@@ -227,9 +227,9 @@
   __syncthreads();
 }
 
-__device__ __forceinline__ void init_lane(Lane& L, char* lds, uint32_t G) {
+__device__ __forceinline__ void init_lane(Lane& L, char* lds, uint32_t G, uint32_t tid) {
   L.lds = lds;
-  L.lane = threadIdx.x & 63;
+  L.lane = tid & 63;
   L.col = L.lane & 15;
   L.grp = L.lane >> 4;
   L.odd = (L.grp & 1) != 0;
@@ -244,6 +244,7 @@
   }
   L.K2 = k2;
 }
+__device__ __forceinline__ void init_lane(Lane& L, char* lds, uint32_t G) { init_lane(L, lds, G, threadIdx.x); }
 
 __device__ __forceinline__ uint32_t group_lin(const Lane& L, const Chains& c) {
   const uint32_t X0 = L.odd ? c.v2 : c.v0, X1 = L.odd ? c.v3 : c.v1;
@@ -299,23 +300,27 @@
 };
 
 template <int THREADS = 1024>
-__device__ __forceinline__ StageSet<THREADS> stage_load(const KernelParams& p) {
+__device__ __forceinline__ StageSet<THREADS> stage_load(const KernelParams& p, uint32_t tid) {
   StageSet<THREADS> s;
 #pragma unroll
   for (int i = 0; i < StageSet<THREADS>::kRounds; i++) {
-    const int t = min((int)threadIdx.x + i * THREADS, 1023);
+    const int t = min((int)tid + i * THREADS, 1023);
     s.r[i].cv = *as_global<g_u32>(p.chain_tab + t);
     s.r[i].n0 = *as_global<g_u32x4>(p.nib_img + 8 * t);
     s.r[i].n1 = *as_global<g_u32x4>(p.nib_img + 8 * t + 4);
   }
   return s;
 }
-
-template <int THREADS = 1024>
-__device__ __forceinline__ void stage_store(const StageSet<THREADS>& s, char* lds) {
+template <int THREADS = 1024>
+__device__ __forceinline__ StageSet<THREADS> stage_load(const KernelParams& p) {
+  return stage_load<THREADS>(p, threadIdx.x);
+}
+
+template <int THREADS = 1024>
+__device__ __forceinline__ void stage_store(const StageSet<THREADS>& s, char* lds, uint32_t tid) {
 #pragma unroll
   for (int i = 0; i < StageSet<THREADS>::kRounds; i++) {
-    const int t = (int)threadIdx.x + i * THREADS;
+    const int t = (int)tid + i * THREADS;
     if (1024 % THREADS != 0 && t >= 1024) break;
     const StageRegs& r = s.r[i];
     const uint32_t k = (uint32_t)t >> 8, e = (uint32_t)t & 255u;
@@ -330,4 +335,8 @@
   __builtin_amdgcn_s_barrier();
   __builtin_amdgcn_fence(__ATOMIC_ACQUIRE, "workgroup", "local");
 }
-}
+template <int THREADS = 1024>
+__device__ __forceinline__ void stage_store(const StageSet<THREADS>& s, char* lds) {
+  stage_store<THREADS>(s, lds, threadIdx.x);
+}
+}
diff --git a/uflow_amd/csrc/frame_crc_kernels.hpp b/uflow_amd/csrc/frame_crc_kernels.hpp
--- a/uflow_amd/csrc/frame_crc_kernels.hpp
+++ b/uflow_amd/csrc/frame_crc_kernels.hpp
@@ -24,6 +24,8 @@
   uint32_t G;
   uint32_t* ctr;
   uint32_t front_ok;
+  uint32_t nrounds;
+  uint64_t round_frames;
   uint32_t* defer_list;
   uint32_t* defer_counts;
 };
@@ -34,6 +36,27 @@
 constexpr int kLeanRuns = 8;
 constexpr int lean_runs(int waves) { return waves == 8 ? 32 : kLeanRuns; }
 constexpr int kLeanWavesDefault = 8;
+#if defined(__HIP__) || defined(__HIPCC__)
+#define UFC_RHD __host__ __device__ inline
+#else
+#define UFC_RHD inline
+#endif
+constexpr uint64_t fixed_round_frames(int ncu, int waves, int round_sets) {
+  return (uint64_t)ncu * (uint64_t)waves * (uint64_t)(round_sets > 0 ? round_sets : 16 * lean_runs(waves) - 1) * 4;
+}
+UFC_RHD uint64_t fixed_round_count(uint64_t total, uint64_t chunk) { return (total + chunk - 1) / chunk; }
+UFC_RHD void fixed_round(uint64_t total, uint64_t chunk, uint64_t nrounds, uint64_t r, uint64_t* first,
+                         uint64_t* count) {
+  const uint64_t last = nrounds - 1;
+  const uint64_t cut = (nrounds > 1 && total - last * chunk < 4) ? 4u : 0u;
+  if (r < last) {
+    *first = r * chunk;
+    *count = chunk - (r + 1 == last ? cut : 0u);
+  } else {
+    *first = last * chunk - cut;
+    *count = total - *first;
+  }
+}
 constexpr int kSchedRange = 0;
 constexpr int kSchedClaim = 1;
 constexpr int kSchedInterleave = 2;
diff --git a/uflow_amd/csrc/ufc_api.cpp b/uflow_amd/csrc/ufc_api.cpp
--- a/uflow_amd/csrc/ufc_api.cpp
+++ b/uflow_amd/csrc/ufc_api.cpp
@@ -10,6 +10,7 @@
 #include <vector>
 
 #include "../../include/uflow_frame_codec.h"
+#include "../../include/uflow_fixed_rounds.h"
 #include "../../include/uflow_frame_crc.h"
 #include "crc_math.hpp"
 #include "frame_build.hpp"
@@ -164,13 +165,19 @@
   kp.nib_img = ctx->d_nib;
   kp.G = ctx->G;
   const uint64_t waves_per_block = (uint64_t)waves;
-  const uint64_t chunk = (uint64_t)ctx->ncu * waves_per_block * (16 * ufc_dev::lean_runs(waves) - 1) * 4;
+  const uint64_t chunk = ufc_dev::fixed_round_frames(ctx->ncu, waves, ctx->opt[UFC_OPT_FIXED_ROUND_SETS]);
   const uint64_t total = kp.nframes;
-  for (uint64_t f0 = 0, step = 0; f0 < total; f0 += step) {
+  const uint64_t nrounds = ufc_dev::fixed_round_count(total, chunk);
+  if (nrounds > 0x7FFFFFFFull) return UFC_ERR_INVALID_ARG;
+  const bool per_launch = ctx->opt[UFC_OPT_FIXED_ROUNDS] == UFC_FIXED_ROUNDS_LAUNCHES || sched == ufc_dev::kSchedClaim;
+  const uint64_t nlaunches = per_launch ? nrounds : 1;
+  for (uint64_t l = 0; l < nlaunches; l++) {
     ufc_dev::KernelParams c = kp;
-    c.nframes = std::min(chunk, total - f0);
-    if (total - f0 - c.nframes > 0 && total - f0 - c.nframes < 4) c.nframes -= 4;
-    step = c.nframes;
+    uint64_t f0 = 0, cnt = total;
+    if (per_launch) ufc_dev::fixed_round(total, chunk, nrounds, l, &f0, &cnt);
+    c.nframes = cnt;
+    c.nrounds = per_launch ? 1u : (uint32_t)nrounds;
+    c.round_frames = chunk;
     c.bytes = kp.bytes + f0 * kp.stride;
     if (kp.wbytes) c.wbytes = kp.wbytes + f0 * kp.stride;
     if (kp.crc_out) c.crc_out = kp.crc_out + f0;
@@ -178,7 +185,9 @@
     c.front_ok = (f0 > 0 || front_ok) ? 1u : 0u;
     const uint32_t slot = ctx->ctr_seq.fetch_add(1) % kCtrSlots;
     c.ctr = ctx->d_ctr + (size_t)slot * ctx->ncu * ufc_dev::kCtrWordsPerBlock;
-    const uint64_t nsets = (c.nframes + 3) / 4;
+    uint64_t first = 0, first_cnt = cnt;
+    if (!per_launch) ufc_dev::fixed_round(total, chunk, nrounds, 0, &first, &first_cnt);
+    const uint64_t nsets = (first_cnt + 3) / 4;
     uint64_t blocks = (nsets + waves_per_block - 1) / waves_per_block;
     if (blocks > (uint64_t)ctx->ncu) blocks = (uint64_t)ctx->ncu;
     if (blocks < 1) blocks = 1;
@@ -362,6 +371,12 @@
     case UFC_OPT_SEAL_KERNEL:
       if (value != UFC_SEAL_INLINE && value != UFC_SEAL_TWO_PASS) return UFC_ERR_INVALID_ARG;
       break;
+    case UFC_OPT_FIXED_ROUNDS:
+      if (value != UFC_FIXED_ROUNDS_KERNEL && value != UFC_FIXED_ROUNDS_LAUNCHES) return UFC_ERR_INVALID_ARG;
+      break;
+    case UFC_OPT_FIXED_ROUND_SETS:
+      if (value < 0 || value > 16 * ufc_dev::lean_runs(ufc_dev::kLeanWavesDefault) - 1) return UFC_ERR_INVALID_ARG;
+      break;
     default: return UFC_ERR_INVALID_ARG;
   }
   ctx->opt[option] = value;
@@ -371,6 +386,17 @@
 int ufc_ctx_get_option(const ufc_ctx* ctx, int option) {
   if (!ctx || option < 0 || option >= UFC_OPT_COUNT_) return UFC_ERR_INVALID_ARG;
   return ctx->opt[option];
+}
+
+int ufc_fixed_round(uint64_t n, int ncu, int round_sets, uint64_t round, uint64_t* first, uint64_t* count) {
+  const int waves = ufc_dev::kLeanWavesDefault;
+  if (n == 0 || ncu < 1 || round_sets < 0 || round_sets > 16 * ufc_dev::lean_runs(waves) - 1 || !first || !count)
+    return UFC_ERR_INVALID_ARG;
+  const uint64_t chunk = ufc_dev::fixed_round_frames(ncu, waves, round_sets);
+  const uint64_t nrounds = ufc_dev::fixed_round_count(n, chunk);
+  if (nrounds > 0x7FFFFFFFull || round >= nrounds) return UFC_ERR_INVALID_ARG;
+  ufc_dev::fixed_round(n, chunk, nrounds, round, first, count);
+  return (int)nrounds;
 }
 
 int ufc_ctx_create(ufc_ctx** out, int device) {
```

Result: no change. 6236 (-0.3%).
